# EmanueleCosenza/polyphemus

Hardware: AMD Instinct MI355X
Metric: bar-graphs/sec VAE fwd+bwd (+loss +Adam), LMD2 4-track x 32-ts synthetic (higher is better)
Workload: dtype f32 (fp16-pair MFMA products)

## Files before the change

### include/polyphemus_hip.h

```cpp
#ifndef POLYPHEMUS_HIP_H
#define POLYPHEMUS_HIP_H

#include <stdint.h>

#ifdef __cplusplus
extern "C" {
#endif

typedef void* pm_stream_t;

enum {
  PM_OK = 0,
  PM_E_INVALID = -1,
  PM_E_LAUNCH = -2,
  PM_E_UNSUPPORTED = -3
};

enum { PM_N_REL = 6, PM_N_DIST = 32, PM_N_SLOTS = 15, PM_N_PITCH = 131, PM_N_DUR = 99, PM_N_TOK = 230 };

#define PM_ABI_VERSION 9
int pm_abi_version(void);
const char* pm_build_info(void);

int pm_set_deterministic(int32_t on);
// ... 86 lines not shown
int pm_sample_structure(const float* s_logits , int32_t G, const PmStructureRules* rules, uint32_t seed,
                        float* s_f32 , uint8_t* s_u8 ,
                        int32_t* track_count , pm_stream_t stream);

int pm_notes_from_tokens(const int32_t* tokens , const float* s_tensor ,
                         int32_t G, int32_t n_bars, int64_t N, int32_t* seg_count ,
                         int32_t* seg_ptr , int32_t* bar_nodes , int32_t* node_ptr ,
                         int32_t* notes , int64_t capacity, int32_t* track_ptr ,
                         int32_t* totals , pm_stream_t stream);

#define PM_NOTES_IN_SCRATCH(B, n_bars) (3 * (int64_t)(B) * (n_bars) + 1 + 12 * (int64_t)(B))
int pm_tokens_from_notes(const int32_t* notes , const int32_t* track_ptr ,
                         int32_t B, int32_t n_bars, int64_t M, float* s_tensor ,
                         int32_t* tokens , int64_t capacity,
                         int32_t* scratch , int32_t* status ,
                         pm_stream_t stream);

int pm_edge_table(const float* nn_weight , const float* nn_bias , int32_t d,
                  float* T , pm_stream_t stream);
int pm_edge_table_bwd(const float* dT , int32_t d, float* d_nn_weight ,
                      float* d_nn_bias , pm_stream_t stream);
int pm_segreduce_fwd(const float* x , const float* T , const int32_t* plan,
                     int32_t N, int32_t E, int32_t G, int32_t d, float dropout_p, uint32_t seed,
                     uint32_t layer_uid, int32_t compact, float* A , pm_stream_t stream);
int pm_segreduce_fwd_planes(const float* x, const float* T, const int32_t* plan, int32_t N, int32_t E, int32_t G,
                            int32_t d, float dropout_p, uint32_t seed, uint32_t layer_uid, int32_t compact,
                            uint16_t* planes, int64_t plane_stride, pm_stream_t stream);
int pm_gcl_forward_fused(const float* x , const float* T , const int32_t* plan, int32_t N,
                         int32_t E, int32_t G, int32_t d, float dropout_p, uint32_t seed, uint32_t layer_uid,
                         const uint16_t* w_frag, const float* bias , int32_t use_classes,
                         float* h , double* col_stats ,
                         uint16_t* planes , int64_t plane_stride, pm_stream_t stream);
int pm_gcl_input_grad_fused(const uint16_t* dh_planes , int64_t plane_stride, const int32_t* plan,
                            int32_t N, int32_t E, int32_t G, int32_t d, const uint16_t* w_frag_t, int32_t use_classes,
                            float* dA , pm_stream_t stream);
typedef struct PmBnBwd {
  const float* h;
  const float* du;
  const float* mean; const float* var; const float* gamma; const float* beta;
  const double* acc3;
  float* dgamma; float* dbeta; float* dbias_pre;
  float eps; int32_t relu;
  int32_t add_residual;
  int32_t reserved;
} PmBnBwd;
int pm_gcl_input_grad_bn(const PmBnBwd* norm, uint16_t* dh_planes , int64_t plane_stride,
                         const int32_t* plan, int32_t N, int32_t E, int32_t G, int32_t d, const uint16_t* w_frag_t,
                         int32_t use_classes, float* dA , pm_stream_t stream);
enum { PM_ABSMAX_SLOTS = 64 };
typedef struct PmH2 {
  const uint32_t* absmax_in; const uint32_t* absmax_aux; float* scale_out; float w_scale; int32_t reserved;
} PmH2;
int pm_absmax(const float* x, int64_t n, uint32_t* out, pm_stream_t stream);
int pm_split_planes_frag_h2(const float* W, int32_t rows, int32_t cols, int32_t kind, int32_t n_mats, int64_t src_stride,
                            int64_t dst_stride, float w_scale, uint16_t* out, pm_stream_t stream);
int pm_gcl_forward_fused_h2(const float* x, const float* T, const int32_t* plan, int32_t N, int32_t E, int32_t G, int32_t d,
                            float dropout_p, uint32_t seed, uint32_t layer_uid, const uint16_t* w_frag, const float* bias,
                            int32_t use_classes, float* h, double* col_stats, uint16_t* planes, int64_t plane_stride,
                            const PmH2* h2, pm_stream_t stream);
int pm_gcl_input_grad_bn_h2(const PmBnBwd* norm, uint16_t* dh_planes, int64_t plane_stride, const int32_t* plan, int32_t N,
                            int32_t E, int32_t G, int32_t d, const uint16_t* w_frag_t, int32_t use_classes, float* dA,
                            const PmH2* h2, pm_stream_t stream);
int pm_bn_bwd_fused_h2(const float* x, const float* dy, int32_t O, int32_t C, const float* mean, const float* var, float eps,
                       const float* gamma, const float* beta, int relu, float* dgamma, float* dbeta, float* dbias_pre,
                       double* acc3, uint16_t* dx_planes, int64_t plane_stride, int32_t sums_ready, const PmH2* h2,
                       pm_stream_t stream);
int pm_gcl_input_grad_fused_h2(const uint16_t* dh_planes, int64_t plane_stride, const int32_t* plan, int32_t N, int32_t E,
                               int32_t G, int32_t d, const uint16_t* w_frag_t, int32_t use_classes, float* dA,
                               const float* dh_scale, float w_scale, pm_stream_t stream);
int pm_gcl_weight_grad_fused_h2(const uint16_t* a_planes, int64_t a_plane_stride, const uint16_t* dh_planes,
                                int64_t dh_plane_stride, const int32_t* plan, int32_t N, int32_t E, int32_t G, int32_t d,
                                int32_t use_classes, float* dW, const float* a_scale, const float* dh_scale,
                                pm_stream_t stream);
int pm_gcl_weight_grad_fused(const uint16_t* a_planes , int64_t a_plane_stride,
                             const uint16_t* dh_planes , int64_t dh_plane_stride, const int32_t* plan,
                             int32_t N, int32_t E, int32_t G, int32_t d, int32_t use_classes, float* dW ,
                             pm_stream_t stream);
int pm_gcl_forward_from_planes(const uint16_t* a_planes , int64_t plane_stride, const int32_t* plan,
                               int32_t N, int32_t E, int32_t G, int32_t d, const uint16_t* w_frag,
                               const float* bias , int32_t use_classes, float* h ,
                               double* col_stats , pm_stream_t stream);
int pm_gcl_forward_from_planes_h2(const uint16_t* a_planes, int64_t plane_stride, const int32_t* plan, int32_t N, int32_t E,
                                  int32_t G, int32_t d, const uint16_t* w_frag, const float* bias, int32_t use_classes,
                                  float* h, double* col_stats, const float* a_scale, float w_scale, pm_stream_t stream);
int pm_rows_times_weight(const float* X, int32_t ldx, int32_t N, int32_t K, const uint16_t* w_frag, int32_t kind,
                         int32_t w_tiles, int32_t Nout, const float* bias , float* C, int32_t ldc,
                         pm_stream_t stream);
int pm_rows_times_weight_longk(const float* X, int32_t ldx, int32_t N, int32_t K, const uint16_t* w_frag, int32_t kind,
                               int32_t w_pitch, int32_t Nout, float* C, int32_t ldc, pm_stream_t stream);
int pm_rows_tn_weight_grad(const float* A, int32_t lda, int32_t M, const float* B, int32_t ldb, int32_t Nn, int32_t K,
                           float* C , int32_t ldc, float* colsum_a , pm_stream_t stream);
typedef struct PmNormSums {
  const float* h;
  const float* mean; const float* var; const float* gamma; const float* beta;
  float eps; int32_t relu;
  double* acc3;
  uint32_t* absmax_out;
} PmNormSums;
int pm_segreduce_bwd_norm(const float* x, const float* T, const float* dA, const float* dres, const int32_t* plan,
                          int32_t N, int32_t E, int32_t G, int32_t d, float dropout_p, uint32_t seed,
                          uint32_t layer_uid, int32_t compact, float* dx, float* dT, const PmNormSums* next_norm,
                          pm_stream_t stream);
int pm_segreduce_bwd(const float* x, const float* T, const float* dA ,
                     const float* dres ,
                     const int32_t* plan, int32_t N, int32_t E, int32_t G, int32_t d, float dropout_p,
                     uint32_t seed, uint32_t layer_uid, int32_t compact, float* dx ,
                     float* dT , pm_stream_t stream);

int pm_bar_aggregate_fwd(const float* x, const float* T, const int32_t* plan, int32_t N, int32_t E, int32_t G, int32_t d,
                         float dropout_p, uint32_t seed, uint32_t layer_uid, uint16_t* planes, int64_t plane_stride,
                         const PmH2* h2 , pm_stream_t stream);
int pm_bar_aggregate_bwd(const float* x, const float* T, const float* dA , const float* dres ,
                         const int32_t* plan, int32_t N, int32_t E, int32_t G, int32_t d, float dropout_p, uint32_t seed,
                         uint32_t layer_uid, float* dx , float* dT ,
                         const PmNormSums* next_norm , pm_stream_t stream);

enum { PM_GEMM_RELU = 1, PM_GEMM_ACCUM = 2,
       PM_GEMM_RELU_ADD = 16 ,
       PM_GEMM_ZEROED = 8 ,
       PM_GEMM_PARTITION = 4  };
int pm_gemm_config(int32_t transA, int32_t M, int32_t N, int32_t K);
int pm_gemm_force_config(int32_t cfg);
int pm_gemm_f32(int transA, int transB, int32_t M, int32_t N, int32_t K, const float* A, int32_t lda,
                const float* B, int32_t ldb, float* C, int32_t ldc, const float* bias, int flags,
                int split_k, const int32_t* rowmap, int32_t rows_per_entry, const int32_t* dyn_entries,
                pm_stream_t stream);
int pm_gemm_f32_grouped(int transA, int transB, int32_t M, int32_t N, int32_t K, const float* A, int32_t lda,
                        const float* B, int32_t ldb, float* C, int32_t ldc, const float* bias, int flags,
                        int split_k, const int32_t* rowmap, int32_t rows_per_entry, const int32_t* dyn_entries,
                        int32_t n_groups, int64_t a_group_stride, int64_t b_group_stride, int64_t c_group_stride,
                        int64_t bias_group_stride, int32_t map_group_stride, int32_t dyn_group_stride,
                        pm_stream_t stream);
int pm_split_planes(const float* src, int64_t n, uint16_t* planes, int64_t plane_stride ,
                    pm_stream_t stream);
typedef struct PmGemmDesc {
  int32_t transA, transB, M, N, K;
  const float* A; int32_t lda;
  const float* B; int32_t ldb;
  float* C; int32_t ldc;
  const float* bias;
  int32_t flags, split_k;
  const int32_t* rowmap; int32_t rows_per_entry;
// ... 4 lines not shown
  int32_t b_split_rows; int64_t b_shared_off;
  int32_t c_split_rows; int64_t c_shared_off;
  double* col_stats;
  int32_t operand_planes;
  int64_t a_plane_stride, b_plane_stride;
  const int32_t* class_ptr;
  int32_t class_block;
  const void* b_frag;
  float* a_colsum;
} PmGemmDesc;
int pm_split_planes_frag(const float* W, int32_t rows, int32_t cols, int32_t kind, int32_t n_mats, int64_t src_stride,
                         int64_t dst_stride, uint16_t* out, pm_stream_t stream);
int pm_gemm_f32_desc(const PmGemmDesc* desc, pm_stream_t stream);

int pm_bn_stats(const float* x, int32_t O, int32_t C, int32_t I, float* mean ,
                float* var , float* running_mean ,
                float* running_var, float momentum, double* scratch , pm_stream_t stream);
int pm_bn_apply(const float* x, int32_t O, int32_t C, int32_t I, const float* mean, const float* var,
                float eps, const float* gamma, const float* beta, const float* residual ,
                int relu, float* y, pm_stream_t stream);
int pm_bn_bwd(const float* x, const float* dy, int32_t O, int32_t C, int32_t I, const float* mean,
              const float* var, float eps, const float* gamma, const float* beta, int relu,
              float* dgamma , float* dbeta , float* dbias_pre , float* dx,
              double* scratch , pm_stream_t stream);
#define PM_BN_SCRATCH(C) (256 * 3 * (C) + 4 * (C))
#define PM_BN_SMALL_MAX_ROWS 2048
int pm_bn_small_fwd(const float* x, int32_t O, int32_t C, float eps, const float* gamma, const float* beta,
                    const float* residual , int relu, float* y, float* mean ,
                    float* var , float* running_mean , float* running_var,
                    float momentum, pm_stream_t stream);
int pm_bn_small_bwd(const float* x, const float* dy, int32_t O, int32_t C, const float* mean, const float* var, float eps,
                    const float* gamma, const float* beta, int relu, float* dgamma , float* dbeta ,
                    float* dbias_pre , float* dx, pm_stream_t stream);
int pm_bn_partial_sums(const float* x, const float* dy , int32_t O, int32_t C, int32_t I, const float* mean,
                       const float* var, float eps, const float* gamma, const float* beta, int relu,
                       double* sums , double* scratch , pm_stream_t stream);
int pm_bn_stats_from_sums(const double* sums , double count, int32_t C, float* mean, float* var,
                          float* running_mean , float* running_var, float momentum, pm_stream_t stream);
int pm_bn_bwd_from_sums(const float* x, const float* dy, int32_t O, int32_t C, int32_t I, const float* mean,
                        const float* var, float eps, const float* gamma, const float* beta, int relu,
                        const double* sums_local , const double* sums_global ,
                        double count_global, float* dgamma , float* dbeta , float* dbias_pre ,
                        float* dx, double* scratch , pm_stream_t stream);

enum { PM_BN_REPL = 8 };
int pm_bn_apply_fused(const float* x, int32_t O, int32_t C, const double* sums, float eps, const float* gamma,
                      const float* beta, const float* residual , int relu, float* y,
                      float* mean , float* var , float* running_mean ,
                      float* running_var, float momentum, pm_stream_t stream);
int pm_bn_apply_fused_absmax(const float* x, int32_t O, int32_t C, const double* sums, float eps, const float* gamma,
                             const float* beta, const float* residual, int relu, float* y, float* mean, float* var,
                             float* running_mean, float* running_var, float momentum, uint32_t* absmax_out,
                             pm_stream_t stream);
int pm_bn_bwd_fused(const float* x, const float* dy, int32_t O, int32_t C, const float* mean, const float* var,
                    float eps, const float* gamma, const float* beta, int relu, float* dgamma, float* dbeta,
                    float* dbias_pre , float* dx , double* acc3,
                    uint16_t* dx_planes ,
                    int64_t plane_stride ,
                    int32_t sums_ready ,
                    pm_stream_t stream);
int pm_bn_bwd_sums(const float* x, const float* dy, int32_t O, int32_t C, const float* mean, const float* var, float eps,
                   const float* gamma, const float* beta, int relu, double* acc3, pm_stream_t stream);
int pm_bn_fold_weights(const float* W, int32_t rows, int32_t cols, const float* bias, const float* gamma, const float* beta,
                       const float* running_mean, const float* running_var, float eps, float* W_out, float* b_out,
                       pm_stream_t stream);
int pm_bn_counters_update(int64_t* counters , const int64_t* inc , const int64_t* sel ,
                          const int32_t* group_cnt , int32_t n, pm_stream_t stream);
int pm_relu_bwd(const float* dy, const float* y, int64_t n, float* dx, pm_stream_t stream);
int pm_relu_bwd_planes(const float* dy, const float* h, int64_t n, float* dh, uint16_t* planes, int64_t plane_stride,
                       pm_stream_t stream);
int pm_relu_residual_fwd(const float* x, const float* res, int64_t n, float* y, pm_stream_t stream);
int pm_dropout_rows(const float* x, int64_t rows, int32_t cols, float p, uint32_t seed, uint32_t site, float* y,
                    pm_stream_t stream);
int pm_add(const float* a, const float* b, int64_t n, float* out, pm_stream_t stream);
int pm_colsum_acc(const float* x, int32_t M, int32_t C, int32_t ld, float* out , pm_stream_t stream);
int pm_colsum_rows_acc(const float* x, int32_t C, int32_t ld, const int32_t* rowmap, int32_t rows_per_entry,
                       const int32_t* dyn_entries, int32_t max_entries, float* out , pm_stream_t stream);
int pm_reparam_fwd(const float* mu, const float* log_var, const float* eps, int64_t n, float* z, pm_stream_t stream);
int pm_reparam_bwd(const float* dz, const float* log_var, const float* eps, int64_t n, float* dmu ,
                   float* dlog_var , pm_stream_t stream);

int pm_embed_tables(const float* w_pitch_drum , const float* b_pitch_drum,
                    const float* w_pitch_nd, const float* b_pitch_nd, const float* w_dur ,
                    const float* b_dur, const float* bn_drum_g, const float* bn_drum_b,
                    const float* bn_nd_g, const float* bn_nd_b, const float* bn_dur_g, const float* bn_dur_b,
                    float* rm_drum, float* rv_drum, float* rm_nd, float* rv_nd, float* rm_dur, float* rv_dur,
                    const int32_t* tok_hist , int32_t d, int training, float eps, float momentum,
                    float* tables , float* stats ,
                    pm_stream_t stream);
int pm_embed_gather(const float* tables, const int32_t* tokens , const uint8_t* is_drum,
                    int32_t N, int32_t d, int32_t n_slots, float* X , pm_stream_t stream);
int pm_embed_bwd_scatter(const float* dX , const int32_t* tokens, const int32_t* plan, int32_t N,
                         int32_t E, int32_t G, int32_t d, int32_t n_slots,
                         float* S , pm_stream_t stream);
int pm_chord_pad_fwd(const float* tables, const float* chord_w , const float* chord_b,
                     const uint8_t* is_drum, int32_t N, int32_t d, int32_t n_slots, float* cvec ,
                     float* y , pm_stream_t stream);
int pm_chord_pad_bwd(const float* dy , const uint8_t* is_drum, int32_t N, int32_t d, int32_t n_slots,
                     const float* tables, const float* chord_w, float* gsum ,
                     float* d_chord_w , float* S , pm_stream_t stream);
int pm_chord_pad_vec(const float* tables, const float* chord_w, const float* chord_b, int32_t d, int32_t n_slots,
                     float* cvec , pm_stream_t stream);
int pm_chord_tables_fwd(const float* tables , const float* chord_w , int32_t d, int32_t n_slots,
                        float* PT, const float* chord_b , float* cvec ,
                        pm_stream_t stream);
int pm_chord_sum_fwd(const float* PT, const float* cvec, const int32_t* tokens , const uint8_t* is_drum, int32_t N,
// ... 187 lines not shown

int pm_comm_unique_id(uint8_t* id128 );
int pm_comm_init(const uint8_t* id128 , int32_t rank, int32_t world, void** comm );
int pm_comm_destroy(void* comm);
int pm_allreduce(float* buf, int64_t count, void* comm, pm_stream_t stream);

uint32_t pm_dropout_hash(uint32_t seed, uint32_t layer_uid, uint32_t eid, uint32_t channel);

enum { PM_PROF_NCLASS_PUBLIC = 35 };
int pm_prof_configure(int64_t class_mask, int32_t stride);
int pm_prof_begin(int32_t max_events);
int pm_prof_end(double* ms , double* work , int64_t* count );

#define PM_MAX_LAYERS 16
typedef struct PmLin { int64_t w, b; } PmLin;
typedef struct PmBn { int64_t w, b, rm, rv; } PmBn;
typedef struct PmGcn {
  int64_t nn_w, nn_b;
  int64_t weight[PM_MAX_LAYERS];
  int64_t bias[PM_MAX_LAYERS];
  PmBn norm[PM_MAX_LAYERS];
} PmGcn;
typedef struct PmVaeLayout {
  int32_t d, n_bars, n_layers;
  int32_t flags;
  PmLin enc_conv0; PmBn enc_bn1; PmLin enc_conv4; PmBn enc_bn5; PmLin enc_lin1, enc_lin4, enc_s_bars;
  PmLin enc_pitch_nd, enc_pitch_d, enc_dur; PmBn enc_bn_nd, enc_bn_d, enc_bn_dur; PmLin enc_chord;
  PmGcn enc_gcn; PmLin enc_gate; PmBn enc_gate_bn; PmLin enc_c_bars;
  PmLin enc_merge; PmBn enc_bn_merge; PmLin enc_mu, enc_lv;
  PmLin dec_lin; PmBn dec_bn; PmLin dec_s_bars, dec_s_lin1, dec_s_lin4, dec_conv1; PmBn dec_bn2; PmLin dec_conv4;
  PmLin dec_c_bars; PmGcn dec_gcn; PmLin dec_chord, dec_pitch_d, dec_pitch_nd, dec_dur;
  float dropout;
  int32_t reserved;
} PmVaeLayout;
typedef struct PmBatch {
  const int64_t* edge_index; const int32_t* edge_type; const int32_t* edge_dist;
  const int64_t* bars; const int64_t* batch; const uint8_t* is_drum; const int32_t* tokens; const float* s_tensor;
  int32_t N, E, G, B;
  int32_t n_slots;
  int32_t flags;
  const float* ce_scale;
} PmBatch;
int pm_vae_step_reload_switches(void);
int64_t pm_vae_layout_bytes(void);
int64_t pm_vae_step_state_bytes(void);
int64_t pm_vae_step_workspace_bytes(const PmVaeLayout* lay, int32_t N, int32_t E, int32_t G, int32_t B,
                                    int32_t n_slots);
int pm_vae_step_forward(const PmVaeLayout* lay, const float* params, float* buffers, float* grads,
                        const PmBatch* batch, int32_t* plan, const float* eps , float msg_dropout,
                        uint32_t seed_enc, uint32_t seed_dec, float beta, int structure_loss_on_logits,
                        void* workspace, int64_t workspace_bytes, void* state, double* losses ,
                        pm_stream_t stream);
int pm_vae_step_info(const void* state, int32_t* info );
int pm_vae_step_outputs(const void* state, float* s_logits, float* c_logits, float* mu, float* log_var,
                        pm_stream_t stream);
enum { PM_SAVED_GCN_H = 0,
       PM_SAVED_GCN_X,
       PM_SAVED_GCN_XIN,
       PM_SAVED_GCN_MEAN, PM_SAVED_GCN_VAR,
       PM_SAVED_GCN_T,
       PM_SAVED_X0,
       PM_SAVED_MERGE_PRE, PM_SAVED_MERGE_MEAN, PM_SAVED_MERGE_VAR,
       PM_SAVED_DEC_PRE, PM_SAVED_DEC_MEAN, PM_SAVED_DEC_VAR,
       PM_SAVED_ENC_CNN_LIN1 };
int pm_vae_step_saved(const void* state, int32_t what, int32_t stack, int32_t layer, int64_t* byte_offset, int64_t* numel);
int pm_bn_relu_decisions(const float* x , const float* mean, const float* var, const float* gamma, const float* beta,
                         float eps, int64_t rows, int32_t C, uint8_t* out , pm_stream_t stream);
int pm_vae_step_set_metrics(void* state, int64_t* counts);
int pm_vae_step_set_output_grads(void* state, const float* d_s_logits , const float* d_c_logits ,
                                 const float* d_mu , const float* d_log_var , pm_stream_t stream);
int pm_vae_step_output_views(const void* state, int64_t* byte_offset , int64_t* numel );
int pm_vae_step_backward_decoder(void* state, pm_stream_t stream);
int pm_vae_step_join_decoder_grads(void* state, pm_stream_t stream);
int pm_vae_step_backward_encoder_heads(void* state, pm_stream_t stream);
int pm_vae_step_backward_encoder(void* state, pm_stream_t stream);
int pm_vae_step_backward_encoder_tail(void* state, pm_stream_t stream);

#ifdef __cplusplus
}
#endif
#endif
```

### polyphemus_amd/_lib.py

```python
from __future__ import annotations

import ctypes as C
import os
from typing import Optional

import torch

_HERE = os.path.dirname(os.path.abspath(__file__))
LIB_PATH = os.environ.get("PM_LIB_PATH") or os.path.join(_HERE, "libpolyphemus_hip.so")

PROF_NCLASS = 40
PLAN_FIELDS = ["rowptr", "csr_src", "csr_dist", "csr_eid", "colptr", "csc_dst", "csc_reldist", "csc_eid",
               "csc_invcnt", "node_bar", "bar_ptr", "group_list", "group_cnt", "tok_hist", "row_list", "node_trel", "trk_list", "trk_cnt", "scratch"]

_SIGS = {
    "pm_plan_layout": "iiip",
    "pm_gcl_tile_order": "piipi",
    "pm_row_tile_order": "ipi",
    "pm_plan_build": "pppppppiiiiips",
    "pm_edge_attrs_to_ids": "pipps",
    "pm_tokens_from_onehot": "pips",
    "pm_batch_flags": "pppiipps",
    "pm_edge_table": "ppips",
    "pm_edge_table_bwd": "pipps",
    "pm_graph_count": "pippppps",
    "pm_graph_emit": "piippllppppppps",
    "pm_binary_from_logits": "pifpps",
    "pm_mtp_from_logits": "ppilppps",
    "pm_segreduce_fwd": "pppiiiifuuips",
    "pm_segreduce_fwd_planes": "pppiiiifuuipls",
    "pm_gcl_forward_fused": "pppiiiifuuppipppls",
    "pm_gcl_input_grad_fused": "plpiiiipips",
    "pm_gcl_input_grad_bn": "pplpiiiipips",
    "pm_chord_pad_vec": "pppiips",
    "pm_chord_tables_fwd": "ppiippps",
    "pm_chord_sum_fwd": "ppppiiips",
    "pm_chord_sum_bwd": "pppiiiiips",
    "pm_chord_tables_bwd_w": "ppiipps",
    "pm_chord_tables_bwd_x": "ppiips",
    "pm_bn_bwd_sums": "ppiippfppips",
    "pm_gcl_weight_grad_fused": "plplpiiiiips",
    "pm_gcl_forward_from_planes": "plpiiiippipps",
    "pm_rows_times_weight": "piiipiiippis",
    "pm_rows_times_weight_longk": "piiipiiipis",
    "pm_rows_tn_weight_grad": "piipiiipips",
    "pm_segreduce_bwd": "pppppiiiifuuipps",
    "pm_segreduce_bwd_norm": "pppppiiiifuuippps",
    "pm_gemm_f32": "iiiiipipipipiipips",
    "pm_gemm_f32_grouped": "iiiiipipipipiipipilllliis",
    "pm_gemm_f32_desc": "ps",
    "pm_gemm_config": "iiii",
    "pm_gemm_force_config": "i",
    "pm_bn_stats": "piiippppfps",
    "pm_bn_small_fwd": "piifpppipppppfs",
    "pm_bn_small_bwd": "ppiippfppipppps",
    "pm_bn_apply": "piiippfpppips",
    "pm_bn_partial_sums": "ppiiippfppipps",
    "pm_bn_stats_from_sums": "pDippppfs",
    "pm_bn_bwd_from_sums": "ppiiippfppippDppppps",
    "pm_bn_bwd": "ppiiippfppippppps",
    "pm_bn_apply_fused": "piipfpppipppppfs",
    "pm_bn_bwd_fused": "ppiippfppipppppplis",
    "pm_split_planes": "plpls",
    "pm_split_planes_frag": "piiiillps",
    "pm_relu_bwd": "pplps",
    "pm_add": "pplps",
    "pm_bn_counters_update": "ppppis",
    "pm_grad_accumulate": "pplfis",
    "pm_colsum_acc": "piiips",
    "pm_colsum_rows_acc": "piipipips",
    "pm_reparam_fwd": "ppplps",
    "pm_reparam_bwd": "ppplpps",
    "pm_embed_tables": "pppppppppppppppppppiiffpps",
    "pm_embed_gather": "pppiiips",
    "pm_chord_pad_fwd": "ppppiiipps",
    "pm_chord_pad_bwd": "ppiiippppps",
    "pm_embed_bwd_scatter": "pppiiiiips",
    "pm_embed_tables_bwd": "ppppppppppppifpppppppppppps",
    "pm_embed_tables_bwd_sync": "ppppppppppppifppppppppppppppps",
    "pm_gate_fwd": "pppiips",
    "pm_attnpool_fwd": "ppppfpppiiiipps",
    "pm_attnpool_bwd": "ppppfpppppiiiipppppppps",
    "pm_attnpool_bwd_sums": "ppppfpppiiiips",
    "pm_attnpool_bwd_from_sums": "ppppfpppppiiiipppppppppDs",
    "pm_relu_residual_fwd": "pplps",
    "pm_bn_fold_weights": "piipppppfpps",
    "pm_dropout_rows": "plifuups",
    "pm_bar_broadcast_fwd": "ppiiiips",
    "pm_bar_broadcast_bwd": "ppiiiips",
    "pm_conv3x3_fwd": "pppiiiiiips",
    "pm_conv3x3_bwd_data": "ppiiiiiips",
    "pm_conv3x3_bwd_weight": "ppiiiiiipps",
    "pm_maxpool4_fwd": "plps",
    "pm_maxpool4_bwd": "pplps",
    "pm_cnn_enc_fwd": "pppppppppiffppppppppppppppls",
    "pm_cnn_dec_fwd": "pppppppiffppppppppls",
    "pm_cnn_enc_bwd": "pppppppppppppppifppppppppppppls",
    "pm_content_ce": "ppppiifppppps",
    "pm_content_ce_scaled": "ppppiifpppppps",
    "pm_unembed_ce": "pppppppppiiiiifpppppppps",
    "pm_unembed_dh": "pppppiiiiippis",
    "pm_unembed_dh_scratch_bytes": "i",
    "pm_unembed_row_counts_len": "ii",
    "pm_unembed_dw": "pppiiiiippppps",
    "pm_unembed_row_lists": "ppiiiiipppps",
    "pm_unembed_ce_rows": "pppppppppiiiiifpppppppppps",
    "pm_unembed_dh_rows": "pppppiiiiipppps",
    "pm_unembed_scratch_bytes": "i",
    "pm_kld": "ppiifppps",
    "pm_unembed_bias_grads": "ppiippps",
    "pm_bce_logits": "pplfpps",
    "pm_content_accuracy": "pppips",
    "pm_structure_metrics": "pplps",
    "pm_adam_step": "pppplffffifs",
    "pm_comm_unique_id": "p",
    "pm_comm_init": "piip",
    "pm_comm_destroy": "p",
    "pm_allreduce": "plps",
    "pm_prof_configure": "li",
    "pm_prof_begin": "i",
    "pm_prof_end": "ppp",
    "pm_vae_step_workspace_bytes": "piiiii",
    "pm_vae_step_forward": "pppppppfuufiplpps",
    "pm_vae_step_info": "pp",
    "pm_vae_step_outputs": "ppppps".replace(" ", ""),
    "pm_vae_step_set_output_grads": "ppppps",
    "pm_vae_step_saved": "piiipp",
    "pm_vae_step_output_views": "ppp",
    "pm_bn_relu_decisions": "pppppflips",
    "pm_vae_step_backward_decoder": "ps",
    "pm_vae_step_backward_encoder": "ps",
    "pm_vae_step_backward_encoder_tail": "ps",
    "pm_vae_step_join_decoder_grads": "ps",
    "pm_vae_step_backward_encoder_heads": "ps",
    "pm_vae_step_reload_switches": "",
    "pm_relu_bwd_planes": "pplppls",
    "pm_absmax": "plps",
    "pm_split_planes_frag_h2": "piiiillfps",
    "pm_gcl_forward_fused_h2": "pppiiiifuuppippplps",
    "pm_gcl_input_grad_bn_h2": "pplpiiiipipps",
    "pm_gcl_weight_grad_fused_h2": "plplpiiiiippps",
    "pm_bn_bwd_fused_h2": "ppiippfppippppplips",
    "pm_gcl_input_grad_fused_h2": "plpiiiipippfs",
    "pm_bn_apply_fused_absmax": "piipfpppipppppfps",
    "pm_bar_aggregate_fwd": "pppiiiifuuplps",
    "pm_bar_aggregate_bwd": "pppppiiiifuuppps",
    "pm_gcl_forward_from_planes_h2": "plpiiiippipppfs",
    "pm_set_deterministic": "i",
    "pm_get_deterministic": "",
    "pm_deterministic_faults": "",
    "pm_h2_clamp_events": "i",
    "pm_h2_clamp_init": "",
    "pm_overflow_snapshot": "ps",
    "pm_overflow_poison": "pps",
    "pm_grad_nonfinite_check": "plpppfffis",
    "pm_adam_step_guarded": "pppplffffps",
    "pm_adam_bias_scalars": "plfffps",
    "pm_vae_step_set_metrics": "pp",
    "pm_unembed_ce_metrics": "pppppppppiiiiifppppppppppps",
    "pm_unembed_ce_rows_metrics": "pppppppppiiiiifppppppppppppps",
    "pm_content_accuracy_slots": "pppiipps",
    "pm_train_metric_counts": "pppiipplps",
    "pm_grad_sumsq": "plps",
    "pm_grad_nonfinite_check_sumsq": "plpppfffips",
    "pm_grad_clip_finish": "pffps",
    "pm_adam_step_clipped": "pppplffffipps",
    "pm_adam_step_ema": "ppppplffffiffpps",
    "pm_buffer_swap": "ppls",
    "pm_sample_tokens": "plfifups",
    "pm_mtp_from_tokens": "ppilppps",
    "pm_sample_chords": "pplpupps",
    "pm_node_tracks": "pilppps",
    "pm_sample_structure": "pipuppps",
    "pm_notes_from_tokens": "ppiilppppplpps",
    "pm_tokens_from_notes": "ppiilpplpps",
}
_CT = {"p": C.c_void_p, "i": C.c_int32, "l": C.c_int64, "f": C.c_float, "u": C.c_uint32, "s": C.c_void_p, "D": C.c_double}
_RET64 = {"pm_vae_step_workspace_bytes", "pm_vae_layout_bytes", "pm_vae_step_state_bytes", "pm_unembed_scratch_bytes",
          "pm_unembed_dh_scratch_bytes", "pm_unembed_row_counts_len"}
ABI_VERSION = 9
EXPORTED = sorted(list(_SIGS) + ["pm_abi_version", "pm_build_info", "pm_dropout_hash", "pm_sample_hash",
                                 "pm_vae_layout_bytes", "pm_vae_step_state_bytes"])



class PmChordRules(C.Structure):
    _fields_ = [("temperature", C.c_float * 2), ("top_k", C.c_int32), ("top_p", C.c_float), ("min_notes", C.c_int32 * 4),
                ("max_notes", C.c_int32 * 4), ("pitch_mask", (C.c_uint32 * 4) * 4)]


class PmStructureRules(C.Structure):
# ... 107 lines not shown
```

### polyphemus_amd/csrc/common.h

```cpp
#pragma once
#include <hip/hip_runtime.h>
#include <stdint.h>
#include "../../include/polyphemus_hip.h"

#define PM_WAVE 64

static inline int pm_check_launch() {
  hipError_t e = hipGetLastError();
  return e == hipSuccess ? PM_OK : PM_E_LAUNCH;
}

static inline int pm_device_slot() {
  int d = 0;
  if (hipGetDevice(&d) != hipSuccess || d < 0 || d >= 16) d = 0;
  return d;
}

static inline int64_t pm_cdiv(int64_t a, int64_t b) { return (a + b - 1) / b; }
static inline int64_t pm_align4(int64_t x) { return (x + 3) & ~int64_t(3); }

struct PmPlanView {
  const int32_t* rowptr; const int32_t* csr_src; const int32_t* csr_dist; const int32_t* csr_eid;
  const int32_t* colptr; const int32_t* csc_dst; const int32_t* csc_reldist; const int32_t* csc_eid;
  const float* csc_invcnt; const int32_t* node_bar; const int32_t* bar_ptr; const int32_t* group_list;
// ... 97 lines not shown
  for (int o = 32; o > 0; o >>= 1) v += __shfl_xor(v, o, 64);
  return v;
}
__device__ static inline double pm_wave_sum_d(double v) {
#pragma unroll
  for (int o = 32; o > 0; o >>= 1) v += __shfl_xor(v, o, 64);
  return v;
}
typedef __bf16 pm_bf16x2 __attribute__((ext_vector_type(2)));
typedef float pm_f32x2 __attribute__((ext_vector_type(2)));
typedef unsigned int pm_u32x2 __attribute__((ext_vector_type(2)));
__device__ static inline unsigned pm_pk_bf16(float a, float b) {
  pm_f32x2 v = {a, b};
  return __builtin_bit_cast(unsigned, __builtin_convertvector(v, pm_bf16x2));
}
__device__ static inline void pm_split3_pair(float a, float b, unsigned& h1, unsigned& h2, unsigned& h3) {
  h1 = pm_pk_bf16(a, b);
  a -= __uint_as_float(h1 << 16); b -= __uint_as_float(h1 & 0xffff0000u);
  h2 = pm_pk_bf16(a, b);
  a -= __uint_as_float(h2 << 16); b -= __uint_as_float(h2 & 0xffff0000u);
  h3 = pm_pk_bf16(a, b);
}
typedef _Float16 pm_f16x2 __attribute__((ext_vector_type(2)));
__device__ static inline unsigned pm_pk_f16(float a, float b) {
  pm_f32x2 v = {a, b};
  return __builtin_bit_cast(unsigned, __builtin_convertvector(v, pm_f16x2));
}
__device__ static inline void pm_split2h_pair(float a, float b, unsigned& h1, unsigned& h2) {
  h1 = pm_pk_f16(a, b);
  const pm_f16x2 hv = __builtin_bit_cast(pm_f16x2, h1);
  a -= (float)hv.x; b -= (float)hv.y;
  h2 = pm_pk_f16(a, b);
}
__device__ static inline float pm_pow2_scale(float bound, int target) {
  if (!(bound > 0.f) || !(bound < 3.0e38f)) return 1.f;
  const int e = (int)((__float_as_uint(bound) >> 23) & 0xff) - 126;
  int k = target - e;
  k = k < -120 ? -120 : (k > 120 ? 120 : k);
  return __uint_as_float((unsigned)(k + 127) << 23);
}
__device__ static inline float pm_clamp_f16(float v) { return fminf(fmaxf(v, -65504.f), 65504.f); }
__device__ static inline float pm_clamp_f16(float v, bool& cut) {
  const float c = fminf(fmaxf(v, -65504.f), 65504.f);
  cut = cut || (c != v);
  return c;
}
__device__ static inline float pm_absmax_read(const unsigned* __restrict__ p) {
  static_assert(PM_ABSMAX_SLOTS == 64, "one slot per lane");
  float v = __uint_as_float(p[__lane_id()]);
#pragma unroll
  for (int o = 32; o > 0; o >>= 1) v = fmaxf(v, __shfl_xor(v, o, 64));
  return v;
}
__device__ static inline void pm_absmax_block(unsigned* __restrict__ out, float v, unsigned* sm) {
  v = fabsf(v);
#pragma unroll
  for (int o = 32; o > 0; o >>= 1) v = fmaxf(v, __shfl_xor(v, o, 64));
  if ((threadIdx.x & 63) == 0) atomicMax(sm, __float_as_uint(v));
  __syncthreads();
  if (threadIdx.x == 0) atomicMax(out + (blockIdx.x % PM_ABSMAX_SLOTS), *sm);
}
__device__ static inline void pm_store_planes4(uint16_t* __restrict__ planes, int64_t plane_stride, int64_t idx, float x0,
                                               float x1, float x2, float x3) {
  unsigned l1, l2, l3, u1, u2, u3;
  pm_split3_pair(x0, x1, l1, l2, l3);
  pm_split3_pair(x2, x3, u1, u2, u3);
  const pm_u32x2 p1 = {l1, u1}, p2 = {l2, u2}, p3 = {l3, u3};
  *reinterpret_cast<pm_u32x2*>(planes + idx) = p1;
  *reinterpret_cast<pm_u32x2*>(planes + plane_stride + idx) = p2;
  *reinterpret_cast<pm_u32x2*>(planes + 2 * plane_stride + idx) = p3;
}
__device__ static inline double pm_repl_sum(const double* __restrict__ acc, int nacc, int C, int a, int c) {
  double t = 0;
#pragma unroll
  for (int r = 0; r < PM_BN_REPL; ++r) t += acc[((int64_t)r * nacc + a) * C + c];
  return t;
}
__device__ static inline float pm_bn_bwd_elem(float x, float dy, float mean, float rstd, float ga, float be, float m0,
                                              float m1, int relu) {
  const float xh = (x - mean) * rstd;
  float du = dy;
  if (relu && !(xh * ga + be > 0.f)) du = 0.f;
  return ga * rstd * (du - m0 - xh * m1);
}
__device__ static inline float pm_wave_max(float v) {
#pragma unroll
  for (int o = 32; o > 0; o >>= 1) v = fmaxf(v, __shfl_xor(v, o, 64));
  return v;
}
#endif
```

### polyphemus_amd/csrc/gemm.hip

```cpp
#include "common.h"
#include "prof.h"
#include <stdlib.h>

typedef float f32x16 __attribute__((ext_vector_type(16)));

#ifndef PM_BD_DUAL
#define PM_BD_DUAL 0
#endif
#ifndef PM_TN_DUAL
#define PM_TN_DUAL 1
#endif
#ifndef PM_PL_WAVES
#define PM_PL_WAVES 5
#endif
#ifndef PM_BD_WAVES
#define PM_BD_WAVES 5
#endif
struct GemmArgs {
  const float* A; const float* B; float* C; const float* bias;
  const int32_t* rowmap; const int32_t* dyn_entries;
  int M, N, K, lda, ldb, ldc, rpe, flags, kper, ntm, ntn;
  int64_t a_boff, b_boff, c_boff, bias_boff; int map_boff, dyn_boff;
  int b_split, c_split; int64_t b_hi, c_hi;
  int ngroups, packed;
// ... 878 lines not shown
      break;
    default: launch_t<128, 128, 32, 2, 2, 2>(transA, transB, va, vb, grid, st, g); break;
  }
  pm_prof_close(st, pe);
  return pm_check_launch();
}

extern "C" int pm_gemm_f32_grouped(int transA, int transB, int32_t M, int32_t N, int32_t K, const float* A, int32_t lda,
                                   const float* B, int32_t ldb, float* C, int32_t ldc, const float* bias, int flags,
                                   int split_k, const int32_t* rowmap, int32_t rows_per_entry,
                                   const int32_t* dyn_entries, int32_t n_groups, int64_t a_group_stride,
                                   int64_t b_group_stride, int64_t c_group_stride, int64_t bias_group_stride,
                                   int32_t map_group_stride, int32_t dyn_group_stride, pm_stream_t stream) {
  PmGemmDesc q;
  q.transA = transA; q.transB = transB; q.M = M; q.N = N; q.K = K; q.A = A; q.lda = lda; q.B = B; q.ldb = ldb;
  q.C = C; q.ldc = ldc; q.bias = bias; q.flags = flags; q.split_k = split_k; q.rowmap = rowmap;
  q.rows_per_entry = rows_per_entry; q.dyn_entries = dyn_entries; q.n_groups = n_groups;
  q.a_group_stride = a_group_stride; q.b_group_stride = b_group_stride; q.c_group_stride = c_group_stride;
  q.bias_group_stride = bias_group_stride; q.map_group_stride = map_group_stride; q.dyn_group_stride = dyn_group_stride;
  q.b_split_rows = 0; q.b_shared_off = 0; q.c_split_rows = 0; q.c_shared_off = 0; q.col_stats = nullptr;
  q.operand_planes = 0; q.a_plane_stride = 0; q.b_plane_stride = 0; q.a_colsum = nullptr;
  q.class_ptr = nullptr; q.class_block = 0; q.b_frag = nullptr;
  return pm_gemm_f32_desc(&q, stream);
}

extern "C" int pm_gemm_f32(int transA, int transB, int32_t M, int32_t N, int32_t K, const float* A, int32_t lda,
                           const float* B, int32_t ldb, float* C, int32_t ldc, const float* bias, int flags,
                           int split_k, const int32_t* rowmap, int32_t rows_per_entry, const int32_t* dyn_entries,
                           pm_stream_t stream) {
  return pm_gemm_f32_grouped(transA, transB, M, N, K, A, lda, B, ldb, C, ldc, bias, flags, split_k, rowmap,
                             rows_per_entry, dyn_entries, 1, 0, 0, 0, 0, 0, 0, stream);
}

__global__ void __launch_bounds__(256) k_split_planes(const float* __restrict__ src, int64_t n4, uint16_t* __restrict__ planes,
                                                      int64_t plane_stride) {
  for (int64_t i = (int64_t)blockIdx.x * blockDim.x + threadIdx.x; i < n4; i += (int64_t)gridDim.x * blockDim.x) {
    const float4 v = reinterpret_cast<const float4*>(src)[i];
    pm_store_planes4(planes, plane_stride, i * 4, v.x, v.y, v.z, v.w);
  }
}
extern "C" int pm_split_planes(const float* src, int64_t n, uint16_t* planes, int64_t plane_stride, pm_stream_t stream) {
  if (!src || !planes || n <= 0 || (n & 3) || plane_stride < n || (plane_stride & 3) || ((uintptr_t)src % 16) ||
      ((uintptr_t)planes % 8))
    return PM_E_INVALID;
  int64_t grid = pm_cdiv(n / 4, 256);
  if (grid > 4096) grid = 4096;
  hipLaunchKernelGGL(k_split_planes, dim3((unsigned)grid), dim3(256), 0, (hipStream_t)stream, src, n / 4, planes, plane_stride);
  return pm_check_launch();
}

template <bool H2>
__global__ void __launch_bounds__(256) k_split_planes_frag(const float* __restrict__ W, int rows, int cols, int kind,
                                                           int64_t src_stride, int64_t dst_stride,
                                                           uint16_t* __restrict__ out, float w_scale, unsigned* clamps) {
  bool cut = false;
  const float* src = W + (int64_t)blockIdx.y * src_stride;
  uint16_t* dst = out + (int64_t)blockIdx.y * dst_stride;
  const int64_t chunks = (int64_t)rows * cols / 8;
  for (int64_t c = (int64_t)blockIdx.x * blockDim.x + threadIdx.x; c < chunks; c += (int64_t)gridDim.x * blockDim.x) {
    float x[8];
    int64_t blk;
    int lane;
    if (kind == 0) {
      const int n = (int)(c / (cols / 8)), k0 = (int)(c % (cols / 8)) * 8;
      const float4 u = *reinterpret_cast<const float4*>(src + (int64_t)n * cols + k0);
      const float4 w = *reinterpret_cast<const float4*>(src + (int64_t)n * cols + k0 + 4);
      x[0] = u.x; x[1] = u.y; x[2] = u.z; x[3] = u.w; x[4] = w.x; x[5] = w.y; x[6] = w.z; x[7] = w.w;
      blk = (int64_t)(n >> 5) * (cols / 16) + (k0 >> 4);
      lane = ((k0 >> 3) & 1) * 32 + (n & 31);
    } else {
      const int n = (int)(c % cols), k0 = (int)(c / cols) * 8;
#pragma unroll
      for (int e = 0; e < 8; ++e) x[e] = src[(int64_t)(k0 + e) * cols + n];
      blk = (int64_t)(k0 >> 4) * (cols / 32) + (n >> 5);
      lane = ((k0 >> 3) & 1) * 32 + (n & 31);
    }
    unsigned p1[4], p2[4], p3[4];
    uint16_t* o = dst + blk * 1536 + lane * 8;
    if constexpr (H2) {
#pragma unroll
      for (int e = 0; e < 4; ++e) pm_split2h_pair(pm_clamp_f16(x[2 * e] * w_scale, cut), pm_clamp_f16(x[2 * e + 1] * w_scale, cut), p1[e], p2[e]);
    } else {
#pragma unroll
      for (int e = 0; e < 4; ++e) pm_split3_pair(x[2 * e], x[2 * e + 1], p1[e], p2[e], p3[e]);
      *reinterpret_cast<u32x4*>(o + 1024) = u32x4{p3[0], p3[1], p3[2], p3[3]};
    }
    *reinterpret_cast<u32x4*>(o) = u32x4{p1[0], p1[1], p1[2], p1[3]};
    *reinterpret_cast<u32x4*>(o + 512) = u32x4{p2[0], p2[1], p2[2], p2[3]};
  }
  if (H2 && cut && clamps) atomicAdd(clamps, 1u);
}
static int split_planes_frag_impl(const float* W, int32_t rows, int32_t cols, int32_t kind, int32_t n_mats,
                                  int64_t src_stride, int64_t dst_stride, float w_scale, uint16_t* out, pm_stream_t stream) {
  if (!W || !out || rows <= 0 || cols <= 0 || (rows % 32) || (cols % 32) || (kind != 0 && kind != 1) || n_mats <= 0 ||
      ((uintptr_t)W % 16) || ((uintptr_t)out % 16) || (src_stride % 4) || (dst_stride % 8))
    return PM_E_INVALID;
  int64_t grid = pm_cdiv((int64_t)rows * cols / 8, 256);
  if (grid > 2048) grid = 2048;
  if (w_scale > 0.f)
    hipLaunchKernelGGL(k_split_planes_frag<true>, dim3((unsigned)grid, (unsigned)n_mats), dim3(256), 0, (hipStream_t)stream, W,
                       rows, cols, kind, src_stride, dst_stride, out, w_scale, pm_h2_clamp_word());
  else
    hipLaunchKernelGGL(k_split_planes_frag<false>, dim3((unsigned)grid, (unsigned)n_mats), dim3(256), 0, (hipStream_t)stream, W,
                       rows, cols, kind, src_stride, dst_stride, out, 0.f, nullptr);
  return pm_check_launch();
}
extern "C" int pm_split_planes_frag(const float* W, int32_t rows, int32_t cols, int32_t kind, int32_t n_mats,
                                    int64_t src_stride, int64_t dst_stride, uint16_t* out, pm_stream_t stream) {
  return split_planes_frag_impl(W, rows, cols, kind, n_mats, src_stride, dst_stride, 0.f, out, stream);
}
extern "C" int pm_split_planes_frag_h2(const float* W, int32_t rows, int32_t cols, int32_t kind, int32_t n_mats,
                                       int64_t src_stride, int64_t dst_stride, float w_scale, uint16_t* out, pm_stream_t stream) {
  if (!(w_scale > 0.f)) return PM_E_INVALID;
  return split_planes_frag_impl(W, rows, cols, kind, n_mats, src_stride, dst_stride, w_scale, out, stream);
}
__global__ void __launch_bounds__(256) k_absmax(const float* __restrict__ x, int64_t n, unsigned* __restrict__ out) {
  __shared__ unsigned sm;
  if (threadIdx.x == 0) sm = 0u;
  __syncthreads();
  float m = 0.f;
  const int64_t n4 = n >> 2, stride = (int64_t)gridDim.x * blockDim.x;
  for (int64_t i = (int64_t)blockIdx.x * blockDim.x + threadIdx.x; i < n4; i += stride) {
    const float4 v = reinterpret_cast<const float4*>(x)[i];
    m = fmaxf(fmaxf(m, fmaxf(fabsf(v.x), fabsf(v.y))), fmaxf(fabsf(v.z), fabsf(v.w)));
  }
  if (blockIdx.x == 0 && threadIdx.x < (int)(n & 3)) m = fmaxf(m, fabsf(x[(n4 << 2) + threadIdx.x]));
  pm_absmax_block(out, m, &sm);
}
extern "C" int pm_absmax(const float* x, int64_t n, uint32_t* out, pm_stream_t stream) {
  if (!x || !out || n <= 0 || ((uintptr_t)x % 16)) return PM_E_INVALID;
  int64_t grid = pm_cdiv(n / 4 + 1, 256 * 4);
  if (grid > 512) grid = 512;
  hipLaunchKernelGGL(k_absmax, dim3((unsigned)grid), dim3(256), 0, (hipStream_t)stream, x, n, out);
  return pm_check_launch();
}

PmProfState g_pm_prof = {false, 0, 0, nullptr, ~0ull, 1, {0}};

extern "C" int pm_prof_configure(int64_t class_mask, int32_t stride) {
  if (stride < 1) return PM_E_INVALID;
  g_pm_prof.mask = (uint64_t)class_mask;
  g_pm_prof.stride = stride;
  return PM_OK;
}


extern "C" int pm_prof_begin(int32_t max_events) {
  PmProfState& p = g_pm_prof;
  if (max_events <= 0) return PM_E_INVALID;
  if (p.cap < max_events) {
    PmProfEvent* ev = (PmProfEvent*)realloc(p.ev, sizeof(PmProfEvent) * max_events);
    if (!ev) return PM_E_INVALID;
    p.ev = ev;
    for (int i = p.cap; i < max_events; ++i) {
      if (hipEventCreate(&p.ev[i].a) != hipSuccess || hipEventCreate(&p.ev[i].b) != hipSuccess) return PM_E_LAUNCH;
    }
    p.cap = max_events;
  }
  p.n = 0;
  for (int c = 0; c < PM_PROF_NCLASS; ++c) p.seen[c] = 0;
  p.on = true;
  return PM_OK;
}
extern "C" int pm_prof_end(double* ms, double* work, int64_t* count) {
  PmProfState& p = g_pm_prof;
  p.on = false;
  if (!ms || !work || !count) return PM_E_INVALID;
  for (int c = 0; c < PM_PROF_NCLASS; ++c) { ms[c] = 0; work[c] = 0; count[c] = 0; }
  for (int i = 0; i < p.n; ++i) {
    float t = 0.f;
    if (hipEventSynchronize(p.ev[i].b) != hipSuccess || hipEventElapsedTime(&t, p.ev[i].a, p.ev[i].b) != hipSuccess)
      return PM_E_LAUNCH;
    ms[p.ev[i].cls] += t; work[p.ev[i].cls] += p.ev[i].work; count[p.ev[i].cls] += 1;
  }
  p.n = 0;
  return PM_OK;
}
```

### polyphemus_amd/csrc/linear.hip

```cpp
#include "gcl_tiles.h"
#include <type_traits>
#include <stdlib.h>
#include "prof.h"
#include "wide.h"

#ifndef ROWS_NMW
#define ROWS_NMW 4
#endif
template <int D> constexpr int rows_nmw() { return D == 256 ? ROWS_NMW : 4; }
template <int D> constexpr int rows_threads() { return (rows_nmw<D>() + 4) * 64; }
template <int D, int BKIND>
__global__ void __launch_bounds__(rows_threads<D>()) __attribute__((amdgpu_waves_per_eu((rows_nmw<D>() + 4) / 4, (rows_nmw<D>() + 4) / 4)))
k_rows_w(const float* __restrict__ X, int ldx, int N, const char* __restrict__ wfrag, int wtiles, int nblk,
         const float* __restrict__ bias, float* __restrict__ C, int ldc) {
  constexpr int NMW = rows_nmw<D>(), WC = D / NMW, TN = WC / 32, KS = D / 16, RB = D * 2, PL = BM * RB;
  extern __shared__ __attribute__((aligned(16))) char smem[];
  float* const sC = reinterpret_cast<float*>(smem + 3 * PL);
  int m0 = 0, rows = BM;
  if (!pm_row_tile(N, blockIdx.x, m0, rows)) return;
  const bool full = rows > BM / 2;
  N = min(N, m0 + rows);
  const int tid = threadIdx.x, lane = tid & 63, wave = tid >> 6, li = lane & 31, lh = lane >> 5;
  if (wave >= NMW) {
    constexpr int LPR = D / 4, RPW = 64 / LPR, NR = BM / (4 * RPW);
    const int st = tid - NMW * 64, c4 = st % LPR, r0 = st / LPR;
    const __amdgpu_buffer_rsrc_t crs = __builtin_amdgcn_make_buffer_rsrc(C, 0, GCL_OOB, 0x00020000);
    __syncthreads();
#pragma unroll 1
    for (int qb = 0; qb < nblk; ++qb) {
      __syncthreads();
      __syncthreads();
      float4 bv = make_float4(0.f, 0.f, 0.f, 0.f);
      if (bias) bv = *reinterpret_cast<const float4*>(bias + qb * D + c4 * 4);
#pragma unroll
      for (int k = 0; k < NR; ++k) {
        const int rr = r0 + k * 4 * RPW, row = m0 + rr;
        float4 v = *reinterpret_cast<const float4*>(sC + rr * D + c4 * 4);
        v.x += bv.x; v.y += bv.y; v.z += bv.z; v.w += bv.w;
        __builtin_amdgcn_raw_buffer_store_b128(__builtin_bit_cast(u32x4, v), crs,
            row < N ? (int)(((int64_t)row * ldc + qb * D + c4 * 4) * 4) : GCL_OOB, 0, 0);
      }
    }
    return;
  }
  {
    const __amdgpu_buffer_rsrc_t rs = __builtin_amdgcn_make_buffer_rsrc(const_cast<float*>(X), 0, GCL_OOB, 0x00020000);
    constexpr int CPR = D / 8, NST = NMW * 64, NCHK = BM * CPR / NST;
    u32x4 v[NCHK][2];
#pragma unroll
    for (int k = 0; k < NCHK; ++k) {
      const int ci = tid + k * NST, rr = ci / CPR, ch = ci % CPR, row = m0 + rr;
#pragma unroll
      for (int h = 0; h < 2; ++h)
        v[k][h] = __builtin_amdgcn_raw_buffer_load_b128(rs, row < N ? (int)(((int64_t)row * ldx + ch * 8 + h * 4) * 4) : GCL_OOB, 0, 0);
    }
#pragma unroll
    for (int k = 0; k < NCHK; ++k) {
      const int ci = tid + k * NST, rr = ci / CPR, ch = ci % CPR;
      unsigned p1[4], p2[4], p3[4];
#pragma unroll
      for (int h = 0; h < 2; ++h) {
        pm_split3_pair(__uint_as_float(v[k][h][0]), __uint_as_float(v[k][h][1]), p1[2 * h], p2[2 * h], p3[2 * h]);
        pm_split3_pair(__uint_as_float(v[k][h][2]), __uint_as_float(v[k][h][3]), p1[2 * h + 1], p2[2 * h + 1], p3[2 * h + 1]);
      }
      char* dst = smem + rr * RB + ((ch ^ (rr & 15)) << 4);
      *reinterpret_cast<u32x4*>(dst) = u32x4{p1[0], p1[1], p1[2], p1[3]};
      *reinterpret_cast<u32x4*>(dst + PL) = u32x4{p2[0], p2[1], p2[2], p2[3]};
      *reinterpret_cast<u32x4*>(dst + 2 * PL) = u32x4{p3[0], p3[1], p3[2], p3[3]};
    }
  }
  const __amdgpu_buffer_rsrc_t brs = __builtin_amdgcn_make_buffer_rsrc(const_cast<char*>(wfrag), 0, GCL_OOB, 0x00020000);
  auto bload = [&](bf16x8 (&dst)[3][TN], int gs) {
    const int qb = min(gs / KS, nblk - 1), ks = gs % KS;
    const int n0 = qb * D + wave * WC;
    const int soff = __builtin_amdgcn_readfirstlane(BKIND == 0 ? ((n0 >> 5) * KS + ks) * 3072 : (ks * wtiles + (n0 >> 5)) * 3072);
#pragma unroll
    for (int j = 0; j < TN; ++j)
#pragma unroll
      for (int p = 0; p < 3; ++p)
        dst[p][j] = __builtin_bit_cast(bf16x8, __builtin_amdgcn_raw_buffer_load_b128(brs, lane * 16, soff + j * (BKIND == 0 ? KS : 1) * 3072 + p * 1024, 0));
  };
  bf16x8 bq[GCL_BDEPTH][3][TN];
#pragma unroll
  for (int s2 = 0; s2 < GCL_BDEPTH; ++s2) bload(bq[s2], s2);
  __syncthreads();
  auto aload = [&](bf16x8 (&a)[3][2], int ks) {
#pragma unroll
    for (int p = 0; p < 3; ++p)
#pragma unroll
      for (int i = 0; i < 2; ++i) {
        const int rr = i * 32 + li;
        a[p][i] = *reinterpret_cast<const bf16x8*>(smem + p * PL + rr * RB + (((ks * 2 + lh) ^ (rr & 15)) << 4));
      }
  };
  bf16x8 af[2][3][2];
  aload(af[0], 0);
  auto blocks = [&](auto ni_tag) {
  constexpr int NI = decltype(ni_tag)::value;
#pragma unroll 1
  for (int qb = 0; qb < nblk; ++qb) {
    f32x16 acc[2][TN];
#pragma unroll
    for (int i = 0; i < 2; ++i)
#pragma unroll
      for (int j = 0; j < TN; ++j)
#pragma unroll
        for (int r = 0; r < 16; ++r) acc[i][j][r] = 0.f;
#pragma unroll
    for (int ks = 0; ks < KS; ++ks) {
      aload(af[(ks + 1) & 1], (ks + 1) % KS);
      constexpr int PA[6] = {2, 1, 0, 1, 0, 0}, PB[6] = {0, 1, 2, 0, 1, 0};
#pragma unroll
      for (int t6 = 0; t6 < 6; ++t6)
#pragma unroll
        for (int i = 0; i < NI; ++i)
#pragma unroll
          for (int j = 0; j < TN; ++j)
            acc[i][j] = __builtin_amdgcn_mfma_f32_32x32x16_bf16(af[ks & 1][PA[t6]][i], bq[ks % GCL_BDEPTH][PB[t6]][j], acc[i][j], 0, 0, 0);
      bload(bq[ks % GCL_BDEPTH], qb * KS + ks + GCL_BDEPTH);
      __builtin_amdgcn_sched_barrier(0);
    }
    __syncthreads();
#pragma unroll
    for (int i = 0; i < 2; ++i)
#pragma unroll
      for (int r = 0; r < 16; ++r)
#pragma unroll
        for (int j = 0; j < TN; ++j)
          sC[(i * 32 + (r & 3) + 8 * (r >> 2) + 4 * lh) * D + wave * WC + j * 32 + li] = acc[i][j][r];
    __syncthreads();
  }
  };
  if (full) blocks(std::integral_constant<int, 2>{});
  else blocks(std::integral_constant<int, 1>{});
}

extern "C" int pm_rows_times_weight(const float* X, int32_t ldx, int32_t N, int32_t K, const uint16_t* w_frag, int32_t kind,
                                    int32_t w_tiles, int32_t Nout, const float* bias, float* C, int32_t ldc,
                                    pm_stream_t stream) {
  if (!X || !w_frag || !C || N <= 0 || (K != 128 && K != 256 && K != 512) || Nout <= 0 || (Nout % K) || (kind != 0 && kind != 1) ||
      ldx < K || ldc < Nout || (ldx & 3) || (ldc & 3) || ((uintptr_t)X % 16) || ((uintptr_t)C % 16) ||
      ((uintptr_t)w_frag % 16) || (bias && ((uintptr_t)bias % 16)) || (int64_t)N * ldx * 4 >= 0x7fffffffLL ||
      (int64_t)N * ldc * 4 >= 0x7fffffffLL || (kind == 1 && w_tiles * 32 < Nout))
    return PM_E_INVALID;
  if (K == 512)
    return pm_wide_rows_times_weight(X, ldx, N, w_frag, kind, w_tiles, Nout, bias, C, ldc, (hipStream_t)stream);
  hipStream_t st = (hipStream_t)stream;
  const dim3 grid(pm_row_grid(N));
  const size_t lds = (size_t)3 * BM * K * 2 + (size_t)BM * K * 4;
  const int pe = pm_prof_open(st, PM_PROF_ROWS_W, 2.0 * N * (double)K * Nout);
#define LAUNCH(DD, KD)                                                                                                 \
  do {                                                                                                                 \
    static bool once_dev[16] = {}; bool& once = once_dev[pm_device_slot()];                                                                                          \
    if (!once) {                                                                                                       \
      hipFuncSetAttribute((const void*)k_rows_w<DD, KD>, hipFuncAttributeMaxDynamicSharedMemorySize, 160 * 1024);      \
      once = true;                                                                                                     \
    }                                                                                                                  \
    hipLaunchKernelGGL((k_rows_w<DD, KD>), grid, dim3(rows_threads<DD>()), lds, st, X, ldx, N, reinterpret_cast<const char*>(w_frag), \
                       w_tiles, Nout / K, bias, C, ldc);                                                               \
  } while (0)
  if (K == 256) { if (kind == 0) LAUNCH(256, 0); else LAUNCH(256, 1); }
  else { if (kind == 0) LAUNCH(128, 0); else LAUNCH(128, 1); }
#undef LAUNCH
  pm_prof_close(st, pe);
  return pm_check_launch();
}

template <int D, int BKIND>
__global__ void __launch_bounds__(rows_threads<D>()) __attribute__((amdgpu_waves_per_eu((rows_nmw<D>() + 4) / 4, (rows_nmw<D>() + 4) / 4)))
k_rows_wk(const float* __restrict__ X, int ldx, int N, int K, const char* __restrict__ wfrag, int wpitch,
          float* __restrict__ C, int ldc) {
  constexpr int NMW = rows_nmw<D>(), WC = D / NMW, TN = WC / 32, HS = D + 8, NTHR = rows_threads<D>();
  extern __shared__ __attribute__((aligned(16))) char smem[];
  float* const sH = reinterpret_cast<float*>(smem);
  const int nchunk = K / CH;
  int m0 = 0, rows = BM;
  if (!pm_row_tile(N, blockIdx.x, m0, rows)) return;
  const bool full = rows > BM / 2;
  N = min(N, m0 + rows);
  const int tid = threadIdx.x, lane = tid & 63, wave = tid >> 6;
  if (wave >= NMW) {
    const int pt = tid - NMW * 64, q = pt & 31, prow = pt >> 5;
    const __amdgpu_buffer_rsrc_t xrs = __builtin_amdgcn_make_buffer_rsrc(const_cast<float*>(X), 0, GCL_OOB, 0x00020000);
    auto issue = [&](float4 (&xs)[8], int c) {
#pragma unroll
      for (int ps = 0; ps < 8; ++ps) {
        const int row = m0 + ps * 8 + prow;
        xs[ps] = __builtin_bit_cast(float4, __builtin_amdgcn_raw_buffer_load_b128(
            xrs, (row < N && c < nchunk) ? (int)(((int64_t)row * ldx + c * CH + q * 4) * 4) : GCL_OOB, 0, 0));
      }
    };
    auto put = [&](const float4 (&xs)[8], int c) {
      char* img = smem + (c & 1) * IMG;
#pragma unroll
      for (int ps = 0; ps < 8; ++ps) {
        const int rr = ps * 8 + prow;
        unsigned l1, l2, l3, u1, u2, u3;
        pm_split3_pair(xs[ps].x, xs[ps].y, l1, l2, l3);
        pm_split3_pair(xs[ps].z, xs[ps].w, u1, u2, u3);
        const pm_u32x2 p1 = {l1, u1}, p2 = {l2, u2}, p3 = {l3, u3};
        char* dst = img + rr * ROWB + (((q >> 1) ^ (rr & 15)) << 4) + ((q & 1) << 3);
        *reinterpret_cast<pm_u32x2*>(dst) = p1;
        *reinterpret_cast<pm_u32x2*>(dst + PLANE) = p2;
        *reinterpret_cast<pm_u32x2*>(dst + 2 * PLANE) = p3;
      }
    };
    float4 xa[8], xb[8];
    issue(xa, 0);
    issue(xb, 1);
    __builtin_amdgcn_sched_barrier(0);
    put(xa, 0);
    __syncthreads();
#pragma unroll 1
    for (int c = 0; c < nchunk; c += 2) {
      issue(xa, c + 2);
      __builtin_amdgcn_sched_barrier(0);
      put(xb, c + 1);
      __syncthreads();
      if (c + 1 >= nchunk) break;
      issue(xb, c + 3);
      __builtin_amdgcn_sched_barrier(0);
      put(xa, c + 2);
      __syncthreads();
    }
  } else {
    const int li = lane & 31, lh = lane >> 5;
    f32x16 acc[2][TN];
#pragma unroll
    for (int i = 0; i < 2; ++i)
#pragma unroll
      for (int j = 0; j < TN; ++j)
#pragma unroll
        for (int r = 0; r < 16; ++r) acc[i][j][r] = 0.f;
    const __amdgpu_buffer_rsrc_t brs = __builtin_amdgcn_make_buffer_rsrc(const_cast<char*>(wfrag), 0, GCL_OOB, 0x00020000);
    const int n0 = wave * WC;
    auto bload = [&](bf16x8 (&dst)[3][TN], int gs) {
      const int kk = min(gs, nchunk * 8 - 1);
      const int soff = __builtin_amdgcn_readfirstlane(BKIND == 0 ? ((n0 >> 5) * wpitch + kk) * 3072 : (kk * (D / 32) + (n0 >> 5)) * 3072);
#pragma unroll
      for (int j = 0; j < TN; ++j)
#pragma unroll
        for (int p = 0; p < 3; ++p)
          dst[p][j] = __builtin_bit_cast(bf16x8, __builtin_amdgcn_raw_buffer_load_b128(brs, lane * 16, soff + j * (BKIND == 0 ? wpitch : 1) * 3072 + p * 1024, 0));
    };
    bf16x8 bq[GCL_BDEPTH][3][TN];
#pragma unroll
    for (int s2 = 0; s2 < GCL_BDEPTH; ++s2) bload(bq[s2], s2);
    __syncthreads();
    auto chunks = [&](auto ni_tag) {
      constexpr int NI = decltype(ni_tag)::value;
#pragma unroll 1
      for (int c = 0; c < nchunk; ++c) {
        const char* img = smem + (c & 1) * IMG;
#pragma unroll
        for (int ks = 0; ks < 8; ++ks) {
          bf16x8 a[3][NI];
#pragma unroll
          for (int p = 0; p < 3; ++p)
#pragma unroll
            for (int i = 0; i < NI; ++i) {
              const int rr = i * 32 + li;
              a[p][i] = *reinterpret_cast<const bf16x8*>(img + p * PLANE + rr * ROWB + (((ks * 2 + lh) ^ (rr & 15)) << 4));
            }
          constexpr int PA[6] = {2, 1, 0, 1, 0, 0}, PB[6] = {0, 1, 2, 0, 1, 0};
#pragma unroll
          for (int t6 = 0; t6 < 6; ++t6)
#pragma unroll
            for (int i = 0; i < NI; ++i)
#pragma unroll
              for (int j = 0; j < TN; ++j)
                acc[i][j] = __builtin_amdgcn_mfma_f32_32x32x16_bf16(a[PA[t6]][i], bq[ks % GCL_BDEPTH][PB[t6]][j], acc[i][j], 0, 0, 0);
          bload(bq[ks % GCL_BDEPTH], c * 8 + ks + GCL_BDEPTH);
          __builtin_amdgcn_sched_barrier(0);
        }
        __syncthreads();
      }
    };
    if (full) chunks(std::integral_constant<int, 2>{});
    else chunks(std::integral_constant<int, 1>{});
#pragma unroll
    for (int j = 0; j < TN; ++j)
#pragma unroll
      for (int i = 0; i < 2; ++i)
#pragma unroll
        for (int r = 0; r < 16; ++r)
          sH[(i * 32 + (r & 3) + 8 * (r >> 2) + 4 * lh) * HS + n0 + j * 32 + li] = acc[i][j][r];
  }
  __syncthreads();
  constexpr int NG = 512 / D, RG = BM / NG;
  static_assert(NTHR >= 512, "row groups");
  const int col = tid % D, rg = tid / D;
  const __amdgpu_buffer_rsrc_t crs = __builtin_amdgcn_make_buffer_rsrc(C, 0, GCL_OOB, 0x00020000);
  if (tid >= 512) return;
#pragma unroll 8
  for (int k = 0; k < RG; ++k) {
    const int rr = rg * RG + k, row = m0 + rr;
    __builtin_amdgcn_raw_buffer_store_b32(__float_as_uint(sH[rr * HS + col]), crs, row < N ? (int)(((int64_t)row * ldc + col) * 4) : GCL_OOB, 0, 0);
  }
}

extern "C" int pm_rows_times_weight_longk(const float* X, int32_t ldx, int32_t N, int32_t K, const uint16_t* w_frag,
                                          int32_t kind, int32_t w_pitch, int32_t Nout, float* C, int32_t ldc,
                                          pm_stream_t stream) {
  if (!X || !w_frag || !C || N <= 0 || K <= 0 || (K % CH) || (Nout != 128 && Nout != 256 && Nout != 512) || (kind != 0 && kind != 1) ||
      ldx < K || ldc < Nout || (ldx & 3) || ((uintptr_t)X % 16) || ((uintptr_t)w_frag % 16) ||
      (int64_t)N * ldx * 4 >= 0x7fffffffLL || (int64_t)N * ldc * 4 >= 0x7fffffffLL || (kind == 0 && w_pitch * 16 < K))
    return PM_E_INVALID;
  if (Nout == 512)
    return pm_wide_rows_times_weight_longk(X, ldx, N, K, w_frag, kind, w_pitch, C, ldc, (hipStream_t)stream);
  hipStream_t st = (hipStream_t)stream;
  const dim3 grid(pm_row_grid(N));
  const size_t lds = 2 * IMG;
  const int pe = pm_prof_open(st, PM_PROF_ROWS_W, 2.0 * N * (double)K * Nout);
#define LAUNCH(DD, KD)                                                                                                 \
  do {                                                                                                                 \
    static bool once_dev[16] = {}; bool& once = once_dev[pm_device_slot()];                                                                                          \
    if (!once) {                                                                                                       \
      hipFuncSetAttribute((const void*)k_rows_wk<DD, KD>, hipFuncAttributeMaxDynamicSharedMemorySize, 160 * 1024);     \
      once = true;                                                                                                     \
    }                                                                                                                  \
    hipLaunchKernelGGL((k_rows_wk<DD, KD>), grid, dim3(rows_threads<DD>()), lds, st, X, ldx, N, K, reinterpret_cast<const char*>(w_frag), \
                       w_pitch, C, ldc);                                                                               \
  } while (0)
  if (Nout == 256) { if (kind == 0) LAUNCH(256, 0); else LAUNCH(256, 1); }
  else { if (kind == 0) LAUNCH(128, 0); else LAUNCH(128, 1); }
#undef LAUNCH
  pm_prof_close(st, pe);
  return pm_check_launch();
}


__global__ void __launch_bounds__(512) __attribute__((amdgpu_waves_per_eu(2, 2)))
k_rows_tn(const float* __restrict__ A, int lda, const float* __restrict__ B, int ldb, int K, int ntn, int nsplit,
          float* __restrict__ C, int ldc, float* __restrict__ colsum_a, unsigned* gate) {
  extern __shared__ __attribute__((aligned(16))) char smem[];
  const int ntile = gridDim.x / nsplit;
  int L = blockIdx.x;
  {
    const int total = gridDim.x, q = total >> 3, r = total & 7, xcd = L & 7, idx = L >> 3;
    L = (xcd < r ? xcd * (q + 1) : r * (q + 1) + (xcd - r) * q) + idx;
  }
  const int zs = L / ntile, within = L % ntile, ft = within / ntn, ct = within % ntn;
  const int kper = (((K + nsplit - 1) / nsplit + DW_KT - 1) / DW_KT) * DW_KT;
  const int kbeg = zs * kper, kend = min(kbeg + kper, K);
  if (kbeg >= kend) { pm_turn_skip_block(gate, 8); return; }
  const int nt = (kend - kbeg + DW_KT - 1) / DW_KT;
  const int tid = threadIdx.x, lane = tid & 63, wave = tid >> 6;
  const unsigned my_turn = blockIdx.x * 8 + wave;
  if (wave >= 4) {
    const int lt = tid - 256, c4 = lt & 31, r0 = lt >> 5;
    const __amdgpu_buffer_rsrc_t ars = __builtin_amdgcn_make_buffer_rsrc(const_cast<float*>(A), 0, GCL_OOB, 0x00020000);
    const __amdgpu_buffer_rsrc_t brs = __builtin_amdgcn_make_buffer_rsrc(const_cast<float*>(B), 0, GCL_OOB, 0x00020000);
    const int acol = (ft * DW_T + c4 * 4) * 4, bcol = (ct * DW_T + c4 * 4) * 4;
    float4 cs = make_float4(0.f, 0.f, 0.f, 0.f);
    const bool want_cs = colsum_a != nullptr && ct == 0;
    auto issue = [&](float4 (&v)[4][2], int t) {
#pragma unroll
      for (int j = 0; j < 4; ++j) {
        const int row = kbeg + t * DW_KT + r0 + j * 8;
        const bool ok = t < nt && row < kend;
        v[j][0] = __builtin_bit_cast(float4, __builtin_amdgcn_raw_buffer_load_b128(ars, ok ? (int)((int64_t)row * lda * 4) + acol : GCL_OOB, 0, 0));
        v[j][1] = __builtin_bit_cast(float4, __builtin_amdgcn_raw_buffer_load_b128(brs, ok ? (int)((int64_t)row * ldb * 4) + bcol : GCL_OOB, 0, 0));
      }
    };
    auto put = [&](const float4 (&v)[4][2], int t) {
      char* st = smem + (t & 1) * DW_STAGE;
#pragma unroll
      for (int j = 0; j < 4; ++j) {
        if (want_cs) { cs.x += v[j][0].x; cs.y += v[j][0].y; cs.z += v[j][0].z; cs.w += v[j][0].w; }
#pragma unroll
        for (int o = 0; o < 2; ++o) {
          unsigned l1, l2, l3, u1, u2, u3;
          pm_split3_pair(v[j][o].x, v[j][o].y, l1, l2, l3);
          pm_split3_pair(v[j][o].z, v[j][o].w, u1, u2, u3);
          const pm_u32x2 p1 = {l1, u1}, p2 = {l2, u2}, p3 = {l3, u3};
          char* dst = st + o * 3 * DW_PLANE + (r0 + j * 8) * DW_PITCH + c4 * 8;
          *reinterpret_cast<pm_u32x2*>(dst) = p1;
          *reinterpret_cast<pm_u32x2*>(dst + DW_PLANE) = p2;
          *reinterpret_cast<pm_u32x2*>(dst + 2 * DW_PLANE) = p3;
        }
      }
// ... 100 lines not shown
```

### polyphemus_amd/csrc/norm.hip

```cpp
#include "common.h"
#include <stdlib.h>

#define BN_MAX_CHUNKS 256
#define BN_NACC 3

struct BnCtx {
  const float* mean; const float* var; const float* gamma; const float* beta; float eps; int relu;
};
template <int MODE>
__device__ static inline void bn_acc(float xv, float dyv, float m, float rstd, float ga, float be, int relu,
                                     double& a, double& b, double& c) {
  if (MODE == 0) { a += (double)xv; b += (double)xv * (double)xv; }
  else {
    const float xh = (xv - m) * rstd;
    float du = dyv;
    if (relu && !(xh * ga + be > 0.f)) du = 0.f;
    a += (double)du; b += (double)du * (double)xh; c += (double)xh;
  }
}

template <int MODE>
__global__ void __launch_bounds__(256) k_colreduce_rows(const float* __restrict__ x, const float* __restrict__ dy,
                                                        int O, int C, BnCtx ctx, int rows_per_chunk,
                                                        double* __restrict__ partial) {
// ... 344 lines not shown
                                  double* sums, double* scratch, pm_stream_t stream) {
  if (!x || !sums || !scratch || O <= 0 || C <= 0 || I <= 0) return PM_E_INVALID;
  if (dy && (!mean || !var || !gamma || !beta)) return PM_E_INVALID;
  hipStream_t st = (hipStream_t)stream;
  BnCtx ctx = {mean, var, gamma, beta, eps, relu};
  int nchunk = 1;
  if (dy) run_reduce<1>(x, dy, O, C, I, ctx, scratch, &nchunk, st);
  else run_reduce<0>(x, nullptr, O, C, I, ctx, scratch, &nchunk, st);
  hipLaunchKernelGGL(k_bn_collect, dim3(pm_cdiv(C, 64)), dim3(1024), 0, st, scratch, nchunk, C, dy ? 3 : 2, sums);
  return pm_check_launch();
}
extern "C" int pm_bn_stats_from_sums(const double* sums, double count, int32_t C, float* mean, float* var,
                                     float* running_mean, float* running_var, float momentum, pm_stream_t stream) {
  if (!sums || !mean || !var || C <= 0 || !(count > 0)) return PM_E_INVALID;
  hipLaunchKernelGGL(k_bn_finalize_stats, dim3(pm_cdiv(C, 64)), dim3(1024), 0, (hipStream_t)stream, sums, 1, C, count, mean,
                     var, running_mean, running_var, momentum);
  return pm_check_launch();
}
__global__ void __launch_bounds__(256) k_bn_finalize_bwd_sync(const double* __restrict__ loc, const double* __restrict__ glob,
                                                              int C, double count_local, double count_global, BnCtx ctx,
                                                              float* dgamma, float* dbeta, float* dbias_pre, double* means) {
  const int c = blockIdx.x * blockDim.x + threadIdx.x;
  if (c >= C) return;
  if (dbeta) dbeta[c] += (float)loc[c];
  if (dgamma) dgamma[c] += (float)loc[C + c];
  const double m0 = glob[c] / count_global, m1 = glob[C + c] / count_global;
  means[c] = m0;
  means[C + c] = m1;
  if (dbias_pre) {
    const double rstd = 1.0 / sqrt((double)ctx.var[c] + (double)ctx.eps);
    dbias_pre[c] += (float)((double)ctx.gamma[c] * rstd * ((loc[c] - count_local * m0) - m1 * loc[2 * C + c]));
  }
}
extern "C" int pm_bn_bwd_from_sums(const float* x, const float* dy, int32_t O, int32_t C, int32_t I, const float* mean,
                                   const float* var, float eps, const float* gamma, const float* beta, int relu,
                                   const double* sums_local, const double* sums_global, double count_global, float* dgamma,
                                   float* dbeta, float* dbias_pre, float* dx, double* scratch, pm_stream_t stream) {
  if (!x || !dy || !mean || !var || !gamma || !beta || !sums_local || !sums_global || !dx || !scratch || O <= 0 || C <= 0 ||
      I <= 0 || !(count_global > 0))
    return PM_E_INVALID;
  hipStream_t st = (hipStream_t)stream;
  BnCtx ctx = {mean, var, gamma, beta, eps, relu};
  hipLaunchKernelGGL(k_bn_finalize_bwd_sync, dim3(pm_cdiv(C, 256)), dim3(256), 0, st, sums_local, sums_global, C,
                     (double)O * (double)I, count_global, ctx, dgamma, dbeta, dbias_pre, scratch);
  const int64_t n = (int64_t)O * C * I;
  hipLaunchKernelGGL(k_bn_bwd_apply, dim3(ew_grid(n)), dim3(256), 0, st, x, dy, n, C, I, ctx, scratch, dx);
  return pm_check_launch();
}

__global__ void __launch_bounds__(1024) k_bn_apply4_sums(const float* __restrict__ x, int64_t n4, int C, double count,
                                                        const double* __restrict__ sums, BnCtx ctx,
                                                        const float* __restrict__ res, float* __restrict__ y,
                                                        float* mean, float* var, float* rmean, float* rvar,
                                                        float momentum, unsigned* absmax) {
  extern __shared__ __attribute__((aligned(16))) float sm[];
  float amax = 0.f;
  __shared__ unsigned s_amax;
  if (threadIdx.x == 0) s_amax = 0u;
  float* const s_m = sm; float* const s_sc = sm + C; float* const s_be = sm + 2 * C;
  const int64_t stride = (int64_t)gridDim.x * blockDim.x, i0 = (int64_t)blockIdx.x * blockDim.x + threadIdx.x;
  for (int c = threadIdx.x; c < C; c += blockDim.x) {
    const double mu = pm_repl_sum(sums, 2, C, 0, c) / count;
    double v = pm_repl_sum(sums, 2, C, 1, c) / count - mu * mu;
    if (v < 0) v = 0;
    s_m[c] = (float)mu;
    s_sc[c] = rsqrtf((float)v + ctx.eps) * ctx.gamma[c];
    s_be[c] = ctx.beta[c];
    if (blockIdx.x == 0) {
      mean[c] = (float)mu;
      var[c] = (float)v;
      if (rmean) {
        const double unb = count > 1 ? v * count / (count - 1) : v;
        rmean[c] = (float)((1.0 - momentum) * rmean[c] + momentum * mu);
        rvar[c] = (float)((1.0 - momentum) * rvar[c] + momentum * unb);
      }
    }
  }
  __syncthreads();
  auto apply = [&](int64_t i, float4 xv, float4 rv) {
    const int c = (int)((i * 4) % C);
    const float4 m = *reinterpret_cast<const float4*>(s_m + c), sc = *reinterpret_cast<const float4*>(s_sc + c);
    const float4 be = *reinterpret_cast<const float4*>(s_be + c);
    float o[4] = {(xv.x - m.x) * sc.x + be.x, (xv.y - m.y) * sc.y + be.y, (xv.z - m.z) * sc.z + be.z,
                  (xv.w - m.w) * sc.w + be.w};
    if (ctx.relu) {
#pragma unroll
      for (int j = 0; j < 4; ++j) o[j] = fmaxf(o[j], 0.f);
    }
    if (res) { o[0] += rv.x; o[1] += rv.y; o[2] += rv.z; o[3] += rv.w; }
    reinterpret_cast<float4*>(y)[i] = make_float4(o[0], o[1], o[2], o[3]);
    if (absmax) amax = fmaxf(fmaxf(amax, fmaxf(fabsf(o[0]), fabsf(o[1]))), fmaxf(fabsf(o[2]), fabsf(o[3])));
  };
  for (int64_t i = i0; i < n4; i += stride) {
    const float4 xv = reinterpret_cast<const float4*>(x)[i];
    float4 rv = make_float4(0.f, 0.f, 0.f, 0.f);
    if (res) rv = reinterpret_cast<const float4*>(res)[i];
    apply(i, xv, rv);
  }
  if (absmax) pm_absmax_block(absmax, amax, &s_amax);
}
extern "C" int pm_bn_apply_fused_absmax(const float* x, int32_t O, int32_t C, const double* sums, float eps,
                                        const float* gamma, const float* beta, const float* residual, int relu, float* y,
                                        float* mean, float* var, float* running_mean, float* running_var, float momentum,
                                        uint32_t* absmax_out, pm_stream_t stream);
extern "C" int pm_bn_apply_fused(const float* x, int32_t O, int32_t C, const double* sums, float eps,
                                 const float* gamma, const float* beta, const float* residual, int relu, float* y,
                                 float* mean, float* var, float* running_mean, float* running_var, float momentum,
                                 pm_stream_t stream) {
  return pm_bn_apply_fused_absmax(x, O, C, sums, eps, gamma, beta, residual, relu, y, mean, var, running_mean, running_var,
                                  momentum, nullptr, stream);
}
extern "C" int pm_bn_apply_fused_absmax(const float* x, int32_t O, int32_t C, const double* sums, float eps,
                                        const float* gamma, const float* beta, const float* residual, int relu, float* y,
                                        float* mean, float* var, float* running_mean, float* running_var, float momentum,
                                        uint32_t* absmax_out, pm_stream_t stream) {
  if (!x || !sums || !gamma || !beta || !y || !mean || !var || O <= 0 || C <= 0 || (C % 4) != 0 || C > 4096)
    return PM_E_INVALID;
  if (((uintptr_t)x % 16) || ((uintptr_t)y % 16) || (residual && ((uintptr_t)residual % 16))) return PM_E_INVALID;
  BnCtx ctx = {nullptr, nullptr, gamma, beta, eps, relu};
  const int64_t n = (int64_t)O * C;
  constexpr int thr = 1024, gcap = 512;
  int64_t gr = pm_cdiv(n / 4, thr); if (gr > gcap) gr = gcap; if (gr < 1) gr = 1;
  hipLaunchKernelGGL(k_bn_apply4_sums, dim3((unsigned)gr), dim3(thr), sizeof(float) * 3 * C, (hipStream_t)stream, x,
                     n / 4, C, (double)O, sums, ctx, residual, y, mean, var, running_mean, running_var, momentum, absmax_out);
  return pm_check_launch();
}

__global__ void __launch_bounds__(512) k_colreduce_rows_bwd_atomic(const float* __restrict__ x,
                                                                   const float* __restrict__ dy, int O, int C,
                                                                   BnCtx ctx, int rows_per_chunk,
                                                                   double* __restrict__ acc3, unsigned* gate,
                                                                   unsigned* __restrict__ absmax_dy) {
  __shared__ double sh[8][64][12];
  __shared__ unsigned s_amax;
  if (threadIdx.x == 0) s_amax = 0u;
  float amax = 0.f;
  const int lane = threadIdx.x & 63, wave = threadIdx.x >> 6, nw = blockDim.x >> 6;
  const int c = (blockIdx.x * 64 + lane) * 4;
  const bool ok = c < C;
  double acc[12] = {0, 0, 0, 0, 0, 0, 0, 0, 0, 0, 0, 0};
  float m[4] = {0, 0, 0, 0}, rs[4] = {1, 1, 1, 1}, ga[4] = {1, 1, 1, 1}, be[4] = {0, 0, 0, 0};
  if (ok) {
#pragma unroll
    for (int j = 0; j < 4; ++j) {
      m[j] = ctx.mean[c + j]; rs[j] = rsqrtf(ctx.var[c + j] + ctx.eps);
      ga[j] = ctx.gamma[c + j]; be[j] = ctx.beta[c + j];
    }
  }
  const int r0 = blockIdx.y * rows_per_chunk;
  int r1 = r0 + rows_per_chunk;
  if (r1 > O) r1 = O;
  if (ok) {
    for (int r = r0 + wave; r < r1; r += 2 * nw) {
      const int rb = r + nw;
      const bool two = rb < r1;
      const float4 xv = *reinterpret_cast<const float4*>(x + (int64_t)r * C + c);
      const float4 dv = *reinterpret_cast<const float4*>(dy + (int64_t)r * C + c);
      float4 xw = make_float4(0.f, 0.f, 0.f, 0.f), dw = xw;
      if (two) {
        xw = *reinterpret_cast<const float4*>(x + (int64_t)rb * C + c);
        dw = *reinterpret_cast<const float4*>(dy + (int64_t)rb * C + c);
      }
      amax = fmaxf(fmaxf(amax, fmaxf(fabsf(dv.x), fabsf(dv.y))), fmaxf(fmaxf(fabsf(dv.z), fabsf(dv.w)), fmaxf(fmaxf(fabsf(dw.x), fabsf(dw.y)), fmaxf(fabsf(dw.z), fabsf(dw.w)))));
      bn_acc<1>(xv.x, dv.x, m[0], rs[0], ga[0], be[0], ctx.relu, acc[0], acc[4], acc[8]);
      bn_acc<1>(xv.y, dv.y, m[1], rs[1], ga[1], be[1], ctx.relu, acc[1], acc[5], acc[9]);
      bn_acc<1>(xv.z, dv.z, m[2], rs[2], ga[2], be[2], ctx.relu, acc[2], acc[6], acc[10]);
      bn_acc<1>(xv.w, dv.w, m[3], rs[3], ga[3], be[3], ctx.relu, acc[3], acc[7], acc[11]);
      if (two) {
        bn_acc<1>(xw.x, dw.x, m[0], rs[0], ga[0], be[0], ctx.relu, acc[0], acc[4], acc[8]);
        bn_acc<1>(xw.y, dw.y, m[1], rs[1], ga[1], be[1], ctx.relu, acc[1], acc[5], acc[9]);
        bn_acc<1>(xw.z, dw.z, m[2], rs[2], ga[2], be[2], ctx.relu, acc[2], acc[6], acc[10]);
        bn_acc<1>(xw.w, dw.w, m[3], rs[3], ga[3], be[3], ctx.relu, acc[3], acc[7], acc[11]);
      }
    }
  }
#pragma unroll
  for (int j = 0; j < 12; ++j) sh[wave][lane][j] = acc[j];
// ... 347 lines not shown
```

### polyphemus_amd/csrc/vae_step.hip

```cpp
#include "common.h"
#include <stdio.h>
#include <string.h>
#include <mutex>

int pm_plan_build_marked(const int64_t* edge_index, const int32_t* edge_type, const int32_t* edge_dist, const int64_t* bars,
                         const int64_t* batch, const uint8_t* is_drum, const int32_t* tokens, int32_t n_bars, int32_t n_slots,
                         int32_t N, int32_t E, int32_t G, int32_t* plan, hipStream_t stream, hipEvent_t after_count);
extern "C" int pm_kld_acc(const float* mu, const float* log_var, int32_t B, int32_t d, float beta, float* dmu, float* dlog_var,
                          double* out, pm_stream_t stream);
extern "C" int pm_chord_sum_fwd_absmax(const float* PT, const float* cvec, const int32_t* tokens, const uint8_t* is_drum, int32_t N, int32_t d,
                                       int32_t n_slots, float* x0, uint32_t* absmax, pm_stream_t stream);
extern "C" int pm_bn_bwd_sums_absmax(const float* x, const float* dy, int32_t O, int32_t C, const float* mean, const float* var, float eps,
                                     const float* gamma, const float* beta, int relu, double* acc3, uint32_t* absmax_dy,
                                     pm_stream_t stream);
extern "C" int pm_bce_logits_acc(const float* logits, const float* target, int64_t n, float grad_scale, float* dlogits, double* out,
                                 pm_stream_t stream);
namespace {

struct StepCfg {
  bool gcl_fused, no_dw, no_rows_w, no_classes, fused_ce, debug;
  int side_stream;
  int side_delay_us;
  bool dagg_bn;
  bool dagg_res;
  bool chord_tables;
  bool plan_side;
  bool h2;
  bool senc_first;
  bool unembed_dw;
  bool pad_skip;
  bool cnn_fused;
  bool bar_route;
  int64_t offset_limit;
};
static StepCfg read_cfg() {
  auto flag = [](const char* n, bool dflt) { const char* v = getenv(n); return v ? atoi(v) != 0 : dflt; };
  StepCfg k;
  k.gcl_fused = flag("PM_GCL_FUSED", true);
  k.no_dw = flag("PM_GCL_NO_DW", false);
  k.no_rows_w = flag("PM_NO_ROWS_W", false);
  k.no_classes = getenv("PM_GCL_NO_CLASSES") != nullptr;
  k.fused_ce = flag("PM_FUSED_CE", true);
  k.debug = getenv("PM_DEBUG") != nullptr;
  k.side_stream = getenv("PM_SIDE_STREAM") ? atoi(getenv("PM_SIDE_STREAM")) : 0xffff;
  k.dagg_bn = flag("PM_DAGG_BN", true);
  k.plan_side = flag("PM_PLAN_SIDE", true);
  k.chord_tables = flag("PM_CHORD_TABLES", true);
  k.dagg_res = flag("PM_DAGG_RES", true);
  k.h2 = flag("PM_H2", true);
  k.side_delay_us = getenv("PM_SIDE_DELAY_US") ? atoi(getenv("PM_SIDE_DELAY_US")) : 0;
  k.bar_route = flag("PM_BAR_ROUTE", true);
  k.pad_skip = flag("PM_PAD_SKIP", true);
  k.unembed_dw = flag("PM_UNEMBED_DW", true);
  k.senc_first = flag("PM_SENC_FIRST", true);
  k.cnn_fused = flag("PM_CNN_FUSED", true);
  k.offset_limit = getenv("PM_GCL_OFFSET_LIMIT") ? atoll(getenv("PM_GCL_OFFSET_LIMIT")) : 0x7fffffffLL;
  return k;
}
static StepCfg g_cfg = read_cfg();
static const StepCfg& cfg() { return g_cfg; }

struct Arena {
  char* base; size_t cap, used; bool overflow;
  size_t zcap, zused;
  void* take(size_t bytes) {
    const size_t a = (used + 255) & ~size_t(255);
    used = a + bytes;
    if (!base) return nullptr;
    if (zcap + used > cap) { overflow = true; return base + zcap; }
    return base + zcap + a;
  }
  void* z(size_t bytes) {
    const size_t a = (zused + 255) & ~size_t(255);
    zused = a + bytes;
    if (!base) return nullptr;
    if (zused > zcap) { overflow = true; return base; }
    return base + a;
  }
  bool zeroed(const void* p) const { return base && (const char*)p >= base && (const char*)p < base + zcap; }
  float* f(size_t n) { return (float*)take(n * sizeof(float)); }
  double* dbl(size_t n) { return (double*)take(n * sizeof(double)); }
  float* zf(size_t n) { return (float*)z(n * sizeof(float)); }
  double* zdbl(size_t n) { return (double*)z(n * sizeof(double)); }
};

constexpr int kDenseDeg = 16;
struct GcnRoute {
  enum Agg { AGG_IN_PRODUCT, AGG_BAR, AGG_SEG_PLANES, AGG_SEG_F32 } agg;
  enum Mul { MUL_FUSED, MUL_FROM_PLANES, MUL_GROUPED, MUL_SEVEN } mul;
  bool h2;
  bool x_tracked;
  bool plain_w_planes;
  enum Norm { NORM_IN_DAGG, NORM_PASS, NORM_NONE } norm;
  bool res_in_dagg;
  enum Dagg { DAGG_BN, DAGG_TILES, DAGG_GROUPED, DAGG_SEVEN } dagg;
  enum Dw { DW_TILES, DW_GROUPED, DW_SEVEN } dw;
  enum Bagg { BAGG_SEG_DROPPED, BAGG_BAR, BAGG_SEG } bagg;
  bool bagg_sums;
  bool bagg_absmax;
  bool frag;
  int classes;
};
struct HeadRoute {
  enum Chord { CHORD_TABLES, CHORD_FULL, CHORD_FRAG, CHORD_TILES } chord;
  bool chord_dw_tn;
  bool dec_rows;
  bool dec_dw_tn;
  enum Ue { UE_KERNEL, UE_PRODUCTS } ue_fwd, ue_dh, ue_dw;
  bool ue_rows;
  bool keep_logits;
  bool logits_only;
  bool cnn_fused;
  bool metrics;
  bool plan_side, prep_main, senc_first;
  bool sw_fused_ce, sw_gcl_fused, sw_dagg_bn; int side_mask;
};

struct GcnSaved {
  GcnRoute rt;
  float* T; float* x[PM_MAX_LAYERS + 1]; float* A[PM_MAX_LAYERS]; float* h[PM_MAX_LAYERS];
  const float* xin[PM_MAX_LAYERS];
  uint32_t site0;
  float* mean[PM_MAX_LAYERS]; float* var[PM_MAX_LAYERS];
  uint16_t* Ap[PM_MAX_LAYERS];
  uint16_t* Wp; int64_t wp_stride; int64_t wp_base;
  uint16_t* Wfn; uint16_t* Wft; int64_t wf_stride;
  double* pool;
  uint32_t seed, uid0; float p;
  uint32_t* mx; uint32_t* mdu; float* sA; float* sdh;
  bool x0_maxed;
  const float* x0_src; int64_t x0_src_n;
};
constexpr float kH2WScale = 16.f;

struct StepState {
  uint64_t magic;
  PmVaeLayout lay;
  const float* P; float* Bf; float* G;
  PmBatch bt; const int32_t* plan; const float* eps;
  Arena ar;
  double* bn_scratch; double* bn_scratch_side; double* losses;
  float beta; int fix_structure;
  float *c0, *a0, *m0, *v0, *p0, *c1, *a1, *m1, *v1, *h1, *h2, *zcat;
  float *emb_stats, *X, *x0, *tables, *cvec; GcnSaved eg; float *g, *gm, *gv, *alpha, *pooled;
  float *m, *mm, *mv, *zg, *mu, *lv, *z;
  float *zd, *dm, *dv, *zr, *sb, *u1, *u2, *c2, *a2, *m2, *v2, *s_logits, *cb; GcnSaved dg; float *H, *c_logits;
  float *dc_logits, *ds_logits, *dmu, *dlv, *dz;
  HeadRoute head;
  int32_t* ue_lists; int32_t* ue_counts; float* dH;
  float* dc_logits_own;
  float* PT;
  uint16_t *wf_enc, *wf_enc_t, *wf_dec, *wf_dec_t, *w_unembed_dh;
  const float *a1d, *h1d, *x0d, *xLg, *zcat_d, *zg_d, *zr_d, *sbd, *u1d, *H_d;
  struct { float *a1, *h1, *x0, *xLg, *zcat, *zg, *zr, *sb, *u1; } dbuf;
  uint32_t seed_enc, seed_dec;
  float *bk_dx0, *bk_dzcat;
  float *bk_dxL;
  int rc;
  unsigned br_open;
  int ext_loss;
  int64_t* metrics;
  uint8_t* verdict;
};
constexpr uint64_t kMagic = 0x504d5354455031ULL;

struct Ctx {
  StepState* s; hipStream_t st; int rc;
  double* bn_scratch;
  int N, E, Gn, B, d, nb, L, S;
  bool bn;
  float pdrop;
  int compact;
  int planes;
  const float* P; float* G; float* Bf;
  void chk(int r, int line = __builtin_LINE()) {
    if (r != PM_OK && rc == PM_OK) {
      rc = r;
      if (cfg().debug) fprintf(stderr, "[polyphemus_hip] vae_step.hip:%d returned %d\n", line, r);
    }
  }
};

// ... 133 lines not shown
static bool fused_ce_on() { return cfg().fused_ce; }
static bool unembed_dh_ok(const Ctx& c) {
  const int dh = c.d / 2;
  return cfg().fused_ce && (dh == 64 || dh == 128 || dh == 256) && (int64_t)c.N * c.S * (c.d > PM_N_TOK ? c.d : PM_N_TOK) * 4 < ((int64_t)1 << 31);
}
PmGemmDesc gcl_desc(const PmPlanView& pv, int N, int d, int classes) {
  PmGemmDesc q;
  memset(&q, 0, sizeof(q));
  q.flags = PM_GEMM_PARTITION; q.split_k = 1; q.rowmap = pv.trk_list; q.rows_per_entry = 1; q.dyn_entries = pv.trk_cnt;
  if (classes) { q.class_ptr = pv.trk_cnt + 8; q.class_block = d; }
  q.n_groups = 4; q.map_group_stride = N; q.dyn_group_stride = 1;
  return q;
}

GcnRoute gcn_route(const Ctx& c, const GcnSaved& sv) {
  const StepCfg& k = cfg();
  const int d = c.d;
  const bool dropping = c.pdrop > 0.f;
  GcnRoute r;
  r.frag = sv.Wfn && sv.Wft;
  r.classes = k.no_classes ? 0 : 1;
  const bool tiles = c.planes && c.compact && k.gcl_fused && gcl_fits(c.N, d, 1);
  const bool gcl_kernels = tiles && r.frag && gcl_width(d);
  const bool dense = (int64_t)c.E >= (int64_t)kDenseDeg * c.N;
  const bool bar = dense && c.compact && c.planes && (d % 128) == 0 && k.bar_route && !pm_det_on();
  const bool fused = gcl_kernels && !dense;
  const bool from_planes = gcl_kernels && dense && d == 512;
  r.agg = fused ? GcnRoute::AGG_IN_PRODUCT : bar ? GcnRoute::AGG_BAR : c.planes ? GcnRoute::AGG_SEG_PLANES : GcnRoute::AGG_SEG_F32;
  r.mul = fused ? GcnRoute::MUL_FUSED : from_planes ? GcnRoute::MUL_FROM_PLANES : c.compact ? GcnRoute::MUL_GROUPED : GcnRoute::MUL_SEVEN;
  r.plain_w_planes = c.planes && r.mul == GcnRoute::MUL_GROUPED;
  r.h2 = k.h2 && gcl_kernels && (!dense || (bar && d == 512)) && c.bn && (((d == 128 || d == 256) && k.dagg_bn) || d == 512) && !k.no_dw;
  r.x_tracked = r.h2 && !dropping;
  const bool in_dagg = c.bn && tiles && r.frag && (d == 128 || d == 256) && k.dagg_bn;
  r.norm = in_dagg ? GcnRoute::NORM_IN_DAGG : c.bn ? GcnRoute::NORM_PASS : GcnRoute::NORM_NONE;
  r.res_in_dagg = in_dagg && !dropping && k.dagg_res;
  r.dagg = !c.compact ? GcnRoute::DAGG_SEVEN : in_dagg ? GcnRoute::DAGG_BN : gcl_kernels ? GcnRoute::DAGG_TILES : GcnRoute::DAGG_GROUPED;
  r.dw = !c.compact ? GcnRoute::DW_SEVEN : (tiles && gcl_width(d) && !k.no_dw) ? GcnRoute::DW_TILES : GcnRoute::DW_GROUPED;
  r.bagg = dropping ? GcnRoute::BAGG_SEG_DROPPED : bar ? GcnRoute::BAGG_BAR : GcnRoute::BAGG_SEG;
  r.bagg_sums = d <= 512 && c.bn && !dropping;
  r.bagg_absmax = r.h2 && (d <= 256 || bar);
  return r;
}
HeadRoute head_route(const Ctx& c) {
  const StepCfg& k = cfg();
  const StepState& s = *c.s;
  const int d = c.d, dh = d / 2;
  const int64_t R = (int64_t)c.N * c.S;
  HeadRoute r;
  r.chord = chord_tab_ok(c) ? HeadRoute::CHORD_TABLES : c.S == PM_N_SLOTS ? HeadRoute::CHORD_FULL
          : enc_frag_ok(c) ? HeadRoute::CHORD_FRAG : HeadRoute::CHORD_TILES;
  r.chord_dw_tn = r.chord == HeadRoute::CHORD_FRAG && rows_tn_pays(d);
  r.dec_rows = rows_w_ok(c);
  r.dec_dw_tn = r.dec_rows && rows_tn_pays(d);
  r.keep_logits = (s.bt.flags & 4) != 0;
  r.logits_only = (s.bt.flags & 8) != 0;
  r.metrics = !r.logits_only && s.metrics != nullptr;
  r.plan_side = k.plan_side;
  r.prep_main = r.chord == HeadRoute::CHORD_TABLES && r.plan_side;
  r.senc_first = k.senc_first;
  r.cnn_fused = k.cnn_fused && c.bn;
  r.ue_fwd = (fused_ce_on() && !r.logits_only) ? HeadRoute::UE_KERNEL : HeadRoute::UE_PRODUCTS;
  r.ue_dh = unembed_dh_ok(c) ? HeadRoute::UE_KERNEL : HeadRoute::UE_PRODUCTS;
  r.ue_rows = k.pad_skip && fused_ce_on() && r.plan_side && unembed_dh_ok(c) && !r.logits_only;
  r.ue_dw = (k.unembed_dw && dh % 128 == 0 && !pm_det_on() && R * PM_N_TOK * 4 < ((int64_t)1 << 31) && R * (int64_t)d * 4 < ((int64_t)1 << 31))
                ? HeadRoute::UE_KERNEL : HeadRoute::UE_PRODUCTS;
  r.sw_fused_ce = k.fused_ce; r.sw_gcl_fused = k.gcl_fused; r.sw_dagg_bn = k.dagg_bn;
  r.side_mask = k.side_stream;
  return r;
}
void head_route_gradient_in_any_row(HeadRoute& r) { r.ue_rows = false; }
void gcn_prepare(Ctx& c, const PmGcn& g, GcnSaved& sv) {
  Arena& ar = c.s->ar;
  const int d = c.d;
  const int64_t dd = (int64_t)d * d;
  sv.T = ar.f((size_t)PM_N_DIST * d);
  if (ar.base) RUN(pm_edge_table(c.P + g.nn_w, c.P + g.nn_b, d, sv.T, c.st));
  sv.pool = ar.zdbl((size_t)c.L * 5 * d * PM_BN_REPL);
  {
    constexpr int SL = PM_ABSMAX_SLOTS;
    uint32_t* w = (uint32_t*)ar.z(sizeof(uint32_t) * (size_t)((2 * c.L + 1) * SL + 2 * c.L));
    sv.mx = w; sv.mdu = w ? w + (c.L + 1) * SL : nullptr; sv.sA = w ? (float*)(w + (2 * c.L + 1) * SL) : nullptr;
    sv.sdh = w ? sv.sA + c.L : nullptr;
  }
  const int64_t lstride = c.L > 2 ? g.weight[2] - g.weight[1] : 7 * dd;
  sv.Wfn = sv.Wft = nullptr; sv.wf_stride = 7 * dd * 3;
  if (c.planes) {
    sv.wp_base = g.weight[0];
    sv.wp_stride = (g.weight[c.L - 1] + 7 * dd - g.weight[0] + 7) & ~(int64_t)7;
    for (int i = 0; i < c.L; ++i)
      if (g.weight[i] < sv.wp_base || ((g.weight[i] - sv.wp_base) & 7)) RUN(PM_E_INVALID);
    sv.Wp = (uint16_t*)ar.take((size_t)sv.wp_stride * 6);
    bool even = (d % 32) == 0 && c.compact && (lstride % 4) == 0;
    for (int i = 2; i < c.L; ++i) even = even && (g.weight[i] - g.weight[i - 1] == lstride);
    if (even) {
      sv.Wfn = (uint16_t*)ar.take((size_t)sv.wf_stride * 2 * c.L);
      sv.Wft = (uint16_t*)ar.take((size_t)sv.wf_stride * 2 * c.L);
    }
  }
  const GcnRoute& r = sv.rt = gcn_route(c, sv);
  if (r.frag) {
    auto split = [&](const float* W, int n_mats, int64_t src_stride, int kind, uint16_t* dst) {
      if (r.h2) RUN(pm_split_planes_frag_h2(W, 7 * d, d, kind, n_mats, src_stride, sv.wf_stride, kH2WScale, dst, c.st));
      else RUN(pm_split_planes_frag(W, 7 * d, d, kind, n_mats, src_stride, sv.wf_stride, dst, c.st));
    };
    for (int kind = 0; kind < 2; ++kind) {
      uint16_t* dst = kind ? sv.Wfn : sv.Wft;
      split(c.P + g.weight[0], 1, 7 * dd, kind, dst);
      if (c.L > 1) split(c.P + g.weight[1], c.L - 1, lstride, kind, dst + sv.wf_stride);
    }
    if (r.h2) RUN(pm_absmax(sv.T, (int64_t)PM_N_DIST * d, sv.mx + c.L * PM_ABSMAX_SLOTS, c.st));
  }
  if (r.plain_w_planes)
    RUN(pm_split_planes(c.P + sv.wp_base, sv.wp_stride & ~(int64_t)3, sv.Wp, sv.wp_stride, c.st));
}

float* gcn_forward(Ctx& c, float* x0, const PmGcn& g, GcnSaved& sv, uint32_t seed, uint32_t uid0, float p) {
  Arena& ar = c.s->ar;
  const int N = c.N, d = c.d, nb = c.compact ? 4 : 7;
  const int64_t dd = (int64_t)d * d;
  sv.seed = seed; sv.uid0 = uid0; sv.p = p;
  PmPlanView pv;
  if (ar.base) pv = pm_plan_view(c.s->plan, N, c.E, c.Gn);
  sv.x[0] = x0;
  const int64_t aps = (int64_t)N * nb * d;
  const GcnRoute& r = sv.rt;
  const bool dropping = c.pdrop > 0.f;
  sv.site0 = uid0 == 0 ? SITE_ENC_GCN : SITE_DEC_GCN;
  for (int i = 0; i < c.L; ++i) {
    if (c.planes) { sv.Ap[i] = (uint16_t*)ar.take((size_t)aps * 6); sv.A[i] = nullptr; }
    else sv.A[i] = ar.f((size_t)N * nb * d);
    sv.h[i] = ar.f((size_t)N * d); sv.x[i + 1] = ar.f((size_t)N * d);
    sv.mean[i] = ar.f(d); sv.var[i] = ar.f(d);
    float* xdrop = dropping ? ar.f((size_t)N * d) : nullptr;
    if (!ar.base) continue;
    sv.xin[i] = drop(c, sv.x[i], N, d, sv.site0 + i, seed, xdrop);
// ... 11 lines not shown
      h2.absmax_in = sv.mx + i * PM_ABSMAX_SLOTS; h2.absmax_aux = sv.mx + c.L * PM_ABSMAX_SLOTS; h2.scale_out = sv.sA + i;
      h2.w_scale = kH2WScale; h2.reserved = 0;
    }
    switch (r.agg) {
      case GcnRoute::AGG_IN_PRODUCT:
        if (r.h2)
          RUN(pm_gcl_forward_fused_h2(sv.xin[i], sv.T, c.s->plan, N, c.E, c.Gn, d, p, seed, uid0 + i, Wf, bias, r.classes,
                                        sv.h[i], sums, sv.Ap[i], aps, &h2, c.st));
        else
          RUN(pm_gcl_forward_fused(sv.xin[i], sv.T, c.s->plan, N, c.E, c.Gn, d, p, seed, uid0 + i, Wf, bias, r.classes,
                                     sv.h[i], sums, sv.Ap[i], aps, c.st));
        break;
      case GcnRoute::AGG_BAR:
        RUN(pm_bar_aggregate_fwd(sv.xin[i], sv.T, c.s->plan, N, c.E, c.Gn, d, p, seed, uid0 + i, sv.Ap[i], aps, r.h2 ? &h2 : nullptr, c.st)); break;
      case GcnRoute::AGG_SEG_PLANES:
        RUN(pm_segreduce_fwd_planes(sv.xin[i], sv.T, c.s->plan, N, c.E, c.Gn, d, p, seed, uid0 + i, 1, sv.Ap[i], aps, c.st)); break;
      case GcnRoute::AGG_SEG_F32:
        RUN(pm_segreduce_fwd(sv.xin[i], sv.T, c.s->plan, N, c.E, c.Gn, d, p, seed, uid0 + i, c.compact, sv.A[i], c.st)); break;
    }
    switch (r.mul) {
      case GcnRoute::MUL_FUSED: break;
      case GcnRoute::MUL_FROM_PLANES:
        if (r.h2)
          RUN(pm_gcl_forward_from_planes_h2(sv.Ap[i], aps, c.s->plan, N, c.E, c.Gn, d, Wf, bias, r.classes, sv.h[i], sums,
                                              sv.sA + i, kH2WScale, c.st));
        else
          RUN(pm_gcl_forward_from_planes(sv.Ap[i], aps, c.s->plan, N, c.E, c.Gn, d, Wf, bias, r.classes, sv.h[i], sums, c.st));
        break;
      case GcnRoute::MUL_SEVEN: {
        PmGemmDesc q;
        memset(&q, 0, sizeof(q));
        q.M = N; q.N = d; q.K = 7 * d; q.split_k = 1; q.n_groups = 1;
        q.A = sv.A[i]; q.lda = 7 * d; q.B = W; q.ldb = d; q.C = sv.h[i]; q.ldc = d; q.bias = bias;
        q.col_stats = sums;
        RUN(pm_gemm_f32_desc(&q, c.st));
        break;
      }
      case GcnRoute::MUL_GROUPED: {
        PmGemmDesc q = gcl_desc(pv, N, d, r.classes);
        q.M = N; q.N = d; q.K = 4 * d;
        q.A = sv.A[i]; q.lda = 4 * d; q.B = W; q.ldb = d; q.C = sv.h[i]; q.ldc = d; q.bias = bias;
        q.b_group_stride = dd; q.b_split_rows = d; q.b_shared_off = 3 * dd;
        q.col_stats = sums;
        if (c.planes) {
          q.operand_planes = 1; q.A = (const float*)sv.Ap[i]; q.a_plane_stride = aps;
          q.B = (const float*)(sv.Wp + (g.weight[i] - sv.wp_base)); q.b_plane_stride = sv.wp_stride;
          q.b_frag = Wf;
        }
        RUN(pm_gemm_f32_desc(&q, c.st));
        break;
      }
    }
    const PmBn& bn = g.norm[i];
    if (c.bn)
      RUN(pm_bn_apply_fused_absmax(sv.h[i], N, d, sums, 1e-5f, c.P + bn.w, c.P + bn.b, sv.x[i], 1, sv.x[i + 1], sv.mean[i],
                                     sv.var[i], c.Bf + bn.rm, c.Bf + bn.rv, 0.1f,
                                     (r.x_tracked && i + 1 < c.L) ? sv.mx + (i + 1) * PM_ABSMAX_SLOTS : nullptr, c.st));
    else
      RUN(pm_relu_residual_fwd(sv.h[i], sv.x[i], (int64_t)N * d, sv.x[i + 1], c.st));
  }
  return sv.x[c.L];
}
float* gcn_backward(Ctx& c, float* dx, const PmGcn& g, GcnSaved& sv) {
  Arena& ar = c.s->ar;
  const int N = c.N, d = c.d, nb = c.compact ? 4 : 7;
  const int64_t dd = (int64_t)d * d;
  float* dT = ar.zf((size_t)PM_N_DIST * d);
  float* dh = ar.f((size_t)N * d);
  float* dA = ar.f((size_t)N * nb * d);
  const int64_t aps = (int64_t)N * nb * d, dps = (int64_t)N * d;
  uint16_t* const dhp = c.planes ? (uint16_t*)ar.take((size_t)dps * 6) : nullptr;
  float* dxa = ar.f((size_t)N * d);
  float* dxb = ar.f((size_t)N * d);
  PmPlanView pv = pm_plan_view(c.s->plan, N, c.E, c.Gn);
  float* dxin = c.pdrop > 0.f ? ar.f((size_t)N * d) : nullptr;
  const GcnRoute& r = sv.rt;
  for (int i = c.L - 1; i >= 0; --i) {
    const float* W = c.P + g.weight[i];
    float* dW = c.G + g.weight[i];
    const PmBn& bn = g.norm[i];
    const uint16_t* Wf = r.frag ? sv.Wft + (int64_t)i * sv.wf_stride : nullptr;
    double* const acc3 = sv.pool + ((size_t)i * 5 + 2) * d * PM_BN_REPL;
    const bool sums_ready = i < c.L - 1 && r.bagg_sums;
    const bool du_tracked = sums_ready && r.bagg_absmax, du_from_sums = r.norm == GcnRoute::NORM_IN_DAGG && !sums_ready;
    PmH2 h2 = {};
    if (r.h2) { h2.absmax_in = sv.mdu + i * PM_ABSMAX_SLOTS; h2.scale_out = sv.sdh + i; h2.w_scale = kH2WScale; }
    switch (r.norm) {
      case GcnRoute::NORM_IN_DAGG:
        if (!sums_ready)
          RUN(pm_bn_bwd_sums_absmax(sv.h[i], dx, N, d, sv.mean[i], sv.var[i], 1e-5f, c.P + bn.w, c.P + bn.b, 1, acc3,
                                      (r.h2 && du_from_sums) ? sv.mdu + i * PM_ABSMAX_SLOTS : nullptr, c.st));
        break;
      case GcnRoute::NORM_PASS:
        if (r.h2) {
          if (!du_tracked) RUN(pm_absmax(dx, (int64_t)N * d, sv.mdu + i * PM_ABSMAX_SLOTS, c.st));
          RUN(pm_bn_bwd_fused_h2(sv.h[i], dx, N, d, sv.mean[i], sv.var[i], 1e-5f, c.P + bn.w, c.P + bn.b, 1, c.G + bn.w, c.G + bn.b,
                                   c.G + g.bias[i], acc3, dhp, dps, sums_ready ? 1 : 0, &h2, c.st));
        } else
          RUN(pm_bn_bwd_fused(sv.h[i], dx, N, d, sv.mean[i], sv.var[i], 1e-5f, c.P + bn.w, c.P + bn.b, 1, c.G + bn.w,
                                c.G + bn.b, c.G + g.bias[i], c.planes ? nullptr : dh, acc3, dhp, dps, sums_ready ? 1 : 0, c.st));
        break;
      case GcnRoute::NORM_NONE:
        RUN(pm_relu_bwd_planes(dx, sv.h[i], (int64_t)N * d, dh, c.planes ? dhp : nullptr, dps, c.st));
        RUN(pm_colsum_acc(dh, N, d, d, c.G + g.bias[i], c.st));
        break;
    }
    switch (r.dagg) {
// ... 190 lines not shown
  br.resume();
  if (!rt.plan_side) chord_encoder_planes(c, 0);
  chord_encoder_planes(c, 1);
  gcn_prepare(c, s.lay.enc_gcn, s.eg);
  br.mark(BR_WPREP);
  br.pause();
}
float* embeddings_and_chord_encoder(Ctx& c) {
  StepState& s = *c.s; Arena& ar = s.ar; const PmVaeLayout& Y = s.lay;
  const HeadRoute& rt = s.head;
  const int N = c.N, B = c.B, d = c.d, dh = d / 2, S = c.S;
  const bool dropping = c.pdrop > 0.f, chord_tab = chord_tab_ok(c);
  s.tables = ar.f((size_t)4 * PM_N_PITCH * dh);
  s.emb_stats = ar.f((size_t)4 * 2 * dh);
  s.X = chord_tab ? nullptr : ar.f((size_t)N * S * d);
  s.PT = chord_tab ? ar.f((size_t)2 * S * 2 * PM_N_PITCH * d) : nullptr;
  s.x0 = ar.f((size_t)N * d);
  s.cvec = ar.f((size_t)2 * d);
  s.dbuf.x0 = dropping ? ar.f((size_t)N * d) : nullptr;
  s.dbuf.xLg = dropping ? ar.f((size_t)N * d) : nullptr;
  s.dbuf.zcat = dropping ? ar.f((size_t)B * 2 * d) : nullptr;
  s.dbuf.zg = dropping ? ar.f((size_t)B * d) : nullptr;
  float* const stack_in = dropping ? s.dbuf.x0 : s.x0;
  if (!ar.base) return stack_in;
  const PmPlanView pv = pm_plan_view(s.plan, N, c.E, c.Gn);
  branch_join(c, BR_PLAN_COUNT);
  RUN(pm_embed_tables(EMB_PARAMS(c.P), c.Bf + Y.enc_bn_d.rm, c.Bf + Y.enc_bn_d.rv, c.Bf + Y.enc_bn_nd.rm, c.Bf + Y.enc_bn_nd.rv,
                        c.Bf + Y.enc_bn_dur.rm, c.Bf + Y.enc_bn_dur.rv, pv.tok_hist, d, 1, 1e-5f, 0.1f, s.tables, s.emb_stats, c.st));
  if (rt.chord == HeadRoute::CHORD_TABLES) {
    RUN(pm_chord_tables_fwd(s.tables, c.P + Y.enc_chord.w, d, S, s.PT, c.P + Y.enc_chord.b, s.cvec, c.st));
    s.eg.x0_maxed = s.eg.mx != nullptr;
    RUN(pm_chord_sum_fwd_absmax(s.PT, s.cvec, s.bt.tokens, s.bt.is_drum, N, d, S, s.x0, s.eg.mx, c.st));
    if (!rt.plan_side) branch_join(c, BR_WPREP);
  } else {
    RUN(pm_embed_gather(s.tables, s.bt.tokens, s.bt.is_drum, N, d, S, s.X, c.st));
    if (!rt.plan_side) branch_join(c, BR_WPREP);
    switch (rt.chord) {
      case HeadRoute::CHORD_FULL: lin(c, s.X, Y.enc_chord, N, d, PM_N_SLOTS * d, s.x0, true); break;
      case HeadRoute::CHORD_FRAG:
        RUN(pm_rows_times_weight_longk(s.X, S * d, N, S * d, s.wf_enc, 0, PM_N_SLOTS * d / 16, d, s.x0, d, c.st)); break;
      default:
        RUN(pm_gemm_f32(0, 1, N, d, S * d, s.X, S * d, c.P + Y.enc_chord.w, PM_N_SLOTS * d, s.x0, d, nullptr, 0, 1, nullptr, 0,
                          nullptr, c.st));
    }
    if (rt.chord != HeadRoute::CHORD_FULL)
      RUN(pm_chord_pad_fwd(s.tables, c.P + Y.enc_chord.w, c.P + Y.enc_chord.b, s.bt.is_drum, N, d, S, s.cvec, s.x0, c.st));
  }
  s.x0d = drop(c, s.x0, N, d, SITE_ENC_CHORD, s.seed_enc, s.dbuf.x0);
  return stack_in;
}
void decoder_prep(Ctx& c, BranchScope& br) {
  StepState& s = *c.s; Arena& ar = s.ar; const PmVaeLayout& Y = s.lay;
  const int N = c.N, d = c.d, S = c.S;
  gcn_prepare(c, Y.dec_gcn, s.dg);
  if (rows_w_ok(c)) {
    s.wf_dec = (uint16_t*)ar.take((size_t)S * d * d * 6);
    s.wf_dec_t = (uint16_t*)ar.take((size_t)S * d * d * 6);
    for (int kind = 0; kind < 2; ++kind)
      RUN(pm_split_planes_frag(c.P + Y.dec_chord.w, S * d, d, kind, 1, (int64_t)S * d * d, (int64_t)S * d * d * 3,
                                 kind ? s.wf_dec_t : s.wf_dec, c.st));
  }
  if (unembed_dh_ok(c)) {
    s.w_unembed_dh = (uint16_t*)ar.take((size_t)pm_unembed_dh_scratch_bytes(d));
    RUN(pm_unembed_dh(nullptr, c.P + Y.dec_pitch_d.w, c.P + Y.dec_pitch_nd.w, c.P + Y.dec_dur.w, nullptr, N, c.E, c.Gn, d, S,
                        nullptr, s.w_unembed_dh, 1, c.st));
  }
  s.dH = ar.f((size_t)N * S * d);
  s.ue_lists = (int32_t*)ar.take((size_t)6 * N * S * sizeof(int32_t));
  s.ue_counts = (int32_t*)ar.take((size_t)pm_unembed_row_counts_len(N, S) * sizeof(int32_t));
  if (s.head.ue_rows)
    RUN(pm_unembed_row_lists(s.bt.tokens, s.plan, N, c.E, c.Gn, d, S, s.ue_lists,
                               s.head.keep_logits ? s.ue_lists + (size_t)3 * N * S : nullptr, s.ue_counts, s.dH, c.st));
  br.mark(BR_WPREP_DEC);
}
void structure_encoder(Ctx& c, BranchScope& br) {
  StepState& s = *c.s; const PmVaeLayout& Y = s.lay;
  const int Gn = c.Gn, d = c.d, nb = c.nb;
  if (s.ar.base) {
    if (s.head.cnn_fused) {
      RUN(pm_cnn_enc_fwd(s.bt.s_tensor, c.P + Y.enc_conv0.w, c.P + Y.enc_conv0.b, c.P + Y.enc_bn1.w, c.P + Y.enc_bn1.b,
                           c.P + Y.enc_conv4.w, c.P + Y.enc_conv4.b, c.P + Y.enc_bn5.w, c.P + Y.enc_bn5.b, Gn, 1e-5f, 0.1f, s.c0, s.a0,
                           s.p0, s.c1, s.a1, s.m0, s.v0, c.Bf + Y.enc_bn1.rm, c.Bf + Y.enc_bn1.rv, s.m1, s.v1, c.Bf + Y.enc_bn5.rm,
                           c.Bf + Y.enc_bn5.rv, c.bn_scratch, bn_scratch_len(c), c.st));
    } else {
      RUN(pm_conv3x3_fwd(s.bt.s_tensor, c.P + Y.enc_conv0.w, c.P + Y.enc_conv0.b, Gn, 1, 8, 4, 32, 0, s.c0, c.st));
      cnn_act_fwd(c, s.c0, Gn, 8, 128, Y.enc_bn1, s.a0, s.m0, s.v0);
      RUN(pm_maxpool4_fwd(s.a0, (int64_t)Gn * 8 * 32, s.p0, c.st));
      RUN(pm_conv3x3_fwd(s.p0, c.P + Y.enc_conv4.w, c.P + Y.enc_conv4.b, Gn, 8, 16, 4, 8, 0, s.c1, c.st));
      cnn_act_fwd(c, s.c1, Gn, 16, 32, Y.enc_bn5, s.a1, s.m1, s.v1);
    }
    s.a1d = drop(c, s.a1, Gn, 512, SITE_ENC_CNN_IN, s.seed_enc, s.dbuf.a1);
    lin(c, s.a1d, Y.enc_lin1, Gn, d, 512, s.h1, true);
    s.h1d = drop(c, s.h1, Gn, d, SITE_ENC_CNN_MID, s.seed_enc, s.dbuf.h1);
    lin(c, s.h1d, Y.enc_lin4, Gn, d, d, s.h2, false);
    lin(c, s.h2, Y.enc_s_bars, c.B, d, nb * d, s.zcat + d, false, nb * d, 2 * d);
  }
  br.mark(BR_ENC_S_FWD);
}
void decoder_prep_and_structure_encoder(Ctx& c, BranchScope& br) {
  br.resume();
  if (c.s->head.senc_first) { structure_encoder(c, br); decoder_prep(c, br); }
  else { decoder_prep(c, br); structure_encoder(c, br); }
  br.end();
}
void attention_pool(Ctx& c, float* xL) {
  StepState& s = *c.s; Arena& ar = s.ar; const PmVaeLayout& Y = s.lay;
  const int N = c.N, Gn = c.Gn, d = c.d;
  s.g = ar.f(N); s.gm = ar.f(4); s.gv = ar.f(4); s.alpha = ar.f(N); s.pooled = ar.f((size_t)Gn * d);
  if (!ar.base) return;
  s.xLg = drop(c, xL, N, d, SITE_ENC_GATE, s.seed_enc, s.dbuf.xLg);
  RUN(pm_gate_fwd(s.xLg, c.P + Y.enc_gate.w, c.P + Y.enc_gate.b, N, d, s.g, c.st));
  RUN(pm_bn_stats(s.g, N, 1, 1, s.gm, s.gv, c.Bf + Y.enc_gate_bn.rm, c.Bf + Y.enc_gate_bn.rv, 0.1f, c.bn_scratch, c.st));
  RUN(pm_attnpool_fwd(xL, s.g, s.gm, s.gv, 1e-5f, c.P + Y.enc_gate_bn.w, c.P + Y.enc_gate_bn.b, s.plan, N, c.E, Gn, d,
// ... 28 lines not shown
  if (!s.fix_structure) RUN(pm_bce_logits_acc(s.bt.s_tensor, s.bt.s_tensor, (int64_t)c.Gn * 128, 1.0f, nullptr, s.losses, c.st));
}
float* decoder_trunk(Ctx& c) {
  StepState& s = *c.s; Arena& ar = s.ar; const PmVaeLayout& Y = s.lay;
  const int N = c.N, Gn = c.Gn, B = c.B, d = c.d;
  const bool dropping = c.pdrop > 0.f;
  s.zd = ar.zf((size_t)B * 2 * d); s.dm = ar.f(2 * d); s.dv = ar.f(2 * d); s.zr = ar.f((size_t)B * 2 * d);
  s.sb = ar.zf((size_t)Gn * d); s.u1 = ar.f((size_t)Gn * d); s.u2 = ar.f((size_t)Gn * 512);
  s.c2 = ar.f((size_t)Gn * 8 * 128); s.a2 = ar.f((size_t)Gn * 8 * 128); s.m2 = ar.f(8); s.v2 = ar.f(8);
  s.s_logits = ar.f((size_t)Gn * 128); s.cb = ar.zf((size_t)Gn * d);
  float* xd0 = ar.f((size_t)N * d);
  s.dbuf.zr = dropping ? ar.f((size_t)B * 2 * d) : nullptr;
  s.dbuf.sb = dropping ? ar.f((size_t)Gn * d) : nullptr;
  s.dbuf.u1 = dropping ? ar.f((size_t)Gn * d) : nullptr;
  if (!ar.base) return xd0;
  lin(c, s.z, Y.dec_lin, B, 2 * d, d, s.zd, false);
  bn_fwd(c, s.zd, B, 2 * d, 1, Y.dec_bn, true, nullptr, s.zr, s.dm, s.dv);
  s.zr_d = drop(c, s.zr, B, 2 * d, SITE_DEC_IN, s.seed_dec, s.dbuf.zr);
  lin(c, s.zr_d + d, Y.dec_c_bars, B, c.nb * d, d, s.cb, false, 2 * d, 0);
  RUN(pm_bar_broadcast_fwd(s.cb, s.plan, N, c.E, Gn, d, xd0, c.st));
  return xd0;
}
void structure_decoder(Ctx& c) {
  StepState& s = *c.s;
  if (!s.ar.base) return;
  const PmVaeLayout& Y = s.lay;
  const int Gn = c.Gn, d = c.d;
  BranchScope br(c, BR_DEC_FWD);
  lin(c, s.zr_d, Y.dec_s_bars, c.B, c.nb * d, d, s.sb, false, 2 * d, 0);
  s.sbd = drop(c, s.sb, Gn, d, SITE_DEC_CNN_IN, s.seed_dec, s.dbuf.sb);
  lin(c, s.sbd, Y.dec_s_lin1, Gn, d, d, s.u1, true);
  s.u1d = drop(c, s.u1, Gn, d, SITE_DEC_CNN_MID, s.seed_dec, s.dbuf.u1);
  lin(c, s.u1d, Y.dec_s_lin4, Gn, 512, d, s.u2, true);
  if (s.head.cnn_fused) {
    RUN(pm_cnn_dec_fwd(s.u2, c.P + Y.dec_conv1.w, c.P + Y.dec_conv1.b, c.P + Y.dec_bn2.w, c.P + Y.dec_bn2.b, c.P + Y.dec_conv4.w,
                         c.P + Y.dec_conv4.b, Gn, 1e-5f, 0.1f, s.c2, s.a2, s.s_logits, s.m2, s.v2, c.Bf + Y.dec_bn2.rm,
                         c.Bf + Y.dec_bn2.rv, c.bn_scratch, bn_scratch_len(c), c.st));
    return;
  }
  RUN(pm_conv3x3_fwd(s.u2, c.P + Y.dec_conv1.w, c.P + Y.dec_conv1.b, Gn, 16, 8, 4, 32, 1, s.c2, c.st));
  cnn_act_fwd(c, s.c2, Gn, 8, 128, Y.dec_bn2, s.a2, s.m2, s.v2);
  RUN(pm_conv3x3_fwd(s.a2, c.P + Y.dec_conv4.w, c.P + Y.dec_conv4.b, Gn, 8, 1, 4, 32, 0, s.s_logits, c.st));
}
void decoder_head(Ctx& c, const float* xdL) {
  StepState& s = *c.s; Arena& ar = s.ar; const PmVaeLayout& Y = s.lay;
  const HeadRoute& rt = s.head;
  const int N = c.N, Gn = c.Gn, d = c.d, S = c.S;
  const int64_t R = (int64_t)N * S;
  s.H = ar.f((size_t)R * d); s.c_logits = ar.f((size_t)R * PM_N_TOK);
  s.dc_logits = s.dc_logits_own = ar.f((size_t)R * PM_N_TOK); s.ds_logits = ar.f((size_t)Gn * 128);
  uint16_t* const w_unembed = fused_ce_on() ? (uint16_t*)ar.take((size_t)pm_unembed_scratch_bytes(d)) : nullptr;
  double* const pad_losses = ar.zdbl(4);
  if (!ar.base) return;
  if (rt.dec_rows) RUN(pm_rows_times_weight(xdL, d, N, d, s.wf_dec, 0, 0, S * d, c.P + Y.dec_chord.b, s.H, S * d, c.st));
  else lin(c, xdL, Y.dec_chord, N, S * d, d, s.H, false);
  drop(c, s.H, N, S * d, SITE_DEC_CHORD, s.seed_dec, s.H);
  int64_t* const met = rt.metrics ? s.metrics : nullptr;
  if (rt.ue_fwd == HeadRoute::UE_KERNEL) {
#define UE_ARGS(logits, db_d, db_nd, db_dur, out)                                                                              \
  s.H, c.P + Y.dec_pitch_d.w, c.P + Y.dec_pitch_d.b, c.P + Y.dec_pitch_nd.w, c.P + Y.dec_pitch_nd.b, c.P + Y.dec_dur.w,       \
  c.P + Y.dec_dur.b, s.bt.tokens, s.plan, N, c.E, Gn, d, S, 1.0f, s.bt.ce_scale, logits, s.dc_logits, db_d, db_nd, db_dur, out, w_unembed
#define UE_STEP UE_ARGS(rt.keep_logits ? s.c_logits : nullptr, c.G + Y.dec_pitch_d.b, c.G + Y.dec_pitch_nd.b, c.G + Y.dec_dur.b, s.losses)
    if (rt.ue_rows && met) RUN(pm_unembed_ce_rows_metrics(UE_STEP, s.ue_lists, s.ue_counts, nullptr, s.verdict, met, c.st));
    else if (met) RUN(pm_unembed_ce_metrics(UE_STEP, nullptr, s.verdict, met, c.st));
    else if (rt.ue_rows) RUN(pm_unembed_ce_rows(UE_STEP, s.ue_lists, s.ue_counts, c.st));
    else RUN(pm_unembed_ce(UE_STEP, c.st));
    if (rt.ue_rows && rt.keep_logits)
      RUN(pm_unembed_ce_rows(UE_ARGS(s.c_logits, nullptr, nullptr, nullptr, pad_losses), s.ue_lists + 3 * R, s.ue_counts + 4, c.st));
#undef UE_STEP
#undef UE_ARGS
  } else {
    unembed_products(c, UE_LOGITS, false, nullptr);
    if (!rt.logits_only) {
      const PmPlanView pv = pm_plan_view(s.plan, N, c.E, Gn);
      RUN(pm_content_ce_scaled(s.c_logits, s.bt.tokens, pv.tok_hist, s.bt.is_drum, N, S, 1.0f, s.bt.ce_scale, s.dc_logits,
                                 c.G + Y.dec_pitch_d.b, c.G + Y.dec_pitch_nd.b, c.G + Y.dec_dur.b, s.losses, c.st));
    }
    if (met) RUN(pm_content_accuracy_slots(s.c_logits, s.bt.tokens, nullptr, N, S, s.verdict, met, c.st));
  }
  branch_join(c, BR_LOSSES);
  branch_join(c, BR_DEC_FWD);
  if (!rt.logits_only && s.fix_structure)
    RUN(pm_bce_logits_acc(s.s_logits, s.bt.s_tensor, (int64_t)Gn * 128, 1.0f, s.ds_logits, s.losses, c.st));
  if (met)
    RUN(pm_train_metric_counts(s.bt.tokens, s.bt.is_drum, s.verdict, N, S, s.fix_structure ? s.s_logits : s.bt.s_tensor,
                               s.bt.s_tensor, (int64_t)Gn * 128, met, c.st));
}

void forward(Ctx& c, float msg_p, uint32_t seed_enc, uint32_t seed_dec) {
  StepState& s = *c.s; Arena& ar = s.ar; const PmVaeLayout& Y = s.lay;
  const bool run = ar.base != nullptr;
  s.seed_enc = seed_enc; s.seed_dec = seed_dec;
  s.head = head_route(c);
  s.bn_scratch = ar.dbl((size_t)bn_scratch_len(c));
  s.bn_scratch_side = ar.dbl((size_t)bn_scratch_len(c));
  c.bn_scratch = s.bn_scratch;
  carve_structure_encoder(c);
  BranchScope br(c, BR_ENC_FWD);
  plan_and_encoder_prep(c, br);
  float* x0 = embeddings_and_chord_encoder(c);
  if (run) branch_join(c, BR_WPREP);
  float* xL = gcn_forward(c, x0, Y.enc_gcn, s.eg, seed_enc, 0, msg_p);
  decoder_prep_and_structure_encoder(c, br);
  attention_pool(c, xL);
  merge_and_latent(c);
  float* xd0 = decoder_trunk(c);
  if (run) branch_join(c, BR_WPREP_DEC);
  if (run) branch_join(c, BR_ENC_FWD);
  s.dg.x0_src = s.cb; s.dg.x0_src_n = (int64_t)c.Gn * c.d;
  float* xdL = gcn_forward(c, xd0, Y.dec_gcn, s.dg, seed_dec, 1000, msg_p);
  structure_decoder(c);
  decoder_head(c, xdL);
}

void structure_decoder_backward(Ctx& c, float* dzr) {
  StepState& s = *c.s; Arena& ar = s.ar; const PmVaeLayout& Y = s.lay;
  const int Gn = c.Gn, d = c.d;
  BranchScope br(c, BR_DEC_BWD);
  float* da2 = ar.f((size_t)Gn * 8 * 128); float* dc2 = ar.f((size_t)Gn * 8 * 128);
  float* du2 = ar.f((size_t)Gn * 512); float* du1 = ar.zf((size_t)Gn * d); float* dsb = ar.zf((size_t)Gn * d);
  RUN(pm_conv3x3_bwd_weight(s.a2, s.ds_logits, Gn, 8, 1, 4, 32, 0, c.G + Y.dec_conv4.w, c.G + Y.dec_conv4.b, c.st));
  RUN(pm_conv3x3_bwd_data(s.ds_logits, c.P + Y.dec_conv4.w, Gn, 8, 1, 4, 32, 0, da2, c.st));
  cnn_act_bwd(c, s.c2, da2, Gn, 8, 128, Y.dec_bn2, s.m2, s.v2, dc2);
  RUN(pm_conv3x3_bwd_weight(s.u2, dc2, Gn, 16, 8, 4, 32, 1, c.G + Y.dec_conv1.w, c.G + Y.dec_conv1.b, c.st));
  RUN(pm_conv3x3_bwd_data(dc2, c.P + Y.dec_conv1.w, Gn, 16, 8, 4, 32, 1, du2, c.st));
  RUN(pm_relu_bwd(du2, s.u2, (int64_t)Gn * 512, du2, c.st));
  lin_bwd(c, du2, s.u1d, Y.dec_s_lin4, Gn, 512, d, du1);
  drop(c, du1, Gn, d, SITE_DEC_CNN_MID, s.seed_dec, du1);
  RUN(pm_relu_bwd(du1, s.u1, (int64_t)Gn * d, du1, c.st));
  lin_bwd(c, du1, s.sbd, Y.dec_s_lin1, Gn, d, d, dsb);
  drop(c, dsb, Gn, d, SITE_DEC_CNN_IN, s.seed_dec, dsb);
  lin_bwd(c, dsb, s.zr_d, Y.dec_s_bars, c.B, c.nb * d, d, dzr, 0, 2 * d, 2 * d);
}
void unembed_input_grad(Ctx& c) {
  StepState& s = *c.s; const PmVaeLayout& Y = s.lay;
  const HeadRoute& rt = s.head;
  const int N = c.N, d = c.d, S = c.S;
  if (rt.ue_dh == HeadRoute::UE_PRODUCTS) unembed_products(c, UE_DH, false, s.dH);
  else if (rt.ue_rows)
    RUN(pm_unembed_dh_rows(s.dc_logits, c.P + Y.dec_pitch_d.w, c.P + Y.dec_pitch_nd.w, c.P + Y.dec_dur.w, s.plan, N, c.E, c.Gn, d, S,
                             s.dH, s.w_unembed_dh, s.ue_lists, s.ue_counts, c.st));
  else
    RUN(pm_unembed_dh(s.dc_logits, c.P + Y.dec_pitch_d.w, c.P + Y.dec_pitch_nd.w, c.P + Y.dec_dur.w, s.plan, N, c.E, c.Gn, d, S,
                        s.dH, s.w_unembed_dh, 0, c.st));
  drop(c, s.dH, N, S * d, SITE_DEC_CHORD, s.seed_dec, s.dH);
}
void decoder_weight_grads(Ctx& c) {
  StepState& s = *c.s; const PmVaeLayout& Y = s.lay;
  const HeadRoute& rt = s.head;
  const int N = c.N, d = c.d, S = c.S;
  BranchScope br(c, BR_DEC_WGRAD);
  if (rt.ue_dw == HeadRoute::UE_KERNEL)
    RUN(pm_unembed_dw(s.dc_logits, s.H, s.plan, N, c.E, c.Gn, d, S, c.G + Y.dec_pitch_d.w, c.G + Y.dec_pitch_nd.w, c.G + Y.dec_dur.w,
                        rt.ue_rows ? s.ue_lists : nullptr, rt.ue_rows ? s.ue_counts : nullptr, c.st));
  else unembed_products(c, UE_DW, rt.ue_rows, nullptr);
  if (s.ext_loss) {
    RUN(pm_unembed_bias_grads(s.dc_logits, s.bt.is_drum, N, S, c.G + Y.dec_pitch_d.b, c.G + Y.dec_pitch_nd.b, c.G + Y.dec_dur.b, c.st));
  }
  if (rt.dec_dw_tn)
    RUN(pm_rows_tn_weight_grad(s.dH, S * d, S * d, s.dg.x[c.L], d, d, N, c.G + Y.dec_chord.w, d, c.G + Y.dec_chord.b, c.st));
  else if (rt.dec_rows) lin_bwd(c, s.dH, s.dg.x[c.L], Y.dec_chord, N, S * d, d, nullptr);
}
// ... 232 lines not shown
    return PM_E_INVALID;
  if (lay->n_layers > PM_MAX_LAYERS || lay->n_layers <= 0 || (lay->d & 7) || batch->G != batch->B * lay->n_bars ||
      batch->n_slots < 1 || batch->n_slots > PM_N_SLOTS)
    return PM_E_INVALID;
  StepState* s = (StepState*)state;
  int64_t* const metrics = s->metrics;
  memset(s, 0, sizeof(*s));
  s->metrics = metrics;
  s->magic = kMagic; s->lay = *lay; s->P = params; s->Bf = buffers; s->G = grads; s->bt = *batch; s->plan = plan;
  s->eps = eps; s->losses = losses; s->beta = beta; s->fix_structure = structure_loss_on_logits;
  s->ar.base = (char*)workspace; s->ar.cap = (size_t)workspace_bytes; s->ar.used = 0; s->ar.overflow = false;
  hipStream_t st = (hipStream_t)stream;
  size_t zb, mb;
  measure_step(lay, *batch, &zb, &mb);
  if (zb + mb > (size_t)workspace_bytes) return PM_E_INVALID;
  if (metrics) {
    const size_t tail = metrics_tail_bytes(batch->N, batch->n_slots);
    if (zb + mb + tail + 256 > (size_t)workspace_bytes) return PM_E_INVALID;
    s->verdict = (uint8_t*)workspace + (((size_t)workspace_bytes - tail) & ~size_t(255));
  }
  s->ar.zcap = zb; s->ar.zused = 0;
  if (cfg().side_stream) {
    Branch* b = branch_of_device();
    if (b && (hipEventRecord(b->idle, b->st) != hipSuccess || hipStreamWaitEvent(st, b->idle, 0) != hipSuccess)) return PM_E_LAUNCH;
  }
  if (hipMemsetAsync(workspace, 0, zb, st) != hipSuccess) return PM_E_LAUNCH;
  Ctx c = make_ctx(s, st);
  forward(c, msg_dropout, seed_enc, seed_dec);
  if (s->ar.overflow) return PM_E_INVALID;
  s->rc = c.rc;
  return c.rc;
}
extern "C" int pm_vae_step_set_metrics(void* state, int64_t* counts) {
  if (!state) return PM_E_INVALID;
  ((StepState*)state)->metrics = counts;
  return PM_OK;
}
extern "C" int pm_vae_step_info(const void* state, int32_t* info) {
  const StepState* s = (const StepState*)state;
  if (!s || !info || s->magic != kMagic) return PM_E_INVALID;
  StepState tmp = *s;
  Ctx c = make_ctx(&tmp, nullptr);
  info[0] = c.compact; info[1] = c.planes; info[2] = c.S;
  info[3] = (s->eg.rt.frag && s->dg.rt.frag) ? 1 : 0;
  info[4] = c.N; info[5] = c.E; info[6] = c.Gn; info[7] = c.B;
  const HeadRoute& rt = s->head;
  info[8] = rt.sw_fused_ce ? 1 : 0; info[9] = pm_det_on() ? 0 : rt.side_mask; info[10] = pm_det_on(); info[11] = rt.sw_gcl_fused ? 1 : 0;
  info[12] = rt.sw_dagg_bn ? 1 : 0;
  info[13] = rt.chord == HeadRoute::CHORD_TABLES ? 1 : 0;
  info[14] = (s->eg.rt.h2 ? 1 : 0) | (s->dg.rt.h2 ? 2 : 0);
  info[15] = rt.ue_rows ? 1 : 0;
  return PM_OK;
}
extern "C" int pm_vae_step_outputs(const void* state, float* s_logits, float* c_logits, float* mu, float* log_var,
                                   pm_stream_t stream) {
  const StepState* s = (const StepState*)state;
  if (!s || s->magic != kMagic || s->rc != PM_OK || !s->s_logits) return PM_E_INVALID;
  hipStream_t st = (hipStream_t)stream;
  const size_t N = s->bt.N, S = s->bt.n_slots, G = s->bt.G, B = s->bt.B, d = s->lay.d;
  hipError_t e = hipSuccess;
  if (s_logits && e == hipSuccess) e = hipMemcpyAsync(s_logits, s->s_logits, sizeof(float) * G * 128, hipMemcpyDeviceToDevice, st);
  if (c_logits && s->head.ue_fwd == HeadRoute::UE_KERNEL && !s->head.keep_logits) return PM_E_INVALID;
  if (c_logits && e == hipSuccess) e = hipMemcpyAsync(c_logits, s->c_logits, sizeof(float) * N * S * PM_N_TOK, hipMemcpyDeviceToDevice, st);
  if (mu && e == hipSuccess) e = hipMemcpyAsync(mu, s->mu, sizeof(float) * B * d, hipMemcpyDeviceToDevice, st);
  if (log_var && e == hipSuccess) e = hipMemcpyAsync(log_var, s->lv, sizeof(float) * B * d, hipMemcpyDeviceToDevice, st);
  return e == hipSuccess ? PM_OK : PM_E_LAUNCH;
}

extern "C" int pm_vae_step_set_output_grads(void* state, const float* d_s_logits, const float* d_c_logits, const float* d_mu,
                                            const float* d_log_var, pm_stream_t stream) {
  StepState* s = (StepState*)state;
  if (!s || s->magic != kMagic || s->rc != PM_OK || !s->dc_logits || !s->dmu || s->bk_dxL || s->bk_dx0) return PM_E_INVALID;
  hipStream_t st = (hipStream_t)stream;
  const size_t N = s->bt.N, S = s->bt.n_slots, G = s->bt.G, B = s->bt.B, d = s->lay.d;
  auto put = [&](float* dst, const float* src, size_t n) {
    if (src == dst) return hipSuccess;
    return src ? hipMemcpyAsync(dst, src, sizeof(float) * n, hipMemcpyDeviceToDevice, st) : hipMemsetAsync(dst, 0, sizeof(float) * n, st);
  };
  hipError_t e = hipSuccess;
  if (d_c_logits && d_c_logits != s->dc_logits_own && !((uintptr_t)d_c_logits % 16)) s->dc_logits = const_cast<float*>(d_c_logits);
  else { s->dc_logits = s->dc_logits_own; if (d_c_logits != s->dc_logits_own) e = put(s->dc_logits_own, d_c_logits, N * S * PM_N_TOK); }
  if (e == hipSuccess && d_s_logits) e = put(s->ds_logits, d_s_logits, G * 128);
  if (e == hipSuccess) e = put(s->dmu, d_mu, B * d);
  if (e == hipSuccess) e = put(s->dlv, d_log_var, B * d);
  const PmVaeLayout& Y = s->lay;
  if (e == hipSuccess) e = hipMemsetAsync(s->G + Y.dec_pitch_d.b, 0, sizeof(float) * PM_N_PITCH, st);
  if (e == hipSuccess) e = hipMemsetAsync(s->G + Y.dec_pitch_nd.b, 0, sizeof(float) * PM_N_PITCH, st);
  if (e == hipSuccess) e = hipMemsetAsync(s->G + Y.dec_dur.b, 0, sizeof(float) * PM_N_DUR, st);
  s->fix_structure = d_s_logits ? 1 : 0;
  s->ext_loss = 1;
  head_route_gradient_in_any_row(s->head);
  return e == hipSuccess ? PM_OK : PM_E_LAUNCH;
}

extern "C" int pm_vae_step_output_views(const void* state, int64_t* byte_offset, int64_t* numel) {
  const StepState* s = (const StepState*)state;
  if (!s || s->magic != kMagic || !byte_offset || !numel || !s->ar.base || !s->s_logits || !s->c_logits) return PM_E_INVALID;
  const int64_t N = s->bt.N, S = s->bt.n_slots, G = s->bt.G, B = s->bt.B, d = s->lay.d;
  const float* p[8] = {s->s_logits, s->c_logits, s->mu, s->lv, s->ds_logits, s->dc_logits_own, s->dmu, s->dlv};
  const int64_t n[8] = {G * 128, N * S * PM_N_TOK, B * d, B * d, G * 128, N * S * PM_N_TOK, B * d, B * d};
  for (int i = 0; i < 8; ++i) {
    if (!p[i]) return PM_E_INVALID;
    byte_offset[i] = (int64_t)((const char*)p[i] - s->ar.base);
    numel[i] = n[i];
  }
  return PM_OK;
// ... 80 lines not shown
```

### polyphemus_amd/native.py

```python
from __future__ import annotations

import ctypes as C
import os

import torch

from ._lib import lib

PM_MAX_LAYERS = 16


_PLANES = os.environ.get("PM_GCL_PLANES", "1") != "0"


class PmLin(C.Structure):
    _fields_ = [("w", C.c_int64), ("b", C.c_int64)]


class PmBn(C.Structure):
    _fields_ = [("w", C.c_int64), ("b", C.c_int64), ("rm", C.c_int64), ("rv", C.c_int64)]


class PmGcn(C.Structure):
    _fields_ = [("nn_w", C.c_int64), ("nn_b", C.c_int64), ("weight", C.c_int64 * PM_MAX_LAYERS),
                ("bias", C.c_int64 * PM_MAX_LAYERS), ("norm", PmBn * PM_MAX_LAYERS)]


_LAYOUT = [
    ("enc_conv0", "lin", "encoder.s_encoder.cnn_encoder.conv.0"), ("enc_bn1", "bn", "encoder.s_encoder.cnn_encoder.conv.1"),
    ("enc_conv4", "lin", "encoder.s_encoder.cnn_encoder.conv.4"), ("enc_bn5", "bn", "encoder.s_encoder.cnn_encoder.conv.5"),
    ("enc_lin1", "lin", "encoder.s_encoder.cnn_encoder.lin.1"), ("enc_lin4", "lin", "encoder.s_encoder.cnn_encoder.lin.4"),
    ("enc_s_bars", "lin", "encoder.s_encoder.bars_encoder"),
    ("enc_pitch_nd", "lin", "encoder.c_encoder.non_drums_pitch_emb"), ("enc_pitch_d", "lin", "encoder.c_encoder.drums_pitch_emb"),
    ("enc_dur", "lin", "encoder.c_encoder.dur_emb"), ("enc_bn_nd", "bn", "encoder.c_encoder.bn_non_drums"),
    ("enc_bn_d", "bn", "encoder.c_encoder.bn_drums"), ("enc_bn_dur", "bn", "encoder.c_encoder.bn_dur"),
    ("enc_chord", "lin", "encoder.c_encoder.chord_encoder"), ("enc_gcn", "gcn", "encoder.c_encoder.graph_encoder"),
    ("enc_gate", "lin", "encoder.c_encoder.graph_attention.gate_nn.0.layers.0"),
    ("enc_gate_bn", "bn", "encoder.c_encoder.graph_attention.gate_nn.1"), ("enc_c_bars", "lin", "encoder.c_encoder.bars_encoder"),
    ("enc_merge", "lin", "encoder.linear_merge"), ("enc_bn_merge", "bn", "encoder.bn_linear_merge"),
    ("enc_mu", "lin", "encoder.linear_mu"), ("enc_lv", "lin", "encoder.linear_log_var"),
    ("dec_lin", "lin", "decoder.lin_decoder"), ("dec_bn", "bn", "decoder.batch_norm"),
    ("dec_s_bars", "lin", "decoder.s_decoder.bars_decoder"), ("dec_s_lin1", "lin", "decoder.s_decoder.cnn_decoder.lin.1"),
    ("dec_s_lin4", "lin", "decoder.s_decoder.cnn_decoder.lin.4"), ("dec_conv1", "lin", "decoder.s_decoder.cnn_decoder.conv.1"),
    ("dec_bn2", "bn", "decoder.s_decoder.cnn_decoder.conv.2"), ("dec_conv4", "lin", "decoder.s_decoder.cnn_decoder.conv.4"),
    ("dec_c_bars", "lin", "decoder.c_decoder.bars_decoder"), ("dec_gcn", "gcn", "decoder.c_decoder.graph_decoder"),
    ("dec_chord", "lin", "decoder.c_decoder.chord_decoder"), ("dec_pitch_d", "lin", "decoder.c_decoder.drums_pitch_emb"),
    ("dec_pitch_nd", "lin", "decoder.c_decoder.non_drums_pitch_emb"), ("dec_dur", "lin", "decoder.c_decoder.dur_emb"),
]
_KIND = {"lin": PmLin, "bn": PmBn, "gcn": PmGcn}


class PmVaeLayout(C.Structure):
    _fields_ = ([("d", C.c_int32), ("n_bars", C.c_int32), ("n_layers", C.c_int32), ("flags", C.c_int32)] +
                [(f, _KIND[k]) for f, k, _ in _LAYOUT] + [("dropout", C.c_float), ("reserved", C.c_int32)])


class PmBatch(C.Structure):
    _fields_ = [("edge_index", C.c_void_p), ("edge_type", C.c_void_p), ("edge_dist", C.c_void_p), ("bars", C.c_void_p),
                ("batch", C.c_void_p), ("is_drum", C.c_void_p), ("tokens", C.c_void_p), ("s_tensor", C.c_void_p),
                ("N", C.c_int32), ("E", C.c_int32), ("G", C.c_int32), ("B", C.c_int32), ("n_slots", C.c_int32),
# ... 109 lines not shown
        self.loss_buf = torch.zeros(4, dtype=torch.float64, device=dev)
        ci = vae._counter_index
        emb = ["encoder.c_encoder.bn_drums", "encoder.c_encoder.bn_non_drums", "encoder.c_encoder.bn_dur"]
        inc = torch.ones(vae.flat_counters.numel(), dtype=torch.int64, device=dev)
        sel = torch.zeros(2, vae.flat_counters.numel(), dtype=torch.int64, device=dev)
        for k, row in zip(emb, ((1, 0), (0, 1), (1, 1))):
            i = ci[k + ".num_batches_tracked"]
            inc[i] = 0
            sel[0, i], sel[1, i] = row
        self._nbt_inc, self._nbt_sel = inc, sel

    @property
    def addr(self) -> int:
        return C.addressof(self.state)

    def forward(self, graph, eps, grads, keep_logits: bool, beta: float = 0.0, fix_structure: bool = False,
                n_slots=None, ce_scale=None, want_token_counts: bool = False, ext_loss: bool = False):
        vae, L = self.vae, lib()
        if vae.flat_params.data_ptr() != self.flat_ptr:
            raise RuntimeError("the model's flat parameter buffer moved after the native step was built; rebuild it")
        inputs = prepare_inputs(graph, want_token_counts)
        et, ed, tok, drum, ei, bars, bat, act_slots, unique = inputs[:9]
        s_tensor = graph.s_tensor
        if s_tensor.dtype != torch.float32 or not s_tensor.is_contiguous():
            s_tensor = s_tensor.float().contiguous()
        s_tensor = s_tensor.reshape(-1, 4, 32)
        bt = make_batch(ei, bars, bat, s_tensor, tok, drum, et, ed, act_slots if n_slots is None else n_slots, unique,
                        keep_logits=keep_logits, ext_loss=ext_loss)
        if ce_scale is not None:
            bt.ce_scale = ce_scale.data_ptr()
        bt.B = bt.G // vae.cfg["n_bars"]
        need = int(L.pm_vae_step_workspace_bytes(C.byref(self.layout), bt.N, bt.E, bt.G, bt.B, bt.n_slots))
        if self.ws is None or self.ws.numel() < need:
            self.ws = torch.empty(need, dtype=torch.uint8, device=grads.device)
        off = self._plan_layout(bt.N, bt.E, bt.G)
        if self.plan_buf is None or self.plan_buf.numel() < off[-1]:
            self.plan_buf = torch.empty(off[-1], dtype=torch.int32, device=grads.device)
        if eps is None:
            eps = torch.randn(bt.B, vae.cfg["d"], device=grads.device)
        self.bt, self.plan_off, self._keep = bt, off, (s_tensor, eps, grads, ce_scale, inputs)
        ptr = self._ptr
        self._call("pm_vae_step_forward", C.addressof(self.layout), ptr(vae.flat_params), ptr(vae.flat_buffers), ptr(grads),
                   C.addressof(bt), ptr(self.plan_buf), ptr(eps), float(vae.msg_dropout), vae._next_seed(), vae._next_seed(),
                   float(beta), int(fix_structure), ptr(self.ws), self.ws.numel(), self.addr, ptr(self.loss_buf), self._stream())
        return self.loss_buf

    def info(self) -> dict:
        info = (C.c_int32 * 16)()
        self._call("pm_vae_step_info", self.addr, C.cast(info, C.c_void_p))
        keys = ("compact", "planes", "n_slots", "b_frag", "N", "E", "G", "B", "fused_ce", "side_stream", "deterministic",
                "gcl_fused", "dagg_bn", "chord_tables", "h2", "pad_skip")
        return dict(zip(keys, (int(v) for v in info)))

    def outputs(self):
        i, vae = self.info(), self.vae
        dev, d, nb = vae.flat_params.device, vae.cfg["d"], vae.cfg["n_bars"]
        s_logits = torch.empty(i["B"], nb, 4, 32, device=dev)
        c_logits = torch.empty(i["N"], i["n_slots"], 230, device=dev)
        mu, lv = torch.empty(i["B"], d, device=dev), torch.empty(i["B"], d, device=dev)
        ptr = self._ptr
        self._call("pm_vae_step_outputs", self.addr, ptr(s_logits), ptr(c_logits), ptr(mu), ptr(lv), self._stream())
        return (s_logits, c_logits), mu, lv

    def output_views(self):
        off, num = (C.c_int64 * 8)(), (C.c_int64 * 8)()
        self._call("pm_vae_step_output_views", self.addr, C.cast(off, C.c_void_p), C.cast(num, C.c_void_p))
        i, vae = self.info(), self.vae
        d, nb = vae.cfg["d"], vae.cfg["n_bars"]
        shapes = ((i["B"], nb, 4, 32), (i["N"], i["n_slots"], 230), (i["B"], d), (i["B"], d))
        s_logits, c_logits, mu, lv = (self.ws[int(off[k]):int(off[k]) + 4 * int(num[k])].view(torch.float32).view(shapes[k])
                                      for k in range(4))
        return (s_logits, c_logits), mu, lv

    def set_output_grads(self, ds_logits, dc_logits, dmu, dlv):
        ptr = self._ptr
        self._grad_refs = (ds_logits, dc_logits, dmu, dlv)
        self._call("pm_vae_step_set_output_grads", self.addr, ptr(ds_logits), ptr(dc_logits), ptr(dmu), ptr(dlv), self._stream())

    def backward_decoder(self):
        self._call("pm_vae_step_backward_decoder", self.addr, self._stream())

    def backward_encoder_heads(self):
        self._call("pm_vae_step_backward_encoder_heads", self.addr, self._stream())

    def backward_encoder(self):
        self._call("pm_vae_step_backward_encoder", self.addr, self._stream())

    def backward_encoder_tail(self):
        self._call("pm_vae_step_backward_encoder_tail", self.addr, self._stream())

    def bump_counters(self):
        vae, ptr = self.vae, self._ptr
        i = self._fields.index("group_cnt")
        off = self.plan_off
        self._call("pm_bn_counters_update", ptr(vae.flat_counters), ptr(self._nbt_inc), ptr(self._nbt_sel),
                   ptr(self.plan_buf[off[i]:off[i] + 2]), vae.flat_counters.numel(), self._stream())

    def plan_word(self, field: str, index: int) -> int:
        j = self._fields.index(field)
        return int(self.plan_buf[self.plan_off[j] + index].item())
```

### polyphemus_amd/trainer.py

```python
from __future__ import annotations

import contextlib
import ctypes
import math
import os
import warnings
from typing import Dict, Optional

import torch

from . import ops
from ._lib import call, h2_clamp_init, lib, ptr, stream
from .model import VAE, prepare_graph
from .native import NativeStep, prepare_inputs
from .parallel import GradBuckets, broadcast_


class ExpDecayLR:

    def __init__(self, peak_lr, warmup_steps, final_lr_scale, decay_steps):
        self.peak_lr, self.warmup_steps = peak_lr, warmup_steps
        self.decay_factor = -math.log(final_lr_scale) / decay_steps
        self.update_steps = 0

# ... 162 lines not shown
            call("pm_vae_step_set_metrics", step.addr, self._mhist[self._mrows].data_ptr())
        step.forward(graph, eps, self.grads, keep_logits=self.keep_logits, beta=self.beta,
                     fix_structure=self.fix_structure_loss, ce_scale=ce_scale, want_token_counts=gtm)
        if prepare_inputs(graph)[8] and os.environ.get("PM_DEBUG", "0") not in ("", "0"):
            bad = step.plan_word("trk_cnt", 4)
            if bad:
                raise RuntimeError(f"{bad} nodes receive track edges of more than one track but the batch was "
                                   "flagged track_unique (graphs.batch_flags); the compact GCL would be wrong")
        step.backward_decoder()
        step.backward_encoder_heads()
        self.buckets.launch(2)
        step.backward_encoder()
        self.buckets.launch(1)
        step.backward_encoder_tail()
        if self._poison:
            ops.overflow_poison(self.grads, self._ovf_status)
        self.buckets.launch(0)
        step.bump_counters()
        return step.loss_buf

    @property
    def last_train_counts(self) -> torch.Tensor:
        if not self.train_metrics:
            raise RuntimeError("last_train_counts needs HipTrainer(..., train_metrics=True)")
        if self._mrows == 0:
            raise RuntimeError("no training-accuracy counts since the last read_train_accuracies()")
        return self._mhist[self._mrows - 1]

    def read_train_accuracies(self, reduce: bool = False) -> list:
        if not self.train_metrics:
            raise RuntimeError("read_train_accuracies needs HipTrainer(..., train_metrics=True)")
        rows = self._mhist[:self._mrows]
        if reduce and self.world > 1:
            import torch.distributed as dist
            rows = rows.clone()
            dist.all_reduce(rows, group=self.pg)
        host = rows.tolist()
        self._mrows = 0
        return [ops.accuracies_from_counts(r) for r in host]

    @property
    def last_grad_norm(self) -> torch.Tensor:
        if self.max_grad_norm is None:
            raise RuntimeError("last_grad_norm needs HipTrainer(..., max_grad_norm=...)")
        return self._clip[ops.CLIP_NORM]

    def read_grad_norms(self) -> list:
        if self.max_grad_norm is None:
            raise RuntimeError("read_grad_norms needs HipTrainer(..., max_grad_norm=...)")
        host = self._nhist[:self._nrows].tolist()
        self._nrows = 0
        return [(r[0], r[1]) for r in host]

    def step_info(self) -> dict:
        return self.step.info()

    def step_outputs(self):
        i = self.step_info()
        if not self.keep_logits and i["fused_ce"]:
            raise RuntimeError("step_outputs needs trainer.keep_logits = True before the step (the fused un-embedding + "
                               "cross-entropy does not store the logits otherwise)")
        return self.step.outputs()

    def _python_forward_backward(self, graph, eps):
        vae, eng = self.vae, self.vae.engine
        if self._guard:
            ops.overflow_snapshot(self._ovf_status)
        eng.msg_dropout = vae.msg_dropout
        graph.__dict__.pop("_pm_plan", None)
        plan = prepare_graph(graph, vae.cfg["n_bars"])
        G = self._G
        s_tensor = graph.s_tensor.float().contiguous()
        mu, lv, esv = eng.encoder_forward(plan, s_tensor, True, vae._next_seed())
        if eps is None:
            eps = torch.randn_like(mu)
        z = ops.reparam_fwd(mu, lv, eps)
        s_logits, c_logits, dsv = eng.decoder_forward(plan, z, True, vae._next_seed())
        ce_scale = 1.0
        if self.global_token_mean and self.world > 1:
            import torch.distributed as dist
            tok = plan.tokens
            n_loc = (tok[:, 1:, 0] != 130).sum().double().reshape(1)
            n_all = n_loc.clone()
            dist.all_reduce(n_all, group=self.pg)
            ce_scale = float(n_loc.item()) * self.world / float(n_all.item())
        out, dc = ops.content_ce(c_logits, plan, grad_scale=ce_scale, want_grad=True, out=self.loss_buf)
        dmu, dlv = torch.zeros_like(mu), torch.zeros_like(lv)
        ops.kld(mu, lv, out, beta=self.beta, dmu=dmu, dlog_var=dlv)
        if self.fix_structure_loss:
            _, ds = ops.bce_logits(s_logits.reshape(-1), s_tensor.reshape(-1), out, 1.0, want_grad=True)
            ds = ds.view_as(s_logits)
        else:
            ops.bce_logits(s_tensor.reshape(-1), s_tensor.reshape(-1), out, 1.0, want_grad=False)
            ds = None
        if self.train_metrics:
            row = self._mhist[self._mrows]
            cl = c_logits.contiguous()
            row[:8].copy_(ops.content_accuracy(cl, plan.tokens, plan.is_drum) if cl.shape[1] == 15 else
                          ops.content_accuracy_slots(cl, plan.tokens, plan.is_drum)[:8])
            s_in = s_logits.reshape(-1).contiguous() if self.fix_structure_loss else s_tensor.reshape(-1)
            row[8:12].copy_(ops.structure_metrics(s_in, s_tensor.reshape(-1)))
            row[12].fill_(s_tensor.numel())
            row[13:].zero_()
        dz = eng.decoder_backward(dsv, ds, dc, G)
        self.buckets.launch(2)
        ops.reparam_bwd(dz, lv, eps, dmu, dlv)
        eng.encoder_backward(esv, dmu, dlv, G)
        self.buckets.launch(1)
# ... 244 lines not shown
```

Measured before the change: 136,000.

## Use two-plane fp16 (h2) products for decoder chord head rows-times-weight GEMM

Adds an h2 variant of the rows-times-weight kernel that splits activations and weights into two scaled fp16 planes instead of three bf16 planes. It uses 3 MFMA passes instead of 6, with scales taken from absmax slots. The last decoder GCN layer's BN apply now writes a 16-slot absmax, and the chord weights get their own absmax to drive the weight split. This targets the MFMA and LDS cost of the decoder chord projection. The risks are fp16 range clamping and some loss of precision, plus one extra absmax launch per step.

Measured after the change: 136,400, median of 6. No clear change (+0.3%).

```diff
diff --git a/include/polyphemus_hip.h b/include/polyphemus_hip.h
--- a/include/polyphemus_hip.h
+++ b/include/polyphemus_hip.h
@@ -162,8 +162,12 @@
   const uint32_t* absmax_in; const uint32_t* absmax_aux; float* scale_out; float w_scale; int32_t reserved;
 } PmH2;
 int pm_absmax(const float* x, int64_t n, uint32_t* out, pm_stream_t stream);
+enum { PM_HEAD_ABSMAX_SLOTS = 16 };
+int pm_absmax_slots(const float* x, int64_t n, uint32_t* out, int32_t slots, pm_stream_t stream);
 int pm_split_planes_frag_h2(const float* W, int32_t rows, int32_t cols, int32_t kind, int32_t n_mats, int64_t src_stride,
                             int64_t dst_stride, float w_scale, uint16_t* out, pm_stream_t stream);
+int pm_split_planes_frag_h2_absmax(const float* W, int32_t rows, int32_t cols, int32_t kind, int32_t n_mats, int64_t src_stride,
+                                   int64_t dst_stride, const uint32_t* absmax, uint16_t* out, pm_stream_t stream);
 int pm_gcl_forward_fused_h2(const float* x, const float* T, const int32_t* plan, int32_t N, int32_t E, int32_t G, int32_t d,
                             float dropout_p, uint32_t seed, uint32_t layer_uid, const uint16_t* w_frag, const float* bias,
                             int32_t use_classes, float* h, double* col_stats, uint16_t* planes, int64_t plane_stride,
@@ -198,6 +202,12 @@
                          pm_stream_t stream);
 int pm_rows_times_weight_longk(const float* X, int32_t ldx, int32_t N, int32_t K, const uint16_t* w_frag, int32_t kind,
                                int32_t w_pitch, int32_t Nout, float* C, int32_t ldc, pm_stream_t stream);
+int pm_rows_times_weight_h2(const float* X, int32_t ldx, int32_t N, int32_t K, const uint16_t* w_frag, int32_t kind,
+                            int32_t w_tiles, int32_t Nout, const float* bias , float* C, int32_t ldc,
+                            const uint32_t* absmax_x, const uint32_t* absmax_w, pm_stream_t stream);
+int pm_rows_times_weight_longk_h2(const float* X, int32_t ldx, int32_t N, int32_t K, const uint16_t* w_frag, int32_t kind,
+                                  int32_t w_pitch, int32_t Nout, float* C, int32_t ldc, const uint32_t* absmax_x,
+                                  const uint32_t* absmax_w, pm_stream_t stream);
 int pm_rows_tn_weight_grad(const float* A, int32_t lda, int32_t M, const float* B, int32_t ldb, int32_t Nn, int32_t K,
                            float* C , int32_t ldc, float* colsum_a , pm_stream_t stream);
 typedef struct PmNormSums {
@@ -308,6 +318,10 @@
                              const float* beta, const float* residual, int relu, float* y, float* mean, float* var,
                              float* running_mean, float* running_var, float momentum, uint32_t* absmax_out,
                              pm_stream_t stream);
+int pm_bn_apply_fused_absmax_slots(const float* x, int32_t O, int32_t C, const double* sums, float eps, const float* gamma,
+                                   const float* beta, const float* residual, int relu, float* y, float* mean, float* var,
+                                   float* running_mean, float* running_var, float momentum, uint32_t* absmax_out,
+                                   int32_t slots, pm_stream_t stream);
 int pm_bn_bwd_fused(const float* x, const float* dy, int32_t O, int32_t C, const float* mean, const float* var,
                     float eps, const float* gamma, const float* beta, int relu, float* dgamma, float* dbeta,
                     float* dbias_pre , float* dx , double* acc3,
@@ -601,6 +615,7 @@
                         void* workspace, int64_t workspace_bytes, void* state, double* losses ,
                         pm_stream_t stream);
 int pm_vae_step_info(const void* state, int32_t* info );
+int pm_vae_step_head_info(const void* state);
 int pm_vae_step_outputs(const void* state, float* s_logits, float* c_logits, float* mu, float* log_var,
                         pm_stream_t stream);
 enum { PM_SAVED_GCN_H = 0,
diff --git a/polyphemus_amd/_lib.py b/polyphemus_amd/_lib.py
--- a/polyphemus_amd/_lib.py
+++ b/polyphemus_amd/_lib.py
@@ -43,6 +43,8 @@
     "pm_gcl_forward_from_planes": "plpiiiippipps",
     "pm_rows_times_weight": "piiipiiippis",
     "pm_rows_times_weight_longk": "piiipiiipis",
+    "pm_rows_times_weight_h2": "piiipiiippipps",
+    "pm_rows_times_weight_longk_h2": "piiipiiipipps",
     "pm_rows_tn_weight_grad": "piipiiipips",
     "pm_segreduce_bwd": "pppppiiiifuuipps",
     "pm_segreduce_bwd_norm": "pppppiiiifuuippps",
@@ -136,7 +138,11 @@
     "pm_vae_step_reload_switches": "",
     "pm_relu_bwd_planes": "pplppls",
     "pm_absmax": "plps",
+    "pm_absmax_slots": "plpis",
     "pm_split_planes_frag_h2": "piiiillfps",
+    "pm_split_planes_frag_h2_absmax": "piiiillpps",
+    "pm_bn_apply_fused_absmax_slots": "piipfpppipppppfpis",
+    "pm_vae_step_head_info": "p",
     "pm_gcl_forward_fused_h2": "pppiiiifuuppippplps",
     "pm_gcl_input_grad_bn_h2": "pplpiiiipipps",
     "pm_gcl_weight_grad_fused_h2": "plplpiiiiippps",
diff --git a/polyphemus_amd/csrc/common.h b/polyphemus_amd/csrc/common.h
--- a/polyphemus_amd/csrc/common.h
+++ b/polyphemus_amd/csrc/common.h
@@ -173,13 +173,20 @@
   for (int o = 32; o > 0; o >>= 1) v = fmaxf(v, __shfl_xor(v, o, 64));
   return v;
 }
-__device__ static inline void pm_absmax_block(unsigned* __restrict__ out, float v, unsigned* sm) {
+__device__ static inline float pm_absmax_read_head(const unsigned* __restrict__ p) {
+  static_assert((PM_HEAD_ABSMAX_SLOTS & (PM_HEAD_ABSMAX_SLOTS - 1)) == 0 && PM_HEAD_ABSMAX_SLOTS <= 64, "a lane per slot");
+  float v = __uint_as_float(p[__lane_id() & (PM_HEAD_ABSMAX_SLOTS - 1)]);
+#pragma unroll
+  for (int o = PM_HEAD_ABSMAX_SLOTS / 2; o > 0; o >>= 1) v = fmaxf(v, __shfl_xor(v, o, 64));
+  return v;
+}
+__device__ static inline void pm_absmax_block(unsigned* __restrict__ out, float v, unsigned* sm, int slots = PM_ABSMAX_SLOTS) {
   v = fabsf(v);
 #pragma unroll
   for (int o = 32; o > 0; o >>= 1) v = fmaxf(v, __shfl_xor(v, o, 64));
   if ((threadIdx.x & 63) == 0) atomicMax(sm, __float_as_uint(v));
   __syncthreads();
-  if (threadIdx.x == 0) atomicMax(out + (blockIdx.x % PM_ABSMAX_SLOTS), *sm);
+  if (threadIdx.x == 0) atomicMax(out + (blockIdx.x % slots), *sm);
 }
 __device__ static inline void pm_store_planes4(uint16_t* __restrict__ planes, int64_t plane_stride, int64_t idx, float x0,
                                                float x1, float x2, float x3) {
diff --git a/polyphemus_amd/csrc/gemm.hip b/polyphemus_amd/csrc/gemm.hip
--- a/polyphemus_amd/csrc/gemm.hip
+++ b/polyphemus_amd/csrc/gemm.hip
@@ -954,8 +954,10 @@
 template <bool H2>
 __global__ void __launch_bounds__(256) k_split_planes_frag(const float* __restrict__ W, int rows, int cols, int kind,
                                                            int64_t src_stride, int64_t dst_stride,
-                                                           uint16_t* __restrict__ out, float w_scale, unsigned* clamps) {
+                                                           uint16_t* __restrict__ out, float w_scale, unsigned* clamps,
+                                                           const unsigned* __restrict__ absmax) {
   bool cut = false;
+  if constexpr (H2) { if (absmax) w_scale = pm_pow2_scale(pm_absmax_read_head(absmax), 13); }
   const float* src = W + (int64_t)blockIdx.y * src_stride;
   uint16_t* dst = out + (int64_t)blockIdx.y * dst_stride;
   const int64_t chunks = (int64_t)rows * cols / 8;
@@ -993,7 +995,8 @@
   if (H2 && cut && clamps) atomicAdd(clamps, 1u);
 }
 static int split_planes_frag_impl(const float* W, int32_t rows, int32_t cols, int32_t kind, int32_t n_mats,
-                                  int64_t src_stride, int64_t dst_stride, float w_scale, uint16_t* out, pm_stream_t stream) {
+                                  int64_t src_stride, int64_t dst_stride, float w_scale, uint16_t* out, pm_stream_t stream,
+                                  const uint32_t* absmax = nullptr) {
   if (!W || !out || rows <= 0 || cols <= 0 || (rows % 32) || (cols % 32) || (kind != 0 && kind != 1) || n_mats <= 0 ||
       ((uintptr_t)W % 16) || ((uintptr_t)out % 16) || (src_stride % 4) || (dst_stride % 8))
     return PM_E_INVALID;
@@ -1001,10 +1004,10 @@
   if (grid > 2048) grid = 2048;
   if (w_scale > 0.f)
     hipLaunchKernelGGL(k_split_planes_frag<true>, dim3((unsigned)grid, (unsigned)n_mats), dim3(256), 0, (hipStream_t)stream, W,
-                       rows, cols, kind, src_stride, dst_stride, out, w_scale, pm_h2_clamp_word());
+                       rows, cols, kind, src_stride, dst_stride, out, w_scale, pm_h2_clamp_word(), absmax);
   else
     hipLaunchKernelGGL(k_split_planes_frag<false>, dim3((unsigned)grid, (unsigned)n_mats), dim3(256), 0, (hipStream_t)stream, W,
-                       rows, cols, kind, src_stride, dst_stride, out, 0.f, nullptr);
+                       rows, cols, kind, src_stride, dst_stride, out, 0.f, nullptr, nullptr);
   return pm_check_launch();
 }
 extern "C" int pm_split_planes_frag(const float* W, int32_t rows, int32_t cols, int32_t kind, int32_t n_mats,
@@ -1016,7 +1019,13 @@
   if (!(w_scale > 0.f)) return PM_E_INVALID;
   return split_planes_frag_impl(W, rows, cols, kind, n_mats, src_stride, dst_stride, w_scale, out, stream);
 }
-__global__ void __launch_bounds__(256) k_absmax(const float* __restrict__ x, int64_t n, unsigned* __restrict__ out) {
+extern "C" int pm_split_planes_frag_h2_absmax(const float* W, int32_t rows, int32_t cols, int32_t kind, int32_t n_mats,
+                                              int64_t src_stride, int64_t dst_stride, const uint32_t* absmax, uint16_t* out,
+                                              pm_stream_t stream) {
+  if (!absmax) return PM_E_INVALID;
+  return split_planes_frag_impl(W, rows, cols, kind, n_mats, src_stride, dst_stride, 1.f, out, stream, absmax);
+}
+__global__ void __launch_bounds__(256) k_absmax(const float* __restrict__ x, int64_t n, unsigned* __restrict__ out, int slots) {
   __shared__ unsigned sm;
   if (threadIdx.x == 0) sm = 0u;
   __syncthreads();
@@ -1027,14 +1036,17 @@
     m = fmaxf(fmaxf(m, fmaxf(fabsf(v.x), fabsf(v.y))), fmaxf(fabsf(v.z), fabsf(v.w)));
   }
   if (blockIdx.x == 0 && threadIdx.x < (int)(n & 3)) m = fmaxf(m, fabsf(x[(n4 << 2) + threadIdx.x]));
-  pm_absmax_block(out, m, &sm);
-}
-extern "C" int pm_absmax(const float* x, int64_t n, uint32_t* out, pm_stream_t stream) {
-  if (!x || !out || n <= 0 || ((uintptr_t)x % 16)) return PM_E_INVALID;
+  pm_absmax_block(out, m, &sm, slots);
+}
+extern "C" int pm_absmax_slots(const float* x, int64_t n, uint32_t* out, int32_t slots, pm_stream_t stream) {
+  if (!x || !out || n <= 0 || ((uintptr_t)x % 16) || slots < 1 || slots > PM_ABSMAX_SLOTS || (slots & (slots - 1))) return PM_E_INVALID;
   int64_t grid = pm_cdiv(n / 4 + 1, 256 * 4);
   if (grid > 512) grid = 512;
-  hipLaunchKernelGGL(k_absmax, dim3((unsigned)grid), dim3(256), 0, (hipStream_t)stream, x, n, out);
+  hipLaunchKernelGGL(k_absmax, dim3((unsigned)grid), dim3(256), 0, (hipStream_t)stream, x, n, out, slots);
   return pm_check_launch();
+}
+extern "C" int pm_absmax(const float* x, int64_t n, uint32_t* out, pm_stream_t stream) {
+  return pm_absmax_slots(x, n, out, PM_ABSMAX_SLOTS, stream);
 }
 
 PmProfState g_pm_prof = {false, 0, 0, nullptr, ~0ull, 1, {0}};
diff --git a/polyphemus_amd/csrc/linear.hip b/polyphemus_amd/csrc/linear.hip
--- a/polyphemus_amd/csrc/linear.hip
+++ b/polyphemus_amd/csrc/linear.hip
@@ -9,11 +9,13 @@
 #endif
 template <int D> constexpr int rows_nmw() { return D == 256 ? ROWS_NMW : 4; }
 template <int D> constexpr int rows_threads() { return (rows_nmw<D>() + 4) * 64; }
-template <int D, int BKIND>
+struct RowsH2 { const unsigned* mx; const unsigned* mw; unsigned* clamps; };
+template <int D, int BKIND, bool H2>
 __global__ void __launch_bounds__(rows_threads<D>()) __attribute__((amdgpu_waves_per_eu((rows_nmw<D>() + 4) / 4, (rows_nmw<D>() + 4) / 4)))
 k_rows_w(const float* __restrict__ X, int ldx, int N, const char* __restrict__ wfrag, int wtiles, int nblk,
-         const float* __restrict__ bias, float* __restrict__ C, int ldc) {
+         const float* __restrict__ bias, float* __restrict__ C, int ldc, RowsH2 h2) {
   constexpr int NMW = rows_nmw<D>(), WC = D / NMW, TN = WC / 32, KS = D / 16, RB = D * 2, PL = BM * RB;
+  constexpr int NPL = H2 ? 2 : 3, T60 = H2 ? 3 : 0;
   extern __shared__ __attribute__((aligned(16))) char smem[];
   float* const sC = reinterpret_cast<float*>(smem + 3 * PL);
   int m0 = 0, rows = BM;
@@ -21,6 +23,11 @@
   const bool full = rows > BM / 2;
   N = min(N, m0 + rows);
   const int tid = threadIdx.x, lane = tid & 63, wave = tid >> 6, li = lane & 31, lh = lane >> 5;
+  float xsc = 1.f, ix = 1.f, iw = 1.f;
+  if constexpr (H2) {
+    xsc = pm_pow2_scale(pm_absmax_read_head(h2.mx), 13);
+    ix = 1.f / xsc; iw = 1.f / pm_pow2_scale(pm_absmax_read_head(h2.mw), 13);
+  }
   if (wave >= NMW) {
     constexpr int LPR = D / 4, RPW = 64 / LPR, NR = BM / (4 * RPW);
     const int st = tid - NMW * 64, c4 = st % LPR, r0 = st / LPR;
@@ -47,6 +54,7 @@
     const __amdgpu_buffer_rsrc_t rs = __builtin_amdgcn_make_buffer_rsrc(const_cast<float*>(X), 0, GCL_OOB, 0x00020000);
     constexpr int CPR = D / 8, NST = NMW * 64, NCHK = BM * CPR / NST;
     u32x4 v[NCHK][2];
+    bool cut = false;
 #pragma unroll
     for (int k = 0; k < NCHK; ++k) {
       const int ci = tid + k * NST, rr = ci / CPR, ch = ci % CPR, row = m0 + rr;
@@ -60,14 +68,22 @@
       unsigned p1[4], p2[4], p3[4];
 #pragma unroll
       for (int h = 0; h < 2; ++h) {
-        pm_split3_pair(__uint_as_float(v[k][h][0]), __uint_as_float(v[k][h][1]), p1[2 * h], p2[2 * h], p3[2 * h]);
-        pm_split3_pair(__uint_as_float(v[k][h][2]), __uint_as_float(v[k][h][3]), p1[2 * h + 1], p2[2 * h + 1], p3[2 * h + 1]);
+        const float x0 = __uint_as_float(v[k][h][0]), x1 = __uint_as_float(v[k][h][1]), x2 = __uint_as_float(v[k][h][2]),
+                    x3 = __uint_as_float(v[k][h][3]);
+        if constexpr (H2) {
+          pm_split2h_pair(pm_clamp_f16(x0 * xsc, cut), pm_clamp_f16(x1 * xsc, cut), p1[2 * h], p2[2 * h]);
+          pm_split2h_pair(pm_clamp_f16(x2 * xsc, cut), pm_clamp_f16(x3 * xsc, cut), p1[2 * h + 1], p2[2 * h + 1]);
+        } else {
+          pm_split3_pair(x0, x1, p1[2 * h], p2[2 * h], p3[2 * h]);
+          pm_split3_pair(x2, x3, p1[2 * h + 1], p2[2 * h + 1], p3[2 * h + 1]);
+        }
       }
       char* dst = smem + rr * RB + ((ch ^ (rr & 15)) << 4);
       *reinterpret_cast<u32x4*>(dst) = u32x4{p1[0], p1[1], p1[2], p1[3]};
       *reinterpret_cast<u32x4*>(dst + PL) = u32x4{p2[0], p2[1], p2[2], p2[3]};
-      *reinterpret_cast<u32x4*>(dst + 2 * PL) = u32x4{p3[0], p3[1], p3[2], p3[3]};
-    }
+      if constexpr (!H2) *reinterpret_cast<u32x4*>(dst + 2 * PL) = u32x4{p3[0], p3[1], p3[2], p3[3]};
+    }
+    if (H2 && cut && h2.clamps) atomicAdd(h2.clamps, 1u);
   }
   const __amdgpu_buffer_rsrc_t brs = __builtin_amdgcn_make_buffer_rsrc(const_cast<char*>(wfrag), 0, GCL_OOB, 0x00020000);
   auto bload = [&](bf16x8 (&dst)[3][TN], int gs) {
@@ -77,7 +93,7 @@
 #pragma unroll
     for (int j = 0; j < TN; ++j)
 #pragma unroll
-      for (int p = 0; p < 3; ++p)
+      for (int p = 0; p < NPL; ++p)
         dst[p][j] = __builtin_bit_cast(bf16x8, __builtin_amdgcn_raw_buffer_load_b128(brs, lane * 16, soff + j * (BKIND == 0 ? KS : 1) * 3072 + p * 1024, 0));
   };
   bf16x8 bq[GCL_BDEPTH][3][TN];
@@ -86,7 +102,7 @@
   __syncthreads();
   auto aload = [&](bf16x8 (&a)[3][2], int ks) {
 #pragma unroll
-    for (int p = 0; p < 3; ++p)
+    for (int p = 0; p < NPL; ++p)
 #pragma unroll
       for (int i = 0; i < 2; ++i) {
         const int rr = i * 32 + li;
@@ -111,12 +127,12 @@
       aload(af[(ks + 1) & 1], (ks + 1) % KS);
       constexpr int PA[6] = {2, 1, 0, 1, 0, 0}, PB[6] = {0, 1, 2, 0, 1, 0};
 #pragma unroll
-      for (int t6 = 0; t6 < 6; ++t6)
+      for (int t6 = T60; t6 < 6; ++t6)
 #pragma unroll
         for (int i = 0; i < NI; ++i)
 #pragma unroll
           for (int j = 0; j < TN; ++j)
-            acc[i][j] = __builtin_amdgcn_mfma_f32_32x32x16_bf16(af[ks & 1][PA[t6]][i], bq[ks % GCL_BDEPTH][PB[t6]][j], acc[i][j], 0, 0, 0);
+            acc[i][j] = gcl_mfma<H2>(af[ks & 1][PA[t6]][i], bq[ks % GCL_BDEPTH][PB[t6]][j], acc[i][j]);
       bload(bq[ks % GCL_BDEPTH], qb * KS + ks + GCL_BDEPTH);
       __builtin_amdgcn_sched_barrier(0);
     }
@@ -127,7 +143,7 @@
       for (int r = 0; r < 16; ++r)
 #pragma unroll
         for (int j = 0; j < TN; ++j)
-          sC[(i * 32 + (r & 3) + 8 * (r >> 2) + 4 * lh) * D + wave * WC + j * 32 + li] = acc[i][j][r];
+          sC[(i * 32 + (r & 3) + 8 * (r >> 2) + 4 * lh) * D + wave * WC + j * 32 + li] = H2 ? acc[i][j][r] * ix * iw : acc[i][j][r];
     __syncthreads();
   }
   };
@@ -135,42 +151,58 @@
   else blocks(std::integral_constant<int, 1>{});
 }
 
-extern "C" int pm_rows_times_weight(const float* X, int32_t ldx, int32_t N, int32_t K, const uint16_t* w_frag, int32_t kind,
-                                    int32_t w_tiles, int32_t Nout, const float* bias, float* C, int32_t ldc,
-                                    pm_stream_t stream) {
+static int rows_times_weight_impl(const float* X, int32_t ldx, int32_t N, int32_t K, const uint16_t* w_frag, int32_t kind,
+                                  int32_t w_tiles, int32_t Nout, const float* bias, float* C, int32_t ldc, const RowsH2* h2,
+                                  pm_stream_t stream) {
   if (!X || !w_frag || !C || N <= 0 || (K != 128 && K != 256 && K != 512) || Nout <= 0 || (Nout % K) || (kind != 0 && kind != 1) ||
       ldx < K || ldc < Nout || (ldx & 3) || (ldc & 3) || ((uintptr_t)X % 16) || ((uintptr_t)C % 16) ||
       ((uintptr_t)w_frag % 16) || (bias && ((uintptr_t)bias % 16)) || (int64_t)N * ldx * 4 >= 0x7fffffffLL ||
       (int64_t)N * ldc * 4 >= 0x7fffffffLL || (kind == 1 && w_tiles * 32 < Nout))
     return PM_E_INVALID;
+  if (h2 && (K == 512 || !h2->mx || !h2->mw)) return PM_E_INVALID;
   if (K == 512)
     return pm_wide_rows_times_weight(X, ldx, N, w_frag, kind, w_tiles, Nout, bias, C, ldc, (hipStream_t)stream);
+  const RowsH2 hh = h2 ? *h2 : RowsH2{nullptr, nullptr, nullptr};
   hipStream_t st = (hipStream_t)stream;
   const dim3 grid(pm_row_grid(N));
   const size_t lds = (size_t)3 * BM * K * 2 + (size_t)BM * K * 4;
   const int pe = pm_prof_open(st, PM_PROF_ROWS_W, 2.0 * N * (double)K * Nout);
-#define LAUNCH(DD, KD)                                                                                                 \
+#define LAUNCH(DD, KD, HH)                                                                                             \
   do {                                                                                                                 \
     static bool once_dev[16] = {}; bool& once = once_dev[pm_device_slot()];                                                                                          \
     if (!once) {                                                                                                       \
-      hipFuncSetAttribute((const void*)k_rows_w<DD, KD>, hipFuncAttributeMaxDynamicSharedMemorySize, 160 * 1024);      \
+      hipFuncSetAttribute((const void*)k_rows_w<DD, KD, HH>, hipFuncAttributeMaxDynamicSharedMemorySize, 160 * 1024);  \
       once = true;                                                                                                     \
     }                                                                                                                  \
-    hipLaunchKernelGGL((k_rows_w<DD, KD>), grid, dim3(rows_threads<DD>()), lds, st, X, ldx, N, reinterpret_cast<const char*>(w_frag), \
-                       w_tiles, Nout / K, bias, C, ldc);                                                               \
+    hipLaunchKernelGGL((k_rows_w<DD, KD, HH>), grid, dim3(rows_threads<DD>()), lds, st, X, ldx, N, reinterpret_cast<const char*>(w_frag), \
+                       w_tiles, Nout / K, bias, C, ldc, hh);                                                           \
   } while (0)
-  if (K == 256) { if (kind == 0) LAUNCH(256, 0); else LAUNCH(256, 1); }
-  else { if (kind == 0) LAUNCH(128, 0); else LAUNCH(128, 1); }
+#define LAUNCH2(DD, KD) do { if (h2) LAUNCH(DD, KD, true); else LAUNCH(DD, KD, false); } while (0)
+  if (K == 256) { if (kind == 0) LAUNCH2(256, 0); else LAUNCH2(256, 1); }
+  else { if (kind == 0) LAUNCH2(128, 0); else LAUNCH2(128, 1); }
+#undef LAUNCH2
 #undef LAUNCH
   pm_prof_close(st, pe);
   return pm_check_launch();
 }
-
-template <int D, int BKIND>
+extern "C" int pm_rows_times_weight(const float* X, int32_t ldx, int32_t N, int32_t K, const uint16_t* w_frag, int32_t kind,
+                                    int32_t w_tiles, int32_t Nout, const float* bias, float* C, int32_t ldc,
+                                    pm_stream_t stream) {
+  return rows_times_weight_impl(X, ldx, N, K, w_frag, kind, w_tiles, Nout, bias, C, ldc, nullptr, stream);
+}
+extern "C" int pm_rows_times_weight_h2(const float* X, int32_t ldx, int32_t N, int32_t K, const uint16_t* w_frag, int32_t kind,
+                                       int32_t w_tiles, int32_t Nout, const float* bias, float* C, int32_t ldc,
+                                       const uint32_t* absmax_x, const uint32_t* absmax_w, pm_stream_t stream) {
+  const RowsH2 h2 = {absmax_x, absmax_w, pm_h2_clamp_word_ready()};
+  return rows_times_weight_impl(X, ldx, N, K, w_frag, kind, w_tiles, Nout, bias, C, ldc, &h2, stream);
+}
+
+template <int D, int BKIND, bool H2>
 __global__ void __launch_bounds__(rows_threads<D>()) __attribute__((amdgpu_waves_per_eu((rows_nmw<D>() + 4) / 4, (rows_nmw<D>() + 4) / 4)))
 k_rows_wk(const float* __restrict__ X, int ldx, int N, int K, const char* __restrict__ wfrag, int wpitch,
-          float* __restrict__ C, int ldc) {
+          float* __restrict__ C, int ldc, RowsH2 h2) {
   constexpr int NMW = rows_nmw<D>(), WC = D / NMW, TN = WC / 32, HS = D + 8, NTHR = rows_threads<D>();
+  constexpr int NPL = H2 ? 2 : 3, T60 = H2 ? 3 : 0;
   extern __shared__ __attribute__((aligned(16))) char smem[];
   float* const sH = reinterpret_cast<float*>(smem);
   const int nchunk = K / CH;
@@ -179,6 +211,11 @@
   const bool full = rows > BM / 2;
   N = min(N, m0 + rows);
   const int tid = threadIdx.x, lane = tid & 63, wave = tid >> 6;
+  float xsc = 1.f, ix = 1.f, iw = 1.f;
+  if constexpr (H2) {
+    xsc = pm_pow2_scale(pm_absmax_read_head(h2.mx), 13);
+    ix = 1.f / xsc; iw = 1.f / pm_pow2_scale(pm_absmax_read_head(h2.mw), 13);
+  }
   if (wave >= NMW) {
     const int pt = tid - NMW * 64, q = pt & 31, prow = pt >> 5;
     const __amdgpu_buffer_rsrc_t xrs = __builtin_amdgcn_make_buffer_rsrc(const_cast<float*>(X), 0, GCL_OOB, 0x00020000);
@@ -190,19 +227,25 @@
             xrs, (row < N && c < nchunk) ? (int)(((int64_t)row * ldx + c * CH + q * 4) * 4) : GCL_OOB, 0, 0));
       }
     };
+    bool cut = false;
     auto put = [&](const float4 (&xs)[8], int c) {
       char* img = smem + (c & 1) * IMG;
 #pragma unroll
       for (int ps = 0; ps < 8; ++ps) {
         const int rr = ps * 8 + prow;
-        unsigned l1, l2, l3, u1, u2, u3;
-        pm_split3_pair(xs[ps].x, xs[ps].y, l1, l2, l3);
-        pm_split3_pair(xs[ps].z, xs[ps].w, u1, u2, u3);
+        unsigned l1, l2, l3 = 0, u1, u2, u3 = 0;
+        if constexpr (H2) {
+          pm_split2h_pair(pm_clamp_f16(xs[ps].x * xsc, cut), pm_clamp_f16(xs[ps].y * xsc, cut), l1, l2);
+          pm_split2h_pair(pm_clamp_f16(xs[ps].z * xsc, cut), pm_clamp_f16(xs[ps].w * xsc, cut), u1, u2);
+        } else {
+          pm_split3_pair(xs[ps].x, xs[ps].y, l1, l2, l3);
+          pm_split3_pair(xs[ps].z, xs[ps].w, u1, u2, u3);
+        }
         const pm_u32x2 p1 = {l1, u1}, p2 = {l2, u2}, p3 = {l3, u3};
         char* dst = img + rr * ROWB + (((q >> 1) ^ (rr & 15)) << 4) + ((q & 1) << 3);
         *reinterpret_cast<pm_u32x2*>(dst) = p1;
         *reinterpret_cast<pm_u32x2*>(dst + PLANE) = p2;
-        *reinterpret_cast<pm_u32x2*>(dst + 2 * PLANE) = p3;
+        if constexpr (!H2) *reinterpret_cast<pm_u32x2*>(dst + 2 * PLANE) = p3;
       }
     };
     float4 xa[8], xb[8];
@@ -223,6 +266,7 @@
       put(xa, c + 2);
       __syncthreads();
     }
+    if (H2 && cut && h2.clamps) atomicAdd(h2.clamps, 1u);
   } else {
     const int li = lane & 31, lh = lane >> 5;
     f32x16 acc[2][TN];
@@ -240,7 +284,7 @@
 #pragma unroll
       for (int j = 0; j < TN; ++j)
 #pragma unroll
-        for (int p = 0; p < 3; ++p)
+        for (int p = 0; p < NPL; ++p)
           dst[p][j] = __builtin_bit_cast(bf16x8, __builtin_amdgcn_raw_buffer_load_b128(brs, lane * 16, soff + j * (BKIND == 0 ? wpitch : 1) * 3072 + p * 1024, 0));
     };
     bf16x8 bq[GCL_BDEPTH][3][TN];
@@ -256,7 +300,7 @@
         for (int ks = 0; ks < 8; ++ks) {
           bf16x8 a[3][NI];
 #pragma unroll
-          for (int p = 0; p < 3; ++p)
+          for (int p = 0; p < NPL; ++p)
 #pragma unroll
             for (int i = 0; i < NI; ++i) {
               const int rr = i * 32 + li;
@@ -264,12 +308,12 @@
             }
           constexpr int PA[6] = {2, 1, 0, 1, 0, 0}, PB[6] = {0, 1, 2, 0, 1, 0};
 #pragma unroll
-          for (int t6 = 0; t6 < 6; ++t6)
+          for (int t6 = T60; t6 < 6; ++t6)
 #pragma unroll
             for (int i = 0; i < NI; ++i)
 #pragma unroll
               for (int j = 0; j < TN; ++j)
-                acc[i][j] = __builtin_amdgcn_mfma_f32_32x32x16_bf16(a[PA[t6]][i], bq[ks % GCL_BDEPTH][PB[t6]][j], acc[i][j], 0, 0, 0);
+                acc[i][j] = gcl_mfma<H2>(a[PA[t6]][i], bq[ks % GCL_BDEPTH][PB[t6]][j], acc[i][j]);
           bload(bq[ks % GCL_BDEPTH], c * 8 + ks + GCL_BDEPTH);
           __builtin_amdgcn_sched_barrier(0);
         }
@@ -284,7 +328,7 @@
       for (int i = 0; i < 2; ++i)
 #pragma unroll
         for (int r = 0; r < 16; ++r)
-          sH[(i * 32 + (r & 3) + 8 * (r >> 2) + 4 * lh) * HS + n0 + j * 32 + li] = acc[i][j][r];
+          sH[(i * 32 + (r & 3) + 8 * (r >> 2) + 4 * lh) * HS + n0 + j * 32 + li] = H2 ? acc[i][j][r] * ix * iw : acc[i][j][r];
   }
   __syncthreads();
   constexpr int NG = 512 / D, RG = BM / NG;
@@ -299,34 +343,49 @@
   }
 }
 
-extern "C" int pm_rows_times_weight_longk(const float* X, int32_t ldx, int32_t N, int32_t K, const uint16_t* w_frag,
-                                          int32_t kind, int32_t w_pitch, int32_t Nout, float* C, int32_t ldc,
-                                          pm_stream_t stream) {
+static int rows_times_weight_longk_impl(const float* X, int32_t ldx, int32_t N, int32_t K, const uint16_t* w_frag,
+                                        int32_t kind, int32_t w_pitch, int32_t Nout, float* C, int32_t ldc, const RowsH2* h2,
+                                        pm_stream_t stream) {
   if (!X || !w_frag || !C || N <= 0 || K <= 0 || (K % CH) || (Nout != 128 && Nout != 256 && Nout != 512) || (kind != 0 && kind != 1) ||
       ldx < K || ldc < Nout || (ldx & 3) || ((uintptr_t)X % 16) || ((uintptr_t)w_frag % 16) ||
       (int64_t)N * ldx * 4 >= 0x7fffffffLL || (int64_t)N * ldc * 4 >= 0x7fffffffLL || (kind == 0 && w_pitch * 16 < K))
     return PM_E_INVALID;
+  if (h2 && (Nout == 512 || !h2->mx || !h2->mw)) return PM_E_INVALID;
   if (Nout == 512)
     return pm_wide_rows_times_weight_longk(X, ldx, N, K, w_frag, kind, w_pitch, C, ldc, (hipStream_t)stream);
+  const RowsH2 hh = h2 ? *h2 : RowsH2{nullptr, nullptr, nullptr};
   hipStream_t st = (hipStream_t)stream;
   const dim3 grid(pm_row_grid(N));
   const size_t lds = 2 * IMG;
   const int pe = pm_prof_open(st, PM_PROF_ROWS_W, 2.0 * N * (double)K * Nout);
-#define LAUNCH(DD, KD)                                                                                                 \
+#define LAUNCH(DD, KD, HH)                                                                                             \
   do {                                                                                                                 \
     static bool once_dev[16] = {}; bool& once = once_dev[pm_device_slot()];                                                                                          \
     if (!once) {                                                                                                       \
-      hipFuncSetAttribute((const void*)k_rows_wk<DD, KD>, hipFuncAttributeMaxDynamicSharedMemorySize, 160 * 1024);     \
+      hipFuncSetAttribute((const void*)k_rows_wk<DD, KD, HH>, hipFuncAttributeMaxDynamicSharedMemorySize, 160 * 1024); \
       once = true;                                                                                                     \
     }                                                                                                                  \
-    hipLaunchKernelGGL((k_rows_wk<DD, KD>), grid, dim3(rows_threads<DD>()), lds, st, X, ldx, N, K, reinterpret_cast<const char*>(w_frag), \
-                       w_pitch, C, ldc);                                                                               \
+    hipLaunchKernelGGL((k_rows_wk<DD, KD, HH>), grid, dim3(rows_threads<DD>()), lds, st, X, ldx, N, K, reinterpret_cast<const char*>(w_frag), \
+                       w_pitch, C, ldc, hh);                                                                           \
   } while (0)
-  if (Nout == 256) { if (kind == 0) LAUNCH(256, 0); else LAUNCH(256, 1); }
-  else { if (kind == 0) LAUNCH(128, 0); else LAUNCH(128, 1); }
+#define LAUNCH2(DD, KD) do { if (h2) LAUNCH(DD, KD, true); else LAUNCH(DD, KD, false); } while (0)
+  if (Nout == 256) { if (kind == 0) LAUNCH2(256, 0); else LAUNCH2(256, 1); }
+  else { if (kind == 0) LAUNCH2(128, 0); else LAUNCH2(128, 1); }
+#undef LAUNCH2
 #undef LAUNCH
   pm_prof_close(st, pe);
   return pm_check_launch();
+}
+extern "C" int pm_rows_times_weight_longk(const float* X, int32_t ldx, int32_t N, int32_t K, const uint16_t* w_frag,
+                                          int32_t kind, int32_t w_pitch, int32_t Nout, float* C, int32_t ldc,
+                                          pm_stream_t stream) {
+  return rows_times_weight_longk_impl(X, ldx, N, K, w_frag, kind, w_pitch, Nout, C, ldc, nullptr, stream);
+}
+extern "C" int pm_rows_times_weight_longk_h2(const float* X, int32_t ldx, int32_t N, int32_t K, const uint16_t* w_frag,
+                                             int32_t kind, int32_t w_pitch, int32_t Nout, float* C, int32_t ldc,
+                                             const uint32_t* absmax_x, const uint32_t* absmax_w, pm_stream_t stream) {
+  const RowsH2 h2 = {absmax_x, absmax_w, pm_h2_clamp_word_ready()};
+  return rows_times_weight_longk_impl(X, ldx, N, K, w_frag, kind, w_pitch, Nout, C, ldc, &h2, stream);
 }
 
 
diff --git a/polyphemus_amd/csrc/norm.hip b/polyphemus_amd/csrc/norm.hip
--- a/polyphemus_amd/csrc/norm.hip
+++ b/polyphemus_amd/csrc/norm.hip
@@ -420,7 +420,7 @@
                                                         const double* __restrict__ sums, BnCtx ctx,
                                                         const float* __restrict__ res, float* __restrict__ y,
                                                         float* mean, float* var, float* rmean, float* rvar,
-                                                        float momentum, unsigned* absmax) {
+                                                        float momentum, unsigned* absmax, int amax_slots) {
   extern __shared__ __attribute__((aligned(16))) float sm[];
   float amax = 0.f;
   __shared__ unsigned s_amax;
@@ -465,7 +465,7 @@
     if (res) rv = reinterpret_cast<const float4*>(res)[i];
     apply(i, xv, rv);
   }
-  if (absmax) pm_absmax_block(absmax, amax, &s_amax);
+  if (absmax) pm_absmax_block(absmax, amax, &s_amax, amax_slots);
 }
 extern "C" int pm_bn_apply_fused_absmax(const float* x, int32_t O, int32_t C, const double* sums, float eps,
                                         const float* gamma, const float* beta, const float* residual, int relu, float* y,
@@ -482,6 +482,14 @@
                                         const float* gamma, const float* beta, const float* residual, int relu, float* y,
                                         float* mean, float* var, float* running_mean, float* running_var, float momentum,
                                         uint32_t* absmax_out, pm_stream_t stream) {
+  return pm_bn_apply_fused_absmax_slots(x, O, C, sums, eps, gamma, beta, residual, relu, y, mean, var, running_mean, running_var,
+                                        momentum, absmax_out, PM_ABSMAX_SLOTS, stream);
+}
+extern "C" int pm_bn_apply_fused_absmax_slots(const float* x, int32_t O, int32_t C, const double* sums, float eps,
+                                              const float* gamma, const float* beta, const float* residual, int relu, float* y,
+                                              float* mean, float* var, float* running_mean, float* running_var, float momentum,
+                                              uint32_t* absmax_out, int32_t slots, pm_stream_t stream) {
+  if (slots < 1 || slots > PM_ABSMAX_SLOTS || (slots & (slots - 1))) return PM_E_INVALID;
   if (!x || !sums || !gamma || !beta || !y || !mean || !var || O <= 0 || C <= 0 || (C % 4) != 0 || C > 4096)
     return PM_E_INVALID;
   if (((uintptr_t)x % 16) || ((uintptr_t)y % 16) || (residual && ((uintptr_t)residual % 16))) return PM_E_INVALID;
@@ -490,7 +498,7 @@
   constexpr int thr = 1024, gcap = 512;
   int64_t gr = pm_cdiv(n / 4, thr); if (gr > gcap) gr = gcap; if (gr < 1) gr = 1;
   hipLaunchKernelGGL(k_bn_apply4_sums, dim3((unsigned)gr), dim3(thr), sizeof(float) * 3 * C, (hipStream_t)stream, x,
-                     n / 4, C, (double)O, sums, ctx, residual, y, mean, var, running_mean, running_var, momentum, absmax_out);
+                     n / 4, C, (double)O, sums, ctx, residual, y, mean, var, running_mean, running_var, momentum, absmax_out, (int)slots);
   return pm_check_launch();
 }
 
diff --git a/polyphemus_amd/csrc/vae_step.hip b/polyphemus_amd/csrc/vae_step.hip
--- a/polyphemus_amd/csrc/vae_step.hip
+++ b/polyphemus_amd/csrc/vae_step.hip
@@ -26,6 +26,7 @@
   bool chord_tables;
   bool plan_side;
   bool h2;
+  bool head_h2;
   bool senc_first;
   bool unembed_dw;
   bool pad_skip;
@@ -48,6 +49,7 @@
   k.chord_tables = flag("PM_CHORD_TABLES", true);
   k.dagg_res = flag("PM_DAGG_RES", true);
   k.h2 = flag("PM_H2", true);
+  k.head_h2 = flag("PM_HEAD_H2", true);
   k.side_delay_us = getenv("PM_SIDE_DELAY_US") ? atoi(getenv("PM_SIDE_DELAY_US")) : 0;
   k.bar_route = flag("PM_BAR_ROUTE", true);
   k.pad_skip = flag("PM_PAD_SKIP", true);
@@ -106,6 +108,7 @@
   bool chord_dw_tn;
   bool dec_rows;
   bool dec_dw_tn;
+  bool dec_h2;
   enum Ue { UE_KERNEL, UE_PRODUCTS } ue_fwd, ue_dh, ue_dw;
   bool ue_rows;
   bool keep_logits;
@@ -128,6 +131,7 @@
   double* pool;
   uint32_t seed, uid0; float p;
   uint32_t* mx; uint32_t* mdu; float* sA; float* sdh;
+  uint32_t* mhead; uint32_t* xl_absmax;
   bool x0_maxed;
   const float* x0_src; int64_t x0_src_n;
 };
@@ -367,6 +371,7 @@
   r.chord_dw_tn = r.chord == HeadRoute::CHORD_FRAG && rows_tn_pays(d);
   r.dec_rows = rows_w_ok(c);
   r.dec_dw_tn = r.dec_rows && rows_tn_pays(d);
+  r.dec_h2 = r.dec_rows && k.h2 && k.head_h2 && (d == 128 || d == 256) && c.bn && c.L >= 1;
   r.keep_logits = (s.bt.flags & 4) != 0;
   r.logits_only = (s.bt.flags & 8) != 0;
   r.metrics = !r.logits_only && s.metrics != nullptr;
@@ -384,7 +389,7 @@
   return r;
 }
 void head_route_gradient_in_any_row(HeadRoute& r) { r.ue_rows = false; }
-void gcn_prepare(Ctx& c, const PmGcn& g, GcnSaved& sv) {
+void gcn_prepare(Ctx& c, const PmGcn& g, GcnSaved& sv, int head_words = 0) {
   Arena& ar = c.s->ar;
   const int d = c.d;
   const int64_t dd = (int64_t)d * d;
@@ -393,9 +398,10 @@
   sv.pool = ar.zdbl((size_t)c.L * 5 * d * PM_BN_REPL);
   {
     constexpr int SL = PM_ABSMAX_SLOTS;
-    uint32_t* w = (uint32_t*)ar.z(sizeof(uint32_t) * (size_t)((2 * c.L + 1) * SL + 2 * c.L));
+    uint32_t* w = (uint32_t*)ar.z(sizeof(uint32_t) * (size_t)((2 * c.L + 1) * SL + 2 * c.L + head_words));
     sv.mx = w; sv.mdu = w ? w + (c.L + 1) * SL : nullptr; sv.sA = w ? (float*)(w + (2 * c.L + 1) * SL) : nullptr;
     sv.sdh = w ? sv.sA + c.L : nullptr;
+    sv.mhead = (w && head_words) ? w + (2 * c.L + 1) * SL + 2 * c.L : nullptr;
   }
   const int64_t lstride = c.L > 2 ? g.weight[2] - g.weight[1] : 7 * dd;
   sv.Wfn = sv.Wft = nullptr; sv.wf_stride = 7 * dd * 3;
@@ -513,7 +519,10 @@
       }
     }
     const PmBn& bn = g.norm[i];
-    if (c.bn)
+    if (c.bn && i + 1 == c.L && sv.xl_absmax)
+      RUN(pm_bn_apply_fused_absmax_slots(sv.h[i], N, d, sums, 1e-5f, c.P + bn.w, c.P + bn.b, sv.x[i], 1, sv.x[i + 1], sv.mean[i],
+                                           sv.var[i], c.Bf + bn.rm, c.Bf + bn.rv, 0.1f, sv.xl_absmax, PM_HEAD_ABSMAX_SLOTS, c.st));
+    else if (c.bn)
       RUN(pm_bn_apply_fused_absmax(sv.h[i], N, d, sums, 1e-5f, c.P + bn.w, c.P + bn.b, sv.x[i], 1, sv.x[i + 1], sv.mean[i],
                                      sv.var[i], c.Bf + bn.rm, c.Bf + bn.rv, 0.1f,
                                      (r.x_tracked && i + 1 < c.L) ? sv.mx + (i + 1) * PM_ABSMAX_SLOTS : nullptr, c.st));
@@ -810,13 +819,19 @@
 void decoder_prep(Ctx& c, BranchScope& br) {
   StepState& s = *c.s; Arena& ar = s.ar; const PmVaeLayout& Y = s.lay;
   const int N = c.N, d = c.d, S = c.S;
-  gcn_prepare(c, Y.dec_gcn, s.dg);
+  gcn_prepare(c, Y.dec_gcn, s.dg, 2 * PM_HEAD_ABSMAX_SLOTS);
   if (rows_w_ok(c)) {
     s.wf_dec = (uint16_t*)ar.take((size_t)S * d * d * 6);
     s.wf_dec_t = (uint16_t*)ar.take((size_t)S * d * d * 6);
+    uint32_t* const mw = s.dg.mhead ? s.dg.mhead + PM_HEAD_ABSMAX_SLOTS : nullptr;
+    if (s.head.dec_h2) RUN(pm_absmax_slots(c.P + Y.dec_chord.w, (int64_t)S * d * d, mw, PM_HEAD_ABSMAX_SLOTS, c.st));
     for (int kind = 0; kind < 2; ++kind)
-      RUN(pm_split_planes_frag(c.P + Y.dec_chord.w, S * d, d, kind, 1, (int64_t)S * d * d, (int64_t)S * d * d * 3,
-                                 kind ? s.wf_dec_t : s.wf_dec, c.st));
+      if (s.head.dec_h2 && kind == 0)
+        RUN(pm_split_planes_frag_h2_absmax(c.P + Y.dec_chord.w, S * d, d, kind, 1, (int64_t)S * d * d, (int64_t)S * d * d * 3, mw,
+                                             kind ? s.wf_dec_t : s.wf_dec, c.st));
+      else
+        RUN(pm_split_planes_frag(c.P + Y.dec_chord.w, S * d, d, kind, 1, (int64_t)S * d * d, (int64_t)S * d * d * 3,
+                                   kind ? s.wf_dec_t : s.wf_dec, c.st));
   }
   if (unembed_dh_ok(c)) {
     s.w_unembed_dh = (uint16_t*)ar.take((size_t)pm_unembed_dh_scratch_bytes(d));
@@ -951,7 +966,10 @@
   uint16_t* const w_unembed = fused_ce_on() ? (uint16_t*)ar.take((size_t)pm_unembed_scratch_bytes(d)) : nullptr;
   double* const pad_losses = ar.zdbl(4);
   if (!ar.base) return;
-  if (rt.dec_rows) RUN(pm_rows_times_weight(xdL, d, N, d, s.wf_dec, 0, 0, S * d, c.P + Y.dec_chord.b, s.H, S * d, c.st));
+  if (rt.dec_h2)
+    RUN(pm_rows_times_weight_h2(xdL, d, N, d, s.wf_dec, 0, 0, S * d, c.P + Y.dec_chord.b, s.H, S * d, s.dg.mhead,
+                                  s.dg.mhead + PM_HEAD_ABSMAX_SLOTS, c.st));
+  else if (rt.dec_rows) RUN(pm_rows_times_weight(xdL, d, N, d, s.wf_dec, 0, 0, S * d, c.P + Y.dec_chord.b, s.H, S * d, c.st));
   else lin(c, xdL, Y.dec_chord, N, S * d, d, s.H, false);
   drop(c, s.H, N, S * d, SITE_DEC_CHORD, s.seed_dec, s.H);
   int64_t* const met = rt.metrics ? s.metrics : nullptr;
@@ -999,6 +1017,7 @@
   plan_and_encoder_prep(c, br);
   float* x0 = embeddings_and_chord_encoder(c);
   if (run) branch_join(c, BR_WPREP);
+  s.eg.xl_absmax = nullptr;
   float* xL = gcn_forward(c, x0, Y.enc_gcn, s.eg, seed_enc, 0, msg_p);
   decoder_prep_and_structure_encoder(c, br);
   attention_pool(c, xL);
@@ -1007,6 +1026,7 @@
   if (run) branch_join(c, BR_WPREP_DEC);
   if (run) branch_join(c, BR_ENC_FWD);
   s.dg.x0_src = s.cb; s.dg.x0_src_n = (int64_t)c.Gn * c.d;
+  s.dg.xl_absmax = s.head.dec_h2 ? s.dg.mhead : nullptr;
   float* xdL = gcn_forward(c, xd0, Y.dec_gcn, s.dg, seed_dec, 1000, msg_p);
   structure_decoder(c);
   decoder_head(c, xdL);
@@ -1345,6 +1365,11 @@
   info[15] = rt.ue_rows ? 1 : 0;
   return PM_OK;
 }
+extern "C" int pm_vae_step_head_info(const void* state) {
+  const StepState* s = (const StepState*)state;
+  if (!s || s->magic != kMagic) return PM_E_INVALID;
+  return s->head.dec_h2 ? 1 : 0;
+}
 extern "C" int pm_vae_step_outputs(const void* state, float* s_logits, float* c_logits, float* mu, float* log_var,
                                    pm_stream_t stream) {
   const StepState* s = (const StepState*)state;
diff --git a/polyphemus_amd/native.py b/polyphemus_amd/native.py
--- a/polyphemus_amd/native.py
+++ b/polyphemus_amd/native.py
@@ -5,7 +5,7 @@
 
 import torch
 
-from ._lib import lib
+from ._lib import HipExtensionError, lib
 
 PM_MAX_LAYERS = 16
 
@@ -221,6 +221,12 @@
                 "gcl_fused", "dagg_bn", "chord_tables", "h2", "pad_skip")
         return dict(zip(keys, (int(v) for v in info)))
 
+    def head_info(self) -> dict:
+        bits = int(lib().pm_vae_step_head_info(self.addr))
+        if bits < 0:
+            raise HipExtensionError(f"pm_vae_step_head_info failed: {bits}")
+        return {"head_h2": bits & 1}
+
     def outputs(self):
         i, vae = self.info(), self.vae
         dev, d, nb = vae.flat_params.device, vae.cfg["d"], vae.cfg["n_bars"]
diff --git a/polyphemus_amd/trainer.py b/polyphemus_amd/trainer.py
--- a/polyphemus_amd/trainer.py
+++ b/polyphemus_amd/trainer.py
@@ -238,8 +238,11 @@
         self._nrows = 0
         return [(r[0], r[1]) for r in host]
 
-    def step_info(self) -> dict:
-        return self.step.info()
+    def step_info(self, head: bool = False) -> dict:
+        info = self.step.info()
+        if head:
+            info.update(self.step.head_info())
+        return info
 
     def step_outputs(self):
         i = self.step_info()
```
